# safe-autonomous-systems/fluidgym

Measured on AMD Instinct MI355X. Metric: env-steps/sec (batched) + pressure-Poisson HBM GB/s vs roofline, 1/2/4/8 GPUs, higher is better.
Workload: dtype f32; 1 GPU; ChannelJet2D-v0 (2D channel stand-in for 'cylinder Re=100 256x128'), 64 envs/GPU, 25 PISO steps/env step, random jets, stirred by a body force N(0,2.0) redrawn every env step; global_batch=64, parallelism=env-sharded x1, 1 bcast + 1 all_gather per step (RCCL), lanes_per_gpu=2, workload_modified=True, capped_solves=0, floor_released_solves=0, advection_solver_form=two-brick, velocity_solver=on-chip Jacobi sweeps (policy advection_jacobi; 11972 solves settled by

## Files before the change

fluidgym_amd/_lib.py:

```python
from __future__ import annotations

import ctypes
import os
from ctypes import POINTER, Structure, c_char_p, c_float, c_int, c_int32, c_int64, c_void_p

_HERE = os.path.dirname(os.path.abspath(__file__))
LIB_PATH = os.environ.get("FLUIDGYM_AMD_LIB") or os.path.join(_HERE, "libfluidgym_hip.so")
LIB_F64_PATH = os.environ.get("FLUIDGYM_AMD_LIB_F64") or os.path.join(_HERE, "libfluidgym_hip_f64.so")

FG_MAX_SCALARS = 4
FG_FIELD_SUMMARY_WORK_BYTES = 128
FG_OK = 0
FG_ERR_NOT_CONVERGED = -5
FG_ERR_NOT_FINITE = -6
FG_ERR_FLUX_BALANCE = -7
FG_PERIODIC, FG_FIXED = 0, 1
FG_DIRICHLET, FG_NEUMANN = 0, 1
FG_VELOCITY, FG_PRESSURE, FG_SCALAR, FG_VELOCITY_SOURCE, FG_VISCOSITY_FIELD = 0, 1, 2, 3, 4
FG_BOUND_VELOCITY, FG_BOUND_SCALAR = 8, 16
FG_SOLVER_CG, FG_SOLVER_JACOBI, FG_SOLVER_RBGS, FG_SOLVER_MGCG, FG_SOLVER_FDCG = 0, 1, 2, 3, 4
(FG_BUF_A, FG_BUF_C_OFF, FG_BUF_ADV_RHS, FG_BUF_VEL_RESULT, FG_BUF_H, FG_BUF_DIV, FG_BUF_P_RESULT,
 FG_BUF_SCALAR_RESULT) = range(8)
FG_ERR_UNSUPPORTED = -4
FG_ERR_INVALID_ARG = -1
# ... 298 lines not shown
    "fg_poisson_cg": (c_int, [c_void_p, c_void_p, c_void_p, c_void_p, c_float, c_int, c_int, POINTER(FgSolveInfo),
                              c_void_p]),
    "fg_poisson_fdcg": (c_int, [c_void_p, c_void_p, c_void_p, c_void_p, c_float, c_int, c_int, POINTER(FgSolveInfo),
                                c_void_p]),
    "fg_sparse_apply_ell": (c_int, [c_void_p, c_void_p, c_int32, c_int32, c_void_p, c_int64, c_int32, c_void_p, c_void_p]),
    "fg_sparse_apply_csr": (c_int, [c_void_p, c_void_p, c_void_p, c_int32, c_void_p, c_int64, c_int32, c_void_p, c_void_p]),
    "fg_stream_triad": (c_int, [c_void_p, c_void_p, c_void_p, c_float, c_int64, c_int32, POINTER(c_float), c_void_p]),
    "fg_mb_multilevel_status": (c_int, [c_void_p, POINTER(c_int32)]),
    "fg_mb_multilevel_apply": (c_int, [c_void_p, c_void_p, c_void_p, c_void_p]),
    "fg_mb_debug_ilu_apply": (c_int, [c_void_p, c_void_p, c_void_p, c_void_p]),
    "fg_mb_debug_pressure_cg": (c_int, [c_void_p, c_float, c_int32, c_int32, POINTER(c_int32), POINTER(c_int32), POINTER(ctypes.c_double), c_void_p]),
    "fg_mb_wall_forces": (c_int, [c_void_p, c_void_p, c_void_p, c_void_p, c_int32, c_int32, c_float, c_float, c_void_p, c_void_p]),
    "fg_mb_wall_forces_batch": (c_int, [c_void_p, c_void_p, c_void_p, c_void_p, c_int32, c_int32, c_float, c_float, c_void_p, c_void_p, c_void_p]),
    "fg_mb_debug_bicgstab": (c_int, [c_void_p, c_float, c_int32, c_int32, POINTER(c_int64), POINTER(ctypes.c_double), POINTER(c_float), c_void_p]),
    "fg_dacc_host_sum": (c_int, [POINTER(ctypes.c_double), c_int64, ctypes.c_double, POINTER(ctypes.c_double)]),
    "fg_dacc_device_sum": (c_int, [POINTER(ctypes.c_double), c_int64, ctypes.c_double, c_int32, POINTER(ctypes.c_double), c_void_p]),
    "fg_field_summary": (c_int, [c_void_p, c_int32, c_int32, c_int64, c_int32, c_void_p, c_void_p, c_void_p, ctypes.c_double, ctypes.c_double,
                                 c_int32, c_void_p, c_void_p]),
    "fg_plane_moments": (c_int, [POINTER(c_void_p), POINTER(c_int64), c_int32, c_int32, c_int32, c_int32, c_int32, c_int32, c_void_p, c_void_p,
                                 c_void_p, c_void_p, c_void_p]),
    "fg_plane_budgets": (c_int, [POINTER(c_void_p), POINTER(c_int64), c_int32, c_int32, c_int32, c_int32, c_int32, c_void_p, c_void_p, c_void_p,
                                 c_int32, c_int32, c_void_p, c_void_p, c_void_p, c_void_p, c_void_p]),
    "fg_plane_timecorr": (c_int, [POINTER(c_void_p), POINTER(c_int64), c_int32, c_int32, c_int32, c_int32, c_int32, c_int32, c_int32,
                                  POINTER(c_int32), c_void_p, c_void_p, c_void_p, c_void_p]),
    "fg_mb_cell_moments": (c_int, [c_void_p, c_void_p, c_int32, c_int32, c_int64, POINTER(c_int64), c_int32, c_int64, c_void_p, c_void_p,
                                   c_void_p]),
    "fg_mb_cell_moments_widths": (c_int, [c_void_p, c_void_p, c_int64, POINTER(c_int64), c_int32, c_void_p, c_void_p, POINTER(c_int32)]),
    "fg_mb_wall_distribution": (c_int, [c_void_p, c_void_p, c_void_p, c_int32, c_int32, c_int64, c_int64, c_void_p, c_void_p, c_void_p, c_int32,
                                        c_int32, c_float, c_void_p, c_void_p, c_void_p]),
    "fg_mb_wall_moments": (c_int, [c_void_p, c_void_p, c_void_p, c_int32, c_int32, c_int64, c_int64, c_void_p, c_void_p, c_void_p, c_int32,
                                   c_int32, c_float, c_void_p, c_int32, c_int64, c_void_p, c_void_p, c_void_p]),
    "fg_plane_spectra": (c_int, [POINTER(c_void_p), POINTER(c_int64), c_int32, c_int32, c_int32, c_int32, c_int32, POINTER(c_int32), c_int32,
                                 c_void_p, c_void_p, c_void_p]),
    "fg_plane_histogram": (c_int, [POINTER(c_void_p), POINTER(c_int64), c_int32, c_int32, c_int32, c_int32, c_int32, POINTER(c_int32), c_int32,
                                   c_void_p, c_void_p, c_int32, POINTER(c_int32), c_int32, c_int32, c_void_p, c_void_p, c_void_p]),
    "fg_coherence_litmus": (c_int, [c_int32, c_int32, c_int32, c_int32, POINTER(c_int64), POINTER(ctypes.c_double), c_void_p]),
    "fg_profile_enable": (c_int, [c_void_p, c_int]),
    "fg_profile_kinds": (c_int, []),
    "fg_profile_kind_name": (ctypes.c_char_p, [c_int]),
    "fg_profile_read": (c_int, [c_void_p, c_int, POINTER(ctypes.c_double), POINTER(c_int64), POINTER(ctypes.c_double),
                                POINTER(ctypes.c_double), POINTER(ctypes.c_double), POINTER(ctypes.c_double),
                                POINTER(c_int64), POINTER(c_int64), POINTER(ctypes.c_double), POINTER(c_int64)]),
    "fg_coords_to_transforms": (c_int, [c_void_p, c_void_p, c_int, c_int, c_int, c_int, c_void_p]),
    "fg_resampler_create": (c_int, [c_int, POINTER(ctypes.c_int32), POINTER(ctypes.c_int32), POINTER(ctypes.c_int32),
                                    POINTER(ctypes.c_float), c_int, c_int, POINTER(c_void_p)]),
    "fg_resampler_destroy": (c_int, [c_void_p]),
    "fg_resample": (c_int, [c_void_p, c_void_p, c_int, c_int, c_void_p, c_int, c_void_p]),
    "fg_frame_colorize": (c_int, [c_void_p, c_int32, c_int32, c_int32, c_int32, c_int32, POINTER(FgFrameSpec), c_void_p, c_void_p, c_void_p,
                                  POINTER(c_int32), c_int32, c_void_p, c_void_p]),
    "fg_render_isosurface": (c_int, [c_void_p, c_int32, c_int32, c_int32, c_int32, c_int32, c_int32, c_void_p, c_void_p, c_int32, c_int32,
                                     c_void_p, c_void_p, c_void_p, POINTER(FgRenderCamera), POINTER(FgRenderOptions), c_int32, c_int32,
                                     POINTER(c_int32), c_int32, c_void_p, c_void_p, c_void_p]),
    "fg_render_volume": (c_int, [c_void_p, c_int32, c_int32, c_int32, c_int32, c_int32, c_int32, c_void_p, c_void_p, c_void_p,
                                 POINTER(FgRenderCamera), POINTER(FgRenderOptions), c_int32, c_int32, POINTER(c_int32), c_int32, c_void_p,
                                 c_void_p]),
    "fg_obs_noise_add": (c_int, [POINTER(FgNoiseSegment), c_int32, c_int32, c_int32, ctypes.c_uint64, c_void_p, c_void_p, c_void_p]),
    "fg_obs_normalize": (c_int, [POINTER(FgNormSegment), c_int32, c_int32, c_int32, c_int64, c_int64, c_void_p, c_int32, c_int32,
                                 ctypes.c_double, ctypes.c_double, c_void_p]),
    "fg_obs_return_normalize": (c_int, [c_void_p, c_void_p, c_void_p, c_void_p, c_int32, c_int32, ctypes.c_double, c_int64,
                                        ctypes.c_double, ctypes.c_double, c_int32, c_void_p]),
    "fg_baseline_opposition": (c_int, [c_void_p, c_int64, c_int32, c_int32, c_int32, c_int32, POINTER(c_int32), POINTER(ctypes.c_double), c_int32,
                                       c_int32, c_void_p, c_void_p]),
    "fg_baseline_pd": (c_int, [c_void_p, c_int64, c_int32, c_int32, c_int32, c_int32, c_int32, c_void_p, ctypes.c_double, ctypes.c_double,
                               c_void_p, c_void_p, c_void_p, c_void_p, c_void_p]),
    "fg_point_sample": (c_int, [POINTER(FgPointGrid), POINTER(c_void_p), POINTER(c_int64), c_int32, c_void_p, c_int64, c_int32, c_void_p,
                                c_void_p]),
    "fg_tracer_advect": (c_int, [POINTER(FgPointGrid), c_float, c_int32, ctypes.c_uint32, c_void_p, c_void_p, c_void_p, c_void_p, c_void_p,
                                 c_int32, c_void_p]),
    "fg_mb_point_locate": (c_int, [POINTER(FgMbPointMesh), c_void_p, c_int64, c_int32, c_void_p, c_int32, c_void_p, c_void_p, c_void_p,
                                   c_void_p]),
    "fg_mb_point_sample": (c_int, [POINTER(FgMbPointMesh), POINTER(c_void_p), POINTER(c_int64), c_int32, c_void_p, c_void_p, c_int64,
                                   c_int32, c_void_p, c_void_p]),
    "fg_mb_tracer_advect": (c_int, [POINTER(FgMbPointMesh), c_float, c_int32, c_void_p, c_void_p, c_void_p, c_void_p, c_void_p, c_void_p,
                                    c_void_p, c_void_p, c_int32, c_void_p]),
    "fg_envglue_jet_schedule": (c_int, [c_void_p, c_void_p, c_void_p, c_void_p, c_int32, c_int32, c_int32, c_void_p, c_void_p, c_void_p]),
    "fg_envglue_channel_observe": (c_int, [c_void_p, c_void_p, c_void_p, c_int32, c_int32, c_int32, c_int32, c_float, c_float, c_void_p,
                                           c_void_p, c_void_p, c_void_p, c_void_p, c_void_p]),
    "fg_envglue_channel_observe_batch": (c_int, [c_void_p, c_void_p, c_void_p, c_int32, c_int32, c_int32, c_int32, c_void_p, c_float, c_void_p,
                                                 c_void_p, c_void_p, c_void_p, c_void_p, c_void_p]),
    "fg_mb_create": (c_int, [c_int32, c_int32, c_int32, POINTER(c_void_p)]),
    "fg_mb_destroy": (c_int, [c_void_p]),
    "fg_config_dump": (c_int, [c_void_p, ctypes.c_char_p, c_int]),
    "fg_mb_config_dump": (c_int, [c_void_p, ctypes.c_char_p, c_int]),
    "fg_switch_values": (c_int, [c_int32, ctypes.c_char_p, c_int32]),
    "fg_mb_add_block": (c_int, [c_void_p, POINTER(c_float), c_int32, c_int32, c_int32, POINTER(c_int32)]),
    "fg_mb_connect": (c_int, [c_void_p, c_int32, c_int32, c_int32, c_int32, c_int32, c_int32]),
    "fg_mb_make_periodic": (c_int, [c_void_p, c_int32, c_int32]),
    "fg_mb_set_reference_quirks": (c_int, [c_void_p, c_int32, c_int32]),
    "fg_mb_set_nonortho_flags": (c_int, [c_void_p, c_int32]),
    "fg_mb_finalize": (c_int, [c_void_p]),
    "fg_mb_sizes": (c_int, [c_void_p, POINTER(c_int32), POINTER(c_int32)]),
    "fg_mb_block_info": (c_int, [c_void_p, c_int32, POINTER(c_int32), POINTER(c_int32)]),
    "fg_mb_get_host_table": (c_int, [c_void_p, c_int32, c_void_p, POINTER(c_int64)]),
    "fg_mb_get_neighbors": (c_int, [c_void_p, POINTER(c_int32)]),
    "fg_mb_bind": (c_int, [c_void_p, c_void_p, c_void_p, c_void_p, c_void_p]),
    "fg_mb_set_viscosity": (c_int, [c_void_p, c_float]),
    "fg_mb_set_viscosity_batch": (c_int, [c_void_p, c_void_p]),
    "fg_mb_piso_step": (c_int, [c_void_p, c_void_p, POINTER(FgMbStepOptions), POINTER(c_int32), c_void_p]),
    "fg_mb_max_velocity": (c_int, [c_void_p, POINTER(c_float), c_void_p]),
    "fg_mb_set_residual_projection": (c_int, [c_void_p, POINTER(c_float)]),
    "fg_mb_set_stall_limit": (c_int, [c_void_p, c_int32]),
    "fg_mb_set_advection_start": (c_int, [c_void_p, c_int]),
    "fg_mb_set_advection_jacobi": (c_int, [c_void_p, c_int]),
    "fg_mb_advection_jacobi_counts": (c_int, [c_void_p, POINTER(c_int64)]),
    "fg_mb_set_multilevel": (c_int, [c_void_p, c_int32, c_int32, POINTER(c_int32), POINTER(c_int32), POINTER(c_int32), POINTER(c_float),
                                     POINTER(c_float), c_float, c_int32]),
    "fg_mb_env_status": (c_int, [c_void_p, POINTER(c_int32)]),
    "fg_mb_ladder": (c_int, [c_void_p, POINTER(c_int64), c_int32]),
    "fg_mb_debug_cycles": (c_int, [c_void_p, POINTER(ctypes.c_uint64)]),
    "fg_mb_solver_hints": (c_int, [c_void_p, POINTER(c_int32), c_int32]),
    "fg_mb_solver_unconverged": (c_int, [c_void_p, POINTER(c_int64)]),
    "fg_solver_unconverged": (c_int, [c_void_p, POINTER(c_int64)]),
    "fg_mb_solver_counters": (c_int, [c_void_p, POINTER(c_int64), c_int32]),
    "fg_set_advection_preconditioner": (c_int, [c_void_p, c_int]),
    "fg_debug_apply_preconditioner": (c_int, [c_void_p, c_int, c_int, c_void_p, c_void_p, POINTER(c_int32), c_void_p]),
    "fg_debug_apply_pressure_preconditioner": (c_int, [c_void_p, c_int, c_void_p, c_void_p, c_void_p, POINTER(ctypes.c_double),
                                                       POINTER(c_int32), c_void_p]),
    "fg_sgs_smagorinsky": (c_int, [c_void_p, c_float, c_void_p, c_void_p]),
    "fg_flow_diagnostic": (c_int, [c_void_p, c_int, c_void_p, c_void_p]),
    "fg_mb_flow_diagnostic": (c_int, [c_void_p, c_int, c_void_p, c_void_p]),
    "fg_set_fd_helmholtz": (c_int, [c_void_p, POINTER(c_float)]),
    "fg_advection_retries": (c_int, [c_void_p, POINTER(c_int64), c_int32]),
    "fg_advection_solver_form": (c_int, [c_void_p, c_int, POINTER(c_int32)]),
    "fg_set_double_fallback": (c_int, [c_void_p, c_int]),
    "fg_set_advection_jacobi": (c_int, [c_void_p, c_int]),
    "fg_advection_jacobi_counts": (c_int, [c_void_p, POINTER(c_int64)]),
    "fg_ladder": (c_int, [c_void_p, POINTER(c_int64), c_int32]),
    "fg_solver_counters": (c_int, [c_void_p, POINTER(c_int64), c_int32]),
    "fg_mb_profile_iterations": (c_int, [c_void_p, POINTER(c_int64)]),
    "fg_mb_unit_pressure_matrix": (c_int, [c_void_p, c_void_p]),
    "fg_mb_profile_enable": (c_int, [c_void_p, c_int32]),
    "fg_mb_profile_kind_name": (c_char_p, [c_int32]),
    "fg_mb_profile_read": (c_int, [c_void_p, c_int32, POINTER(ctypes.c_double), POINTER(c_int64), POINTER(ctypes.c_double),
                                   POINTER(c_int64)]),
    "fg_mb_get_buffer": (c_int, [c_void_p, c_int32, POINTER(c_void_p), POINTER(c_int64)]),
    "fg_mb_read_buffer": (c_int, [c_void_p, c_int32, c_void_p, c_void_p]),
    "fg_mb_single_step": (c_int, [c_void_p, POINTER(FgMbSimOptions), POINTER(c_int32), POINTER(c_float), c_void_p]),
    "fg_mb_update_advective_boundary": (c_int, [c_void_p, c_float, c_int32, c_int32, c_int32, c_int32, POINTER(c_float), c_float, c_void_p]),
    "fg_mb_make_divergence_free": (c_int, [c_void_p, POINTER(FgMbStepOptions), c_void_p]),
    "fg_mb_boundary_flux_balance": (c_int, [c_void_p, POINTER(c_float), c_void_p]),
    "fg_mb_get_boundary_tables": (c_int, [c_void_p, POINTER(c_int32), POINTER(c_int32), POINTER(c_float)]),
    "fg_mb_get_cell_transforms": (c_int, [c_void_p, POINTER(c_float)]),
}

def _f64_struct(cls):
    fields = []
    for name, tp in cls._fields_:
        if tp is c_float:
            tp = ctypes.c_double
        elif isinstance(tp, type) and issubclass(tp, ctypes.Array) and tp._type_ is c_float:
            tp = ctypes.c_double * tp._length_
        elif isinstance(tp, type) and issubclass(tp, Structure) and tp in _F64_STRUCTS:
            tp = _F64_STRUCTS[tp]
        fields.append((name, tp))
    return type(cls.__name__ + "F64", (Structure,), {"_fields_": fields})


_F64_STRUCTS: dict = {}
_F64_STRUCTS[FgStepOptions] = _f64_struct(FgStepOptions)
_F64_STRUCTS[FgSimOptions] = _f64_struct(FgSimOptions)
_F64_STRUCTS[FgMbStepOptions] = _f64_struct(FgMbStepOptions)
_F64_STRUCTS[FgMbSimOptions] = _f64_struct(FgMbSimOptions)
_F64_STRUCTS[FgPointGrid] = _f64_struct(FgPointGrid)
FgPointGridF64 = _F64_STRUCTS[FgPointGrid]
_F64_STRUCTS[FgMbPointMesh] = _f64_struct(FgMbPointMesh)
FgMbPointMeshF64 = _F64_STRUCTS[FgMbPointMesh]
# ... 88 lines not shown
```

fluidgym_amd/csrc/fg_api.hip:

```cpp
#include <stdio.h>
#include <string.h>

#include <cmath>
#include <string>
#include <vector>

#include <stdlib.h>

#include "fg_internal.h"
#include "fg_bicg.h"

static thread_local std::string g_last_error;
void fg_set_error(const std::string& msg) { g_last_error = msg; }

extern "C" int fg_abi_version(void) { return FG_ABI_VERSION; }
extern "C" const char* fg_last_error(void) { return g_last_error.c_str(); }

static FgBounds make_bounds(const fg_state* s, int channel) {
    FgBounds b;
    for (int f = 0; f < 6; ++f) {
        b.vel[f] = s->bvel[f];
        b.scal[f] = s->bscal[f];
        b.scalar_bc[f] = s->cfg.scalar_bc[f][channel < 0 ? 0 : channel];
    }
// ... 6 lines not shown
        if (!s->grid.fixed[f]) continue;
        FG_REQUIRE(s->bvel[f], FG_ERR_NOT_BOUND, "boundary velocity of a FIXED face not bound");
        if (need_scalar) FG_REQUIRE(s->bscal[f], FG_ERR_NOT_BOUND, "boundary scalar of a FIXED face not bound");
    }
    if (need_scalar) FG_REQUIRE(s->scalar, FG_ERR_NOT_BOUND, "passive scalar not bound");
    return FG_OK;
}

extern "C" int fg_create(const fg_config* cfg, const fg_real* hx, const fg_real* hy, const fg_real* hz, fg_handle* out) {
    FG_REQUIRE(cfg && out && hx && hy, FG_ERR_INVALID_ARG, "fg_create: null argument");
    FG_REQUIRE(cfg->dims == 2 || cfg->dims == 3, FG_ERR_INVALID_ARG, "dims must be 2 or 3");
    FG_REQUIRE(cfg->dims == 2 || hz, FG_ERR_INVALID_ARG, "hz required in 3-D");
    FG_REQUIRE(cfg->nx >= 3 && cfg->ny >= 3 && (cfg->dims == 2 ? cfg->nz == 1 : cfg->nz >= 3), FG_ERR_INVALID_ARG,
               "block needs >= 3 cells per axis (nz = 1 in 2-D)");
    FG_REQUIRE(cfg->batch >= 1, FG_ERR_INVALID_ARG, "batch must be >= 1");
    FG_REQUIRE(cfg->n_scalars >= 0 && cfg->n_scalars <= FG_MAX_SCALARS, FG_ERR_INVALID_ARG, "bad n_scalars");
    for (int a = 0; a < cfg->dims; ++a)
        FG_REQUIRE(cfg->face_type[2 * a] == cfg->face_type[2 * a + 1], FG_ERR_INVALID_ARG,
                   "a FIXED face needs a FIXED partner (CloseBoundary closes both, domain_structs.cpp:1981-2002)");
    FG_REQUIRE((long long)cfg->nx * cfg->ny * cfg->nz * cfg->batch * 6 < (1LL << 31), FG_ERR_UNSUPPORTED,
               "index space exceeds int32 (reference index_t is int32 as well)");
    FG_HIP_CHECK(hipSetDevice(cfg->device));

    fg_state* s = new fg_state();
    memset(s, 0, sizeof(*s));
    fg_switches_read(s);
    s->cfg = *cfg;
    FgGrid& g = s->grid;
    g.dims = cfg->dims; g.nx = cfg->nx; g.ny = cfg->ny; g.nz = cfg->nz;
    g.n = cfg->nx * cfg->ny * cfg->nz; g.B = cfg->batch;
    for (int f = 0; f < 6; ++f) g.fixed[f] = (f < 2 * cfg->dims) ? (cfg->face_type[f] == FG_FIXED) : 0;
    s->vec = (!FG_F64 && cfg->nx % 4 == 0) ? 4 : 1;
    s->viscosity = 0.f;

    const fg_real* hsrc[3] = {hx, hy, hz};
    const int hn[3] = {cfg->nx, cfg->ny, cfg->nz};
    for (int a = 0; a < 3; ++a) {
        std::vector<fg_real> h(hn[a], 1.f), rh(hn[a], 1.f);
        if (a < cfg->dims)
            for (int i = 0; i < hn[a]; ++i) {
                if (!(hsrc[a][i] > 0.f)) { delete s; fg_set_error("cell widths must be positive"); return FG_ERR_INVALID_ARG; }
                h[i] = hsrc[a][i]; rh[i] = 1.f / hsrc[a][i];
            }
        FG_HIP_CHECK(hipMalloc(&s->d_h[a], sizeof(fg_real) * hn[a]));
        FG_HIP_CHECK(hipMalloc(&s->d_rh[a], sizeof(fg_real) * hn[a]));
        FG_HIP_CHECK(hipMemcpy(s->d_h[a], h.data(), sizeof(fg_real) * hn[a], hipMemcpyHostToDevice));
        FG_HIP_CHECK(hipMemcpy(s->d_rh[a], rh.data(), sizeof(fg_real) * hn[a], hipMemcpyHostToDevice));
        g.h[a] = s->d_h[a]; g.rh[a] = s->d_rh[a];
    }
    const size_t BN = (size_t)g.B * g.n, d = g.dims;
    auto alloc = [&](fg_real** p, size_t count) -> hipError_t {
        hipError_t e = hipMalloc(p, sizeof(fg_real) * count);
        if (e == hipSuccess) e = hipMemset(*p, 0, sizeof(fg_real) * count);
        return e;
    };
    FG_HIP_CHECK(alloc(&s->A, BN));
    FG_HIP_CHECK(alloc(&s->rA, BN));
    FG_HIP_CHECK(alloc(&s->Coff, BN * 2 * d));
    FG_HIP_CHECK(alloc(&s->adv_rhs, BN * d));
    FG_HIP_CHECK(alloc(&s->vel_result, BN * d));
    FG_HIP_CHECK(alloc(&s->hvec, BN * d));
    FG_HIP_CHECK(alloc(&s->div, BN));
    FG_HIP_CHECK(alloc(&s->p_result, BN));
    FG_HIP_CHECK(alloc(&s->scal_result, BN));
    for (int i = 0; i < 8; ++i) FG_HIP_CHECK(alloc(&s->w[i], BN * d));
    const size_t nsys = (size_t)g.B * d;
    FG_HIP_CHECK(hipMalloc(&s->acc, sizeof(FgDacc) * nsys * FG_ACC_DOUBLES));
    FG_HIP_CHECK(hipMemset(s->acc, 0, sizeof(FgDacc) * nsys * FG_ACC_DOUBLES));
    FG_HIP_CHECK(hipMalloc(&s->flags, sizeof(int32_t) * nsys));
    FG_HIP_CHECK(hipMalloc(&s->info_dev, sizeof(fg_solve_info) * nsys));
    FG_HIP_CHECK(hipHostMalloc(&s->info_pinned, sizeof(fg_solve_info) * nsys));
    FG_HIP_CHECK(hipHostMalloc(&s->flags_pinned, sizeof(int32_t) * nsys));
    FG_HIP_CHECK(alloc(&s->scratch_B, (size_t)g.B * (4 + 2 * d)));
    FG_HIP_CHECK(hipMalloc(&s->d_bvel_ptrs, sizeof(fg_real*) * 6));
    FG_HIP_CHECK(hipMemset(s->d_bvel_ptrs, 0, sizeof(fg_real*) * 6));
    FG_HIP_CHECK(hipHostMalloc(&s->diag_pinned, sizeof(fg_real) * 2 * g.B));
    FG_HIP_CHECK(hipHostMalloc(&s->dt_pinned, sizeof(fg_real) * g.B));
    FG_HIP_CHECK(alloc(&s->dt_dev, g.B));
    FG_HIP_CHECK(hipMalloc(&s->env_sel_dev, sizeof(fg_env_sel) * g.B));
    s->t_rem_dev = nullptr;
#if !FG_F64
    FG_HIP_CHECK(hipMalloc(&s->t_rem_dev, sizeof(double) * g.B));
    FG_HIP_CHECK(hipMemset(s->t_rem_dev, 0, sizeof(double) * g.B));
#endif
    if (int rc = fg_poll_create(&s->poll, (int)(nsys > 2 * (size_t)g.B ? nsys : 2 * (size_t)g.B))) return rc;
    for (int k = 0; k < 4; ++k) { s->pred_bicg[k] = 2; s->pred_cg[k] = 1; }
    s->wall_forcing_axis = -1;
    s->ref64_inner = 1e-4f;
    s->fd_row_epoch = -1; s->rA_epoch = 0; s->fd_row_part_epoch = -1;
    for (int k = 0; k < 4; ++k) s->jac_hist[k] = FgJacHist{0, 0, 0};
    s->jac_solves = s->jac_fallbacks = 0;
    FG_HIP_CHECK(hipHostMalloc(&s->jac_prev, sizeof(float) * 4 * nsys));
    s->jac_rA_epoch = -1;
    FG_HIP_CHECK(hipMalloc(&s->fcg_alpha, sizeof(double) * 2 * (size_t)g.B));
    FG_HIP_CHECK(hipMemset(s->fcg_alpha, 0, sizeof(double) * 2 * (size_t)g.B));
    FG_HIP_CHECK(hipMalloc(&s->fcg_xsum, sizeof(FgDacc) * 2 * (size_t)g.B));
    FG_HIP_CHECK(hipMemset(s->fcg_xsum, 0, sizeof(FgDacc) * 2 * (size_t)g.B));
    FG_HIP_CHECK(hipMalloc(&s->fcg_lazy, sizeof(int32_t) * (size_t)g.B));
    FG_HIP_CHECK(hipMemset(s->fcg_lazy, 0, sizeof(int32_t) * (size_t)g.B));
    s->cg_return_best = 1;
    s->cg_reset_steps = 100;
    s->adv_from_result = 1;
    FG_HIP_CHECK(hipMalloc(&s->cg_acc, sizeof(FgDacc) * (size_t)g.B * 8 * 64));
    FG_HIP_CHECK(hipMemset(s->cg_acc, 0, sizeof(FgDacc) * (size_t)g.B * 8 * 64));
    FG_HIP_CHECK(hipMalloc(&s->cg_best.best_crit, sizeof(fg_real) * g.B));
    FG_HIP_CHECK(hipMalloc(&s->cg_best.saved_crit, sizeof(fg_real) * g.B));
    FG_HIP_CHECK(hipMalloc(&s->cg_best.save_at, sizeof(int32_t) * g.B));
    FG_HIP_CHECK(alloc(&s->cg_best.best_x, BN));
    *out = s;
    return FG_OK;
}

extern "C" int fg_destroy(fg_handle s) {
    if (!s) return FG_OK;
    for (int a = 0; a < 3; ++a) { (void)hipFree(s->d_h[a]); (void)hipFree(s->d_rh[a]); }
    fg_real* owned[] = {s->A, s->rA, s->Coff, s->adv_rhs, s->vel_result, s->hvec, s->div, s->p_result, s->scal_result,
                      s->scratch_B};
    for (fg_real* p : owned) (void)hipFree(p);
    for (int i = 0; i < 8; ++i) (void)hipFree(s->w[i]);
    (void)hipFree(s->acc); (void)hipFree(s->flags); (void)hipFree(s->info_dev);
    (void)hipHostFree(s->info_pinned); (void)hipHostFree(s->flags_pinned);
    fg_prof_destroy(s);
    fg_poll_destroy(&s->poll);
    (void)hipFree(s->d_bvel_ptrs); (void)hipHostFree(s->diag_pinned); (void)hipHostFree(s->dt_pinned); (void)hipFree(s->dt_dev); (void)hipFree(s->t_rem_dev); (void)hipFree(s->env_sel_dev);
    float* fd[] = {s->fd_Qx, s->fd_QxT, s->fd_Qz, s->fd_QzT, s->fd_lower, s->fd_inv, s->fd_cp};
    for (float* p : fd) if (p) (void)hipFree(p);
    if (s->fd_dct_tw) { (void)hipFree(s->fd_dct_tw); (void)hipFree(s->fd_dct_rot); }
    (void)hipFree(s->cg_acc); (void)hipFree(s->fcg_alpha); (void)hipFree(s->fcg_xsum); (void)hipFree(s->fcg_lazy);
    if (s->jac_prev) (void)hipHostFree(s->jac_prev);
    (void)hipFree(s->fd_row_part); (void)hipFree(s->fd_lam_x); (void)hipFree(s->fd_row_inv); (void)hipFree(s->fd_row_cp); (void)hipFree(s->fd_row_lower);
    (void)hipFree(s->line_inv); (void)hipFree(s->line_cp); (void)hipFree(s->ilu_d);
    (void)hipFree(s->r64_buf); (void)hipFree(s->r64_acc); (void)hipFree(s->ref64_x); (void)hipFree(s->force_uniform);
    (void)hipFree(s->fd_lam); (void)hipFree(s->helm_diag); (void)hipFree(s->helm_lower); (void)hipFree(s->helm_upper); (void)hipFree(s->helm_tmp); (void)hipFree(s->helm_lower_row); (void)hipFree(s->helm_lower_row2); (void)hipFree(s->line_inv2); (void)hipFree(s->line_cp2);
    (void)hipFree(s->cg_best.best_crit); (void)hipFree(s->cg_best.saved_crit); (void)hipFree(s->cg_best.save_at); (void)hipFree(s->cg_best.best_x);
    delete s;
    return FG_OK;
}

static int sync_bvel_ptrs(fg_state* s);
extern "C" int fg_bind(fg_handle s, int field, fg_real* ptr) {
    FG_REQUIRE(s, FG_ERR_INVALID_ARG, "null handle");
    if (field == FG_VELOCITY) s->velocity = ptr;
    else if (field == FG_PRESSURE) s->pressure = ptr;
    else if (field == FG_SCALAR) s->scalar = ptr;
    else if (field == FG_VELOCITY_SOURCE) s->velocity_source = ptr;
    else if (field == FG_VISCOSITY_FIELD) s->visc_field = ptr;
    else if (field >= FG_BOUND_VELOCITY && field < FG_BOUND_VELOCITY + 6) {
        s->bvel[field - FG_BOUND_VELOCITY] = ptr;
        return sync_bvel_ptrs(s);
    }
    else if (field >= FG_BOUND_SCALAR && field < FG_BOUND_SCALAR + 6) s->bscal[field - FG_BOUND_SCALAR] = ptr;
    else FG_REQUIRE(false, FG_ERR_INVALID_ARG, "fg_bind: unknown field id");
    return FG_OK;
}

extern "C" int fg_set_viscosity(fg_handle s, fg_real v) {
    FG_REQUIRE(s, FG_ERR_INVALID_ARG, "null handle");
    s->viscosity = v;
    return FG_OK;
}
extern "C" int fg_set_scalar_viscosity(fg_handle s, int ch, fg_real v) {
    FG_REQUIRE(s && ch >= 0 && ch < FG_MAX_SCALARS, FG_ERR_INVALID_ARG, "bad channel");
    s->scalar_viscosity[ch] = v;
    s->scalar_viscosity_set = true;
    return FG_OK;
}
extern "C" int fg_set_viscosity_batch(fg_handle s, const fg_real* nu_B) {
    FG_REQUIRE(s, FG_ERR_INVALID_ARG, "null handle");
    s->viscosity_B = nu_B;
    s->helm_pre_mask = 0;
    return FG_OK;
}
extern "C" int fg_set_scalar_viscosity_batch(fg_handle s, int ch, const fg_real* k_B) {
    FG_REQUIRE(s && ch >= 0 && ch < FG_MAX_SCALARS, FG_ERR_INVALID_ARG, "bad channel");
    s->scalar_viscosity_B[ch] = k_B;
    s->helm_pre_mask = 0;
    return FG_OK;
}

extern "C" int fg_set_fd_preconditioner(fg_handle s, const float* Qx, const float* QxT, const float* Qz, const float* QzT,
                                        const float* lower, const float* inv, const float* cp) {
    FG_REQUIRE(s && Qx && QxT && lower && inv && cp, FG_ERR_INVALID_ARG, "null argument");
    FG_REQUIRE(s->grid.fixed[2] && s->grid.fixed[3], FG_ERR_UNSUPPORTED, "FD preconditioner needs FIXED y faces");
    FG_REQUIRE(s->grid.dims == 2 || (Qz && QzT), FG_ERR_INVALID_ARG, "Qz required in 3-D");
#if !FG_F64
    FG_REQUIRE(s->grid.ny <= 640, FG_ERR_UNSUPPORTED, "FD preconditioner: at most 640 cells along y (LDS of the tridiagonal solve)");
#endif
    const size_t nx = s->grid.nx, ny = s->grid.ny, nz = s->grid.nz;
    auto up = [&](float** dst, const float* src, size_t count) -> hipError_t {
        if (*dst) (void)hipFree(*dst);
        hipError_t e = hipMalloc(dst, sizeof(float) * count);
        if (e == hipSuccess) e = hipMemcpy(*dst, src, sizeof(float) * count, hipMemcpyHostToDevice);
        return e;
    };
    FG_HIP_CHECK(up(&s->fd_Qx, Qx, nx * nx));
    FG_HIP_CHECK(up(&s->fd_QxT, QxT, nx * nx));
    if (s->grid.dims == 3) {
        FG_HIP_CHECK(up(&s->fd_Qz, Qz, nz * nz));
        FG_HIP_CHECK(up(&s->fd_QzT, QzT, nz * nz));
    }
    FG_HIP_CHECK(up(&s->fd_lower, lower, ny));
    FG_HIP_CHECK(up(&s->fd_inv, inv, nx * ny * nz));
    FG_HIP_CHECK(up(&s->fd_cp, cp, nx * ny * nz));
    s->fd_dct_x = 0;
    return FG_OK;
}

// ... 222 lines not shown
    a.vel = s->velocity;
    a.dt = dt_B;
    a.for_scalar = for_scalar;
    a.channel = channel;
    a.n_scalars = s->cfg.n_scalars;
    a.A = s->A; a.Coff = s->Coff; a.rhs = s->adv_rhs;
    if (for_scalar) {
        a.scal = s->scalar + (size_t)channel * s->grid.n;
        a.scal_env_stride = (long)s->cfg.n_scalars * s->grid.n;
        a.nu = fg_nu(s, 1, channel);
    } else {
        a.source = s->velocity_source;
        if (s->wall_forcing_axis >= 0)
            if (int rc = fg_launch_wall_forcing(s, (hipStream_t)stream)) return rc;
        a.force = s->wall_forcing_axis >= 0 ? s->force_uniform : nullptr;
        a.visc = s->visc_field;
        a.nu = fg_nu(s);
        a.rA = s->rA;
        s->adv_last_dt = dt_B;
        s->rA_epoch++;
        s->jac_rA_epoch = s->rA_epoch;
#if !FG_F64
        if (fg_fd_rowmean_ok(s) && s->vec == 4 && (s->grid.nx & 63) == 0) {
            if (!s->fd_row_part) FG_HIP_CHECK(hipMalloc(&s->fd_row_part, sizeof(float) * (size_t)s->grid.B * s->grid.ny * (s->grid.nx / 64)));
            a.row_part = s->fd_row_part;
            s->fd_row_part_epoch = s->rA_epoch;
        }
#endif
        if (buoy_axis >= 0) {
            a.buoy_T = s->scalar; a.buoy_stride = (long)s->cfg.n_scalars * s->grid.n; a.buoy_axis = buoy_axis; a.buoy_factor = buoy_factor;
            a.source_w = s->velocity_source;
        }
    }
    return fg_launch_adv_build(s, make_bounds(s, channel), a, (hipStream_t)stream);
}

static int advection_solve(fg_state* s, FgBicgArgs a, fg_solve_info* info, hipStream_t st, int for_scalar = 0, int channel = 0, bool* spec_ran = nullptr);

extern "C" int fg_solve_advection(fg_handle s, int for_scalar, int channel, fg_real tol, int max_iterations,
                                  fg_solve_info* info_host, void* stream) {
    FG_REQUIRE(s, FG_ERR_INVALID_ARG, "null handle");
    FgBicgArgs a;
    a.diag = s->A; a.off = s->Coff; a.rhs = s->adv_rhs;
    a.dt = s->cur_dt;
    a.tol = tol; a.max_iterations = max_iterations;
    if (for_scalar) { a.x = s->scal_result; a.nc = 1; a.use_x0 = 0; a.kind = 0; }
    else { a.x = s->vel_result; a.nc = s->grid.dims; a.use_x0 = s->adv_from_result; }
    return advection_solve(s, a, info_host, (hipStream_t)stream, for_scalar, channel);
}

extern "C" int fg_copy_scalar_result_to_blocks(fg_handle s, int channel, void* stream) {
    FG_REQUIRE(s && s->scalar, FG_ERR_NOT_BOUND, "scalar not bound");
    const int n = s->grid.n;
    if (s->cfg.n_scalars == 1) return fg_launch_copy_active(s, s->cur_dt, s->scal_result, s->scalar, 1, (hipStream_t)stream);
    FG_HIP_CHECK(hipMemcpy2DAsync(s->scalar + (size_t)channel * n, sizeof(fg_real) * n * s->cfg.n_scalars, s->scal_result,
                                  sizeof(fg_real) * n, sizeof(fg_real) * n, s->grid.B, hipMemcpyDeviceToDevice,
                                  (hipStream_t)stream));
    return FG_OK;
}

extern "C" int fg_setup_pressure_matrix(fg_handle s, void* stream) {
    FG_REQUIRE(s, FG_ERR_INVALID_ARG, "null handle");
    s->rA_epoch++;
    return fg_launch_pressure_setup(s, s->cur_dt, (hipStream_t)stream);
}

extern "C" int fg_setup_pressure_rhs(fg_handle s, const fg_real* dt_B, void* stream) {
    FG_REQUIRE(s && dt_B, FG_ERR_INVALID_ARG, "null argument");
    if (int rc = check_bound(s, false)) return rc;
    hipStream_t st = (hipStream_t)stream;
    if (int rc = fg_launch_h(s, dt_B, s->vel_result, st)) return rc;
    return fg_launch_div(s, make_bounds(s, 0), dt_B, s->hvec, s->div, st);
}

struct SpecH { fg_state* s; const fg_real* dt; const fg_step_options* opt; hipStream_t st; };
static int spec_h(void* p) {
    const SpecH* c = static_cast<const SpecH*>(p);
    fg_state* s = c->s;
    if (int rc = fg_launch_h(s, c->dt, s->vel_result, c->st)) return rc;
    return fg_launch_div(s, make_bounds(s, 0), c->dt, s->hvec, s->div, c->st, !c->opt->pressure_warm_start,
                         c->opt->pressure_method == FG_SOLVER_FDCG && s->fd_Qx != nullptr);
}

static int launch_corrector(fg_state* s, const fg_real* dt, const FgCgOutcome& o, bool last, hipStream_t st) {
    const bool mean_folded = last && o.mean_ready;
    FG_REQUIRE(!o.lazy_z || !last || mean_folded, FG_ERR_UNSUPPORTED, "fg_piso_step: an unmaterialised pressure without its folded mean");
    if (last && !mean_folded)
        if (int rc = fg_launch_mean_sub(s, dt, s->p_result, s->pressure, st)) return rc;
    const FgMeanRef mean = {s->fcg_xsum, s->info_dev, s->pressure, o.marks_valid ? s->fcg_lazy : nullptr, s->fcg_alpha};
    const FgLazyRef lazy = {s->fcg_lazy, s->fcg_alpha, last ? s->p_result : nullptr};
    const fg_real* p = o.lazy_z ? o.lazy_z : ((last && !mean_folded) ? s->pressure : s->p_result);
    return fg_launch_correct(s, dt, s->rA, s->hvec, p, s->vel_result, st, last ? s->velocity : nullptr, mean_folded ? &mean : nullptr, o.lazy_z ? &lazy : nullptr);
}

struct SpecCorrect { fg_state* s; const fg_real* dt; bool last; hipStream_t st; };
static int spec_correct(void* p, const FgCgOutcome& o) {
    const SpecCorrect* c = static_cast<const SpecCorrect*>(p);
    return launch_corrector(c->s, c->dt, o, c->last, c->st);
}

static int solve_pressure(fg_state* s, const fg_real* dt, int method, fg_real tol, int max_iterations, int use_previous,
                          fg_solve_info* info_host, hipStream_t st, bool finalize = true, int kind = 2, FgCgOutcome* out = nullptr,
                          FgCgSpec spec = FgCgSpec{}) {
    int rc = FG_OK;
    FgCgOutcome own;
    if (!out) out = &own;
    if (method == FG_SOLVER_CG || method == FG_SOLVER_FDCG) {
        FgCgArgs a;
        a.rA = s->rA; a.b = s->div; a.x = s->p_result;
        a.r = s->w[0]; a.p = s->w[1]; a.Ap = s->w[2];
        a.dt = dt; a.tol = tol; a.max_iterations = max_iterations; a.use_x0 = use_previous;
        a.reset_steps = s->cg_reset_steps;
        a.precond = (method == FG_SOLVER_FDCG);
        a.kind = kind;
        a.check_every = a.precond ? 2 : 16;
        a.lazy_ok = finalize ? 0 : 1;
        a.spec = spec;
#if !FG_F64
        if (s->ref64_outer > 0) a.lazy_ok = 0;
#endif
        rc = fg_cg_solve(s, a, info_host, st, out);
#if !FG_F64
        if (s->ref64_outer > 0 && (rc == FG_OK || rc == FG_ERR_NOT_CONVERGED)) rc = fg_refine64_pressure(s, a, info_host, st, out);
        if (s->double_fallback && (rc == FG_ERR_NOT_FINITE || (s->ladder_force & 2))) {
            std::vector<fg_solve_info> tmp;
            fg_solve_info* info = info_host;
            if (!info) { tmp.assign(s->info_pinned, s->info_pinned + s->grid.B); info = tmp.data(); }
            s->rung_count[2] += 1;
            rc = fg_rung64_cg(s, a, info, (s->ladder_force & 2) != 0, st, out);
        }
#endif
    } else {
        fg_set_error("fg_solve_pressure: only FG_SOLVER_CG drives the PISO step (Jacobi/RBGS are smoothers)");
        return FG_ERR_UNSUPPORTED;
    }
    if (rc != FG_OK && rc != FG_ERR_NOT_CONVERGED) return rc;
    if (finalize)
        if (int rc2 = fg_launch_mean_sub(s, dt, s->p_result, s->pressure, st)) return rc2;
    return rc;
}

extern "C" int fg_solve_pressure(fg_handle s, int method, fg_real tol, int max_iterations, int use_previous,
                                 fg_solve_info* info_host, void* stream) {
    FG_REQUIRE(s, FG_ERR_INVALID_ARG, "null handle");
    if (int rc = check_bound(s, false)) return rc;
    return solve_pressure(s, s->cur_dt, method, tol, max_iterations, use_previous, info_host, (hipStream_t)stream);
}

extern "C" int fg_set_pressure_refinement(fg_handle s, int32_t max_corrections, fg_real target_tol, fg_real inner_relative_tol) {
    FG_REQUIRE(s, FG_ERR_INVALID_ARG, "null handle");
    FG_REQUIRE(!FG_F64 || max_corrections <= 0, FG_ERR_UNSUPPORTED, "fg_set_pressure_refinement: the fp64 build solves in fp64 already");
    FG_REQUIRE(max_corrections <= 0 || (target_tol > 0 && inner_relative_tol > 0 && inner_relative_tol < 1), FG_ERR_INVALID_ARG,
               "fg_set_pressure_refinement: tolerances must be positive, the relative one below 1");
    s->ref64_outer = max_corrections > 0 ? max_corrections : 0;
    s->ref64_tol = (float)target_tol; s->ref64_inner = (float)inner_relative_tol;
    return FG_OK;
}

extern "C" int fg_correct_velocity(fg_handle s, void* stream) {
    FG_REQUIRE(s, FG_ERR_INVALID_ARG, "null handle");
    if (int rc = check_bound(s, false)) return rc;
    return fg_launch_correct(s, s->cur_dt, s->rA, s->hvec, s->pressure, s->vel_result, (hipStream_t)stream);
}

extern "C" int fg_copy_velocity_result_to_blocks(fg_handle s, void* stream) {
    FG_REQUIRE(s && s->velocity, FG_ERR_NOT_BOUND, "velocity not bound");
    return fg_launch_copy_active(s, s->cur_dt, s->vel_result, s->velocity, s->grid.dims, (hipStream_t)stream);
}
extern "C" int fg_copy_velocity_result_from_blocks(fg_handle s, void* stream) {
    FG_REQUIRE(s && s->velocity, FG_ERR_NOT_BOUND, "velocity not bound");
    return fg_launch_copy_active(s, nullptr, s->velocity, s->vel_result, s->grid.dims, (hipStream_t)stream);
}

static int max_iters(const fg_solve_info* info, int n) {
    int m = -1;
    for (int i = 0; i < n; ++i) m = info[i].used_iterations > m ? info[i].used_iterations : m;
    return m;
}

static int advection_solve(fg_state* s, FgBicgArgs a, fg_solve_info* info, hipStream_t st, int for_scalar, int channel, bool* spec_ran) {
    a.precond = (s->adv_precond == 1) ? 1 : (s->adv_precond == 3 ? 2 : (s->adv_precond == 4 ? 3 : 0));
    if (a.precond == 2 && !for_scalar && s->visc_field) a.precond = 0;
    if (a.precond == 2) {
        a.nu = fg_nu(s, for_scalar, channel);
        a.wall_lo = for_scalar ? (s->cfg.scalar_bc[2][channel] == FG_DIRICHLET) : 1;
        a.wall_hi = for_scalar ? (s->cfg.scalar_bc[3][channel] == FG_DIRICHLET) : 1;
    }
    const int nsys = s->grid.B * a.nc;
    std::vector<fg_solve_info> info_own;
    if (!info) { info_own.resize(nsys); info = info_own.data(); }
    int rc = fg_bicgstab_solve(s, a, info, st, spec_ran);
    bool failed = (rc == FG_ERR_NOT_CONVERGED || rc == FG_ERR_NOT_FINITE) || (s->ladder_force & 1);
#if !FG_F64
    if (failed && s->double_fallback && rc != FG_ERR_HIP) {
        s->rung_count[0] += 1;
        rc = fg_rung64_bicgstab(s, a, info, (s->ladder_force & 1) != 0, st);
        if (rc != FG_OK && rc != FG_ERR_NOT_CONVERGED && rc != FG_ERR_NOT_FINITE) return rc;
        failed = (rc != FG_OK) || (s->ladder_force & 4);
    }
#endif
    if (failed && (s->adv_precond == 2 || s->adv_precond == 5)) {
        s->line_retries += 1;
        s->rung_count[1] += 1;
        a.precond = s->adv_precond == 5 ? 3 : 1; a.use_x0 = 0;
        rc = fg_bicgstab_solve(s, a, info, st);
    }
    (void)nsys;
    return rc;
}

extern "C" int fg_piso_step(fg_handle s, const fg_real* dt_B, const fg_step_options* opt, int32_t* stats_host,
                            void* stream) {
    FG_REQUIRE(s && dt_B && opt, FG_ERR_INVALID_ARG, "null argument");
    const bool scalar = opt->advect_scalar && s->cfg.n_scalars > 0;
    if (int rc = check_bound(s, scalar)) return rc;
    FG_REQUIRE(opt->buoyancy_axis < s->grid.dims, FG_ERR_INVALID_ARG, "bad buoyancy axis");
    FG_REQUIRE(opt->buoyancy_axis < 0 || (s->velocity_source && s->scalar), FG_ERR_NOT_BOUND,
               "buoyancy needs velocity source and scalar bound");
    hipStream_t st = (hipStream_t)stream;
    const int B = s->grid.B, d = s->grid.dims;
    std::vector<fg_solve_info> info((size_t)B * d);
    int32_t stats[4] = {-1, -1, -1, -1};
    struct DropHelmRecord { fg_state* s; ~DropHelmRecord() { s->helm_pre_mask = 0; } } drop_helm_record{s};
    int status = FG_OK;
    auto soft = [&](int rc) {
        if (rc == FG_ERR_NOT_CONVERGED) { status = rc; return FG_OK; }
        return rc;
    };
#if !FG_F64
    const bool sweeps_first = s->adv_linesweep && s->grid.dims == 2 && s->jac_hist[0].skip == 0 && s->jac_hist[1].skip == 0;
    if (scalar && s->cfg.n_scalars == 1 && s->adv_precond == 3 && s->fd_lam && !s->visc_field && !sweeps_first) {
        const FgNu nu2[2] = {fg_nu(s, 1, 0), fg_nu(s)};
        const int wlo[2] = {s->cfg.scalar_bc[2][0] == FG_DIRICHLET, 1}, whi[2] = {s->cfg.scalar_bc[3][0] == FG_DIRICHLET, 1};
        if (int rc = fg_helm_factor_pair(s, dt_B, nu2, wlo, whi, st)) return rc;
    }
#endif
    if (scalar) {
        FgRange range_scalar("scalar_advection");
        for (int ch = 0; ch < s->cfg.n_scalars; ++ch) {
            if (int rc = fg_setup_advection(s, dt_B, 1, ch, stream)) return rc;
            FgBicgArgs a;
            a.diag = s->A; a.off = s->Coff; a.rhs = s->adv_rhs; a.x = s->scal_result; a.nc = 1;
            a.dt = dt_B; a.tol = opt->advection_tol; a.max_iterations = opt->max_iterations; a.use_x0 = 0; a.kind = 0;
            if (int rc = soft(advection_solve(s, a, info.data(), st, 1, ch))) return rc;
            const int m = max_iters(info.data(), B);
            stats[0] = m > stats[0] ? m : stats[0];
            s->ctr.add(0, info.data(), B);
            const int n = s->grid.n;
            if (s->cfg.n_scalars == 1) {
                if (int rc = fg_launch_copy_active(s, dt_B, s->scal_result, s->scalar, 1, st)) return rc;
            } else {
                (void)n;
                fg_set_error("multi-channel scalar copy with inactive envs not implemented");
                return FG_ERR_UNSUPPORTED;
            }
        }
    }
    fg_range_push("velocity_assembly_and_solve");
    struct PopOnce { bool armed = true; void fire() { if (armed) { fg_range_pop(); armed = false; } } ~PopOnce() { fire(); } } range_velocity;
    if (int rc = setup_advection(s, dt_B, 0, 0, stream, opt->buoyancy_axis, opt->buoyancy_factor)) return rc;
    bool h_div_ran = false;
    {
        FgBicgArgs a;
        a.diag = s->A; a.off = s->Coff; a.rhs = s->adv_rhs; a.x = s->vel_result; a.nc = d;
        a.dt = dt_B; a.tol = opt->advection_tol; a.max_iterations = opt->max_iterations; a.use_x0 = s->adv_from_result;
        SpecH spec_h_ctx = {s, dt_B, opt, st};
        if (opt->corrector_steps > 0) a.spec = FgSpecHook{spec_h, &spec_h_ctx};
        if (int rc = soft(advection_solve(s, a, info.data(), st, 0, 0, &h_div_ran))) return rc;
        stats[1] = max_iters(info.data(), B * d);
        s->ctr.add(1, info.data(), B * d);
    }
    range_velocity.fire();
    for (int c = 0; c < opt->corrector_steps; ++c) {
        FgRange range_corr(c == 0 ? "pressure_corrector_0" : "pressure_corrector_1+");
        const bool last = (c + 1 == opt->corrector_steps);
        if (!(c == 0 && h_div_ran)) {
            if (int rc = fg_launch_h(s, dt_B, s->vel_result, st)) return rc;
            if (int rc = fg_launch_div(s, make_bounds(s, 0), dt_B, s->hvec, s->div, st, !opt->pressure_warm_start,
                                       opt->pressure_method == FG_SOLVER_FDCG && s->fd_Qx != nullptr))
                return rc;
        }
        SpecCorrect spec_ctx = {s, dt_B, last, st};
        FgCgOutcome outcome;
        if (int rc = soft(solve_pressure(s, dt_B, opt->pressure_method, opt->pressure_tol, opt->max_iterations, opt->pressure_warm_start ? 1 : 0,
                                         info.data(), st, false, c == 0 ? 0 : 1, &outcome, FgCgSpec{spec_correct, &spec_ctx})))
            return rc;
        if (c < 2) { stats[2 + c] = max_iters(info.data(), B); s->ctr.add(2 + c, info.data(), B); }
        if (!outcome.spec_done)
            if (int rc = launch_corrector(s, dt_B, outcome, last, st)) return rc;
    }
    if (opt->corrector_steps <= 0)
        if (int rc = fg_launch_copy_active(s, dt_B, s->vel_result, s->velocity, d, st)) return rc;
    if (stats_host) memcpy(stats_host, stats, sizeof(stats));
    s->ctr.piso_steps += 1;
    return status;
}

extern "C" int fg_config_dump(fg_handle s, char* buf, int n) {
    FG_REQUIRE(s && buf && n > 0, FG_ERR_INVALID_ARG, "fg_config_dump: bad argument");
    std::string out = std::string("{\"build\": \"") + (FG_F64 ? "f64" : "f32") + "\"";
    fg_switches_json(s, out);
    const std::pair<const char*, long long> state[] = {
        {"fast_transform_x", s->fd_dct_x}, {"fd_preconditioner", s->fd_Qx ? 1 : 0}, {"helmholtz", s->fd_lam ? 1 : 0}, {"advection_preconditioner", s->adv_precond},
        {"advection_from_result", s->adv_from_result}, {"return_best", s->cg_return_best}, {"cg_reset_steps", s->cg_reset_steps}, {"double_fallback", s->double_fallback},
        {"wall_forcing_axis", s->wall_forcing_axis}, {"first_iterate_polls", s->fcg_first_polls}, {"unstored_pressure_solves", s->fcg_unstored},
        {"jacobi_speculation_misses", s->jac_spec_missed}, {"jacobi_floor_released", s->jac_floor_released}, {"pressure_refinement_corrections", s->ref64_corrections}};
    for (const auto& kv : state) fg_json_put(out, kv.first, kv.second);
    return fg_json_out(out + "}", buf, n);
}

extern "C" int fg_solver_unconverged(fg_handle s, int64_t* out4) {
    FG_REQUIRE(s != nullptr && out4 != nullptr, FG_ERR_INVALID_ARG, "fg_solver_unconverged: bad argument");
    for (int k = 0; k < 4; ++k) out4[k] = s->ctr.unconv[k];
    return FG_OK;
}

extern "C" int fg_solver_counters(fg_handle s, int64_t* out13, int32_t reset) {
    FG_REQUIRE(s != nullptr, FG_ERR_INVALID_ARG, "fg_solver_counters: null handle");
    if (out13) s->ctr.write(out13);
    if (reset) s->ctr.reset();
    return FG_OK;
}

extern "C" int fg_single_step(fg_handle s, const fg_sim_options* o, int32_t* out, fg_real* flux_host, void* stream);
extern "C" int fg_multi_step(fg_handle s, const fg_sim_options* o, int32_t n, const fg_real* const* bvel_schedule, int32_t* out_6n,
                             fg_real* flux_host, int32_t* steps_done, void* stream) {
    FG_REQUIRE(s && o && out_6n && n >= 0, FG_ERR_INVALID_ARG, "fg_multi_step: bad argument");
    if (steps_done) *steps_done = 0;
    for (int k = 0; k < n; ++k) {
        if (bvel_schedule)
            for (int f = 0; f < 2 * s->grid.dims; ++f)
                if (const fg_real* p = bvel_schedule[(size_t)k * 6 + f])
                    if (int rc = fg_bind(s, FG_BOUND_VELOCITY + f, const_cast<fg_real*>(p))) return rc;
        if (int rc = fg_single_step(s, o, out_6n + 6 * (size_t)k, flux_host, stream)) return rc;
        if (steps_done) *steps_done = k + 1;
        if (out_6n[6 * (size_t)k + 5] == 0 && !s->cg_return_best) break;
    }
    return FG_OK;
}

static inline bool is_close_zero(double a) { return std::fabs(a) <= 1e-8; }

extern "C" int fg_single_step(fg_handle s, const fg_sim_options* o, int32_t* out, fg_real* flux_host, void* stream) {
    fg_htrace("single_step_in");
    FgRange range_sim("fg_single_step");
    FG_REQUIRE(s && o && out, FG_ERR_INVALID_ARG, "null argument");
    if (int rc = check_bound(s, o->step.advect_scalar && s->cfg.n_scalars > 0)) return rc;
    hipStream_t st = (hipStream_t)stream;
    const int B = s->grid.B;
    const FgBounds bnd = make_bounds(s, 0);
    std::vector<double> t_rem(B, (double)o->time_step);
    int32_t stats[4] = {-1, -1, -1, -1};
    int substeps = 0, all_ok = 1;
    bool first = true;
    int fixed_left = o->adaptive ? 0 : (o->substeps > 0 ? o->substeps : 1);
    for (;;) {
        bool any = false;
        if (o->adaptive) {
            for (int b = 0; b < B; ++b) any = any || (t_rem[b] > 0 && !is_close_zero(t_rem[b]));
        } else {
            any = fixed_left > 0;
        }
        if (!any) break;
        auto advance = [&](int b, fg_real max_vel) -> fg_real {
            fg_real ts = 0.f;
            if (!o->adaptive) {
                ts = o->time_step;
            } else if (t_rem[b] > 0 && !is_close_zero(t_rem[b])) {
                const double mv = (double)max_vel;
                const double max_ts = is_close_zero(mv) ? t_rem[b] : (double)o->cfl / mv;
                double tsd;
                if (max_ts >= t_rem[b]) tsd = t_rem[b];
                else tsd = t_rem[b] / (double)(long long)std::ceil(t_rem[b] / max_ts);
                t_rem[b] -= tsd;
                ts = (fg_real)tsd;
            }
            return ts;
        };
        auto flux_guard = [&]() -> int {
            fg_real worst = 0.f;
            for (int b = 0; b < B; ++b) {
                if (flux_host) flux_host[b] = s->diag_pinned[b];
                const fg_real a = std::fabs(s->diag_pinned[b]);
                worst = (a > worst || a != a) ? a : worst;
            }
            if (!(worst <= o->flux_balance_tol)) {
                fg_set_error("Domain boundary fluxes not balanced, cannot proceed with simulation step.");
                return FG_ERR_FLUX_BALANCE;
            }
            return FG_OK;
        };
        bool deferred = false;
        FgPollOut po_cfl = FgPollOut{nullptr, 0};
        if (o->adaptive || first) {
            const FgPollOut po = fg_poll_next(&s->poll);
            po_cfl = po;
            if (first && !o->adaptive) { if (int rc = fg_launch_flux_balance(s, bnd, s->diag_pinned, st, FgPollOut{po.seq, po.value})) return rc; }
            if (o->adaptive) {
                deferred = po.gran != nullptr && s->dev_dt && s->t_rem_dev != nullptr;
                const FgDtRule rule = deferred ? FgDtRule{s->t_rem_dev, s->dt_dev, (float)o->cfl, (double)o->time_step, first ? 1 : 0}
                                               : FgDtRule{nullptr, nullptr, 0.f, 0.0, 0};
                if (int rc = fg_launch_max_velocity(s, bnd, s->scratch_B + B, st, s->diag_pinned + B, po.seq ? FgPollOut{po.seq + B, po.value, po.gran} : po,
                                                    first ? s->scratch_B : nullptr, first ? s->diag_pinned : nullptr, rule))
                    return rc;
            }
            fg_htrace("maxvel_launched");
            if (!deferred) {
                if (o->adaptive && po.gran) {
                    if (int rc = fg_poll_wait_words(&s->poll, po, 12 * B, first ? 2 * B : B, st)) return rc;
                    for (int b = 0; b < B; ++b) {
                        s->diag_pinned[B + b] = fg_poll_word_float(&s->poll, 12 * B + b);
                        if (first) s->diag_pinned[b] = fg_poll_word_float(&s->poll, 13 * B + b);
                    }
                } else if (int rc = fg_poll_wait(&s->poll, po, o->adaptive ? B : 0, o->adaptive ? 1 : B, st)) return rc;
                fg_htrace("maxvel_poll_done");
                if (first) if (int rc = flux_guard()) return rc;
            }
        }
        if (!deferred)
            for (int b = 0; b < B; ++b) s->dt_pinned[b] = advance(b, o->adaptive ? s->diag_pinned[B + b] : (fg_real)0);
        const bool folded = o->outflow_mask && fg_outflow_folds(s, o->outflow_mask);
        const bool dt_by_value = folded && B <= 64 && !deferred;
        if (!dt_by_value && !deferred) FG_HIP_CHECK(hipMemcpyAsync(s->dt_dev, s->dt_pinned, sizeof(fg_real) * B, hipMemcpyHostToDevice, st));
        if (o->outflow_mask) {
            for (int f = 0; f < 2 * s->grid.dims; ++f)
                if ((o->outflow_mask >> f) & 1) FG_REQUIRE(s->grid.fixed[f], FG_ERR_INVALID_ARG, "outflow face is not FIXED");
            if (!folded)
                for (int f = 0; f < 2 * s->grid.dims; ++f)
                    if ((o->outflow_mask >> f) & 1)
                        if (int rc = fg_launch_outflow(s, f, o->outflow_velm[f >> 1], s->dt_dev, st)) return rc;
            fg_real velm3[3] = {o->outflow_velm[0], o->outflow_velm[1], o->outflow_velm[2]};
            if (int rc = fg_launch_balance(s, bnd, o->outflow_mask, (fg_real)0.01 * o->outflow_tol, s->dt_dev, st, folded ? o->outflow_mask : 0, velm3,
                                           dt_by_value ? s->dt_pinned : nullptr))
                return rc;
        }
        int rc = fg_piso_step(s, s->dt_dev, &o->step, stats, stream);
        if (rc == FG_ERR_NOT_CONVERGED) all_ok = 0;
        else if (rc != FG_OK) return rc;
        if (deferred) {
            if (int rc2 = fg_poll_wait_words(&s->poll, po_cfl, 12 * B, first ? 2 * B : B, st)) return rc2;
            for (int b = 0; b < B; ++b) {
                s->diag_pinned[B + b] = fg_poll_word_float(&s->poll, 12 * B + b);
                if (first) s->diag_pinned[b] = fg_poll_word_float(&s->poll, 13 * B + b);
            }
            if (first) if (int rc2 = flux_guard()) return rc2;
            for (int b = 0; b < B; ++b) s->dt_pinned[b] = advance(b, s->diag_pinned[B + b]);
        }
        ++substeps;
        first = false;
        if (!o->adaptive) --fixed_left;
        if (substeps >= (o->max_substeps > 0 ? o->max_substeps : 100000)) break;
    }
    fg_htrace("single_step_out");
    for (int i = 0; i < 4; ++i) out[i] = stats[i];
    out[4] = substeps;
    out[5] = all_ok;
    return FG_OK;
}

extern "C" int fg_make_divergence_free(fg_handle s, fg_real tol, int max_iterations, fg_solve_info* info_host,
                                       void* stream) {
    FG_REQUIRE(s, FG_ERR_INVALID_ARG, "null handle");
    if (int rc = check_bound(s, false)) return rc;
    s->cur_dt = nullptr;
    hipStream_t st = (hipStream_t)stream;
    const size_t BN = (size_t)s->grid.B * s->grid.n;
    std::vector<fg_real> ones(BN, 1.f);
    FG_HIP_CHECK(hipMemcpyAsync(s->rA, ones.data(), sizeof(fg_real) * BN, hipMemcpyHostToDevice, st));
    s->rA_epoch++;
    FG_HIP_CHECK(hipStreamSynchronize(st));
    if (int rc = fg_launch_copy_active(s, nullptr, s->velocity, s->hvec, s->grid.dims, st)) return rc;
    if (int rc = fg_launch_div(s, make_bounds(s, 0), nullptr, s->hvec, s->div, st)) return rc;
    int rc = solve_pressure(s, nullptr, FG_SOLVER_CG, tol, max_iterations, 0, info_host, st);
    if (rc != FG_OK && rc != FG_ERR_NOT_CONVERGED) return rc;
    if (int rc2 = fg_launch_correct(s, nullptr, s->rA, s->hvec, s->pressure, s->vel_result, st)) return rc2;
    if (int rc2 = fg_launch_copy_active(s, nullptr, s->vel_result, s->velocity, s->grid.dims, st)) return rc2;
    return rc;
}

extern "C" int fg_reset_solver_state(fg_handle s, void* stream) {
    FG_REQUIRE(s && s->velocity, FG_ERR_NOT_BOUND, "velocity not bound");
    for (int k = 0; k < 4; ++k) s->jac_hist[k] = FgJacHist{0, 0, 0};
    FG_HIP_CHECK(hipMemsetAsync(s->p_result, 0, sizeof(fg_real) * (size_t)s->grid.B * s->grid.n, (hipStream_t)stream));
    return fg_launch_copy_active(s, nullptr, s->velocity, s->vel_result, s->grid.dims, (hipStream_t)stream);
}

extern "C" int fg_solver_hints(fg_handle s, int32_t* hints12, int32_t set) {
    FG_REQUIRE(s != nullptr && hints12 != nullptr, FG_ERR_INVALID_ARG, "fg_solver_hints: bad argument");
    for (int k = 0; k < 4; ++k) {
        FgJacHist& H = s->jac_hist[k];
        if (set) { H.sweeps = hints12[3 * k]; H.skip = hints12[3 * k + 1]; H.fails = hints12[3 * k + 2]; }
        else { hints12[3 * k] = H.sweeps; hints12[3 * k + 1] = H.skip; hints12[3 * k + 2] = H.fails; }
    }
    return FG_OK;
}

extern "C" int fg_get_buffer(fg_handle s, int which, fg_real** out_ptr, int64_t* out_count) {
    FG_REQUIRE(s && out_ptr && out_count, FG_ERR_INVALID_ARG, "null argument");
    const int64_t BN = (int64_t)s->grid.B * s->grid.n, d = s->grid.dims;
    switch (which) {
        case FG_BUF_A: *out_ptr = s->A; *out_count = BN; break;
        case FG_BUF_C_OFF: *out_ptr = s->Coff; *out_count = BN * 2 * d; break;
        case FG_BUF_ADV_RHS: *out_ptr = s->adv_rhs; *out_count = BN * d; break;
        case FG_BUF_VEL_RESULT: *out_ptr = s->vel_result; *out_count = BN * d; break;
        case FG_BUF_H: *out_ptr = s->hvec; *out_count = BN * d; break;
        case FG_BUF_DIV: *out_ptr = s->div; *out_count = BN; break;
        case FG_BUF_P_RESULT: *out_ptr = s->p_result; *out_count = BN; break;
        case FG_BUF_SCALAR_RESULT: *out_ptr = s->scal_result; *out_count = BN; break;
        default:
            if (which >= 100 && which < 108) { *out_ptr = s->w[which - 100]; *out_count = BN * d; break; }
            FG_REQUIRE(false, FG_ERR_INVALID_ARG, "unknown buffer id");
    }
    return FG_OK;
}

extern "C" int fg_read_buffer(fg_handle s, int which, fg_real* dst, void* stream) {
    fg_real* src = nullptr;
    int64_t count = 0;
    if (int rc = fg_get_buffer(s, which, &src, &count)) return rc;
    FG_REQUIRE(dst, FG_ERR_INVALID_ARG, "null destination");
    FG_HIP_CHECK(hipMemcpyAsync(dst, src, sizeof(fg_real) * count, hipMemcpyDeviceToDevice, (hipStream_t)stream));
    return FG_OK;
}

extern "C" int fg_poisson_apply(fg_handle s, const fg_real* rA, const fg_real* x, fg_real* y, void* stream) {
    FG_REQUIRE(s && rA && x && y, FG_ERR_INVALID_ARG, "null argument");
    return fg_poisson_apply_launch(s, rA, x, y, (hipStream_t)stream);
}

extern "C" int fg_poisson_jacobi(fg_handle s, const fg_real* rA, const fg_real* b, fg_real* x, int n_sweeps, fg_real omega,
                                 void* stream) {
    FG_REQUIRE(s && rA && b && x && n_sweeps >= 0, FG_ERR_INVALID_ARG, "bad argument");
    hipStream_t st = (hipStream_t)stream;
    fg_real* buf[2] = {x, s->w[5]};
    for (int i = 0; i < n_sweeps; ++i)
        if (int rc = fg_poisson_jacobi_launch(s, rA, b, buf[i & 1], buf[(i + 1) & 1], omega, st)) return rc;
// ... 53 lines not shown
```

fluidgym_amd/csrc/fg_internal.h:

```cpp
#pragma once
#include <hip/hip_runtime.h>
#include <hip/hip_ext.h>
#include <math.h>
#include <stdint.h>
#include <cstring>
#include <string>
#include <type_traits>

#include "../../include/fluidgym_hip.h"
#include "fg_switches.h"

#ifdef FG_REAL_DOUBLE
struct alignas(16) fg_real4 { double x, y, z, w; };
__host__ __device__ __forceinline__ fg_real4 make_fg_real4(double x, double y, double z, double w) { fg_real4 r; r.x = x; r.y = y; r.z = z; r.w = w; return r; }
#define FG_F64 1
#define FG_FMAX fmax
#define FG_FABS fabs
#define FG_SQRT sqrt
#else
typedef float4 fg_real4;
#define make_fg_real4 make_float4
#define FG_F64 0
#define FG_FMAX fmaxf
#define FG_FABS fabsf
// ... 562 lines not shown
    bool cg_for(const fg_real* dt) const { return cg_ns > 0 && cg_dt == dt; }
    void set_cg_start(int form) { cg_start = form; }
    bool take_bicg(int nc, const fg_real* dt) { const bool ready = bicg_nc == nc && bicg_dt == dt; clear(); return ready; }
    int take_cg(int ns, int best, const fg_real* dt) {
        const int got = (cg_ns == ns && cg_best == best && cg_dt == dt) ? cg_start : -1; clear(); return got;
    }
};

struct FgNu {
    fg_real v = 0; const fg_real* per_env = nullptr;
#ifdef __HIPCC__
    __device__ __forceinline__ fg_real at(int b) const { return per_env ? per_env[b] : v; }
#endif
    bool same(const FgNu& o) const { return v == o.v && per_env == o.per_env; }
};

struct fg_state {
    fg_config cfg;
    FgGrid grid;
    int vec;
    fg_real viscosity;
    fg_real scalar_viscosity[FG_MAX_SCALARS];
    bool scalar_viscosity_set;
    const fg_real* viscosity_B;
    const fg_real* scalar_viscosity_B[FG_MAX_SCALARS];
    fg_real* d_h[3];
    fg_real* d_rh[3];
    fg_real* velocity;
    fg_real* pressure;
    fg_real* scalar;
    fg_real* velocity_source;
    fg_real* visc_field;
    fg_real* bvel[6];
    fg_real* bscal[6];
    fg_real* A;
    fg_real* rA;
    fg_real* Coff;
    fg_real* adv_rhs;
    fg_real* vel_result;
    fg_real* hvec;
    fg_real* div;
    fg_real* p_result;
    fg_real* scal_result;
    fg_real* w[8];
    FgDacc* acc;
    int32_t* flags;
    fg_solve_info* info_dev;
    fg_solve_info* info_pinned;
    int32_t* flags_pinned;
    fg_real* scratch_B;
    FgProf prof;
    FgDacc* cg_acc;
    FgBest cg_best;
    int cg_return_best;
    int cg_reset_steps;
    int adv_from_result;
    int adv_precond; long long line_retries;
    int wall_forcing_axis; fg_real wall_forcing_coef[2]; fg_real* force_uniform;
    FG_SB_SWITCHES(FG_SW_MEMBER)
    double* fcg_alpha; FgDacc* fcg_xsum;
    int32_t* fcg_lazy;
    long jac_spec_missed;
    long jac_floor_released = 0;
    long fcg_unstored, fcg_first_polls;
    fg_real* line_inv; fg_real* line_cp;
    fg_real* ilu_d;
    int double_fallback; int ladder_force; long long rung_count[4];
    double* r64_buf; FgDacc* r64_acc;
    int ref64_outer; float ref64_tol, ref64_inner; double* ref64_x; long ref64_corrections;
    float* fd_Qx; float* fd_QxT; float* fd_Qz; float* fd_QzT; float* fd_lower; float* fd_inv; float* fd_cp;
    float* fd_lam; float* helm_diag; float* helm_lower; float* helm_upper; float* helm_tmp;
    float* helm_lower_row; float helm_rs; int helm_cb;
    float* line_inv2; float* line_cp2; float* helm_lower_row2; int helm_pre_mask; const fg_real* helm_pre_dt; FgNu helm_pre_nu[2]; int helm_pre_walls[2][2]; int helm_set;
    int fd_dct_x; float2* fd_dct_tw; float2* fd_dct_rot; float fd_dct_fwd[2]; float fd_dct_inv[2];
    float* fd_lam_x; float* fd_row_inv; float* fd_row_cp; float* fd_row_lower; long fd_row_epoch; mutable long rA_epoch;
    float* fd_row_part; long fd_row_part_epoch;
    int32_t* forms_rec;
    const fg_real* adv_last_dt;
    fg_real** d_bvel_ptrs;
    fg_real* diag_pinned;
    fg_real* dt_pinned;
    fg_real* dt_dev;
    double* t_rem_dev;
    int pred_bicg[4], pred_cg[4];
    int adv_jacobi, adv_jacobi_env; FgJacHist jac_hist[4]; float* jac_prev;
    long long jac_solves, jac_fallbacks;
    long jac_rA_epoch;
    FgCounters ctr;
    const fg_real* cur_dt;
    FgPoll poll;
    mutable int maxvel_clean;
    FgPrepared prepared;
    fg_env_sel* env_sel_dev;
    size_t n_cells() const { return (size_t)grid.n; }
};
inline FgNu fg_nu(const fg_state* s, int for_scalar = 0, int channel = 0) {
    FgNu n;
    if (for_scalar && s->scalar_viscosity_B[channel]) { n.v = s->scalar_viscosity[channel]; n.per_env = s->scalar_viscosity_B[channel]; }
    else if (for_scalar && s->scalar_viscosity_set) n.v = s->scalar_viscosity[channel];
    else { n.v = s->viscosity; n.per_env = s->viscosity_B; }
    return n;
}

void fg_set_error(const std::string& msg);
#define FG_REQUIRE(cond, code, msg)  \
    do {                             \
        if (!(cond)) {               \
            fg_set_error(msg);       \
            return code;             \
        }                            \
    } while (0)
#define FG_HIP_CHECK(expr)                                                                        \
    do {                                                                                          \
        hipError_t _e = (expr);                                                                   \
        if (_e != hipSuccess) {                                                                   \
            fg_set_error(std::string(#expr) + ": " + hipGetErrorString(_e));                      \
            return FG_ERR_HIP;                                                                    \
        }                                                                                         \
    } while (0)

#if FG_F64
#define FG_DISPATCH(s, ...)                                                       \
    do {                                                                          \
        if ((s)->grid.dims == 2) { constexpr int DIMS = 2, VEC = 1; __VA_ARGS__; } \
        else { constexpr int DIMS = 3, VEC = 1; __VA_ARGS__; }                    \
    } while (0)
#else
#define FG_DISPATCH(s, ...)                                                       \
    do {                                                                          \
        if ((s)->grid.dims == 2) {                                                \
            if ((s)->vec == 4) { constexpr int DIMS = 2, VEC = 4; __VA_ARGS__; }  \
            else { constexpr int DIMS = 2, VEC = 1; __VA_ARGS__; }                \
        } else {                                                                  \
            if ((s)->vec == 4) { constexpr int DIMS = 3, VEC = 4; __VA_ARGS__; }  \
            else { constexpr int DIMS = 3, VEC = 1; __VA_ARGS__; }                \
        }                                                                         \
    } while (0)
#endif

struct FgBicgBegin { FgDacc* acc; fg_real* sc; int32_t* flags; fg_solve_info* info; int nc; };
#ifdef __HIPCC__
__device__ __forceinline__ void fg_bicg_begin_sys(const FgBicgBegin& q, const fg_real* __restrict__ dt, int sys) {
    for (int k = 0; k < FG_ACC_DOUBLES; ++k) acc_st(q.acc + ((size_t)sys * FG_ACC_DOUBLES + k), 0.0);
    sc_st(q.sc + (sys * 2), 1.f); sc_st(q.sc + (sys * 2 + 1), 1.f);
    const bool active = (dt == nullptr) || (dt[sys / q.nc] > 0.f);
    flag_st(q.flags + (sys), active ? 0 : 3);
    q.info[sys].final_residual = 0.f;
    q.info[sys].used_iterations = -1;
    q.info[sys].converged = active ? 0 : 1;
    q.info[sys].is_finite = 1;
}
#endif
struct FgAdvArgs {
    const fg_real* vel;
    const fg_real* scal;
    long scal_env_stride;
    const fg_real* source;
    const fg_real* force;
    const fg_real* dt;
    FgNu nu;
    const fg_real* visc;
    int for_scalar;
    int channel, n_scalars;
    fg_real* A; fg_real* Coff; fg_real* rhs;
    fg_real* rA;
    FgBicgBegin begin;
    const fg_real* buoy_T; long buoy_stride; int buoy_axis; fg_real buoy_factor; fg_real* source_w;
    fg_real* row_part;
};
int fg_launch_adv_build(fg_state* s, const FgBounds& bnd, const FgAdvArgs& a, hipStream_t st);
int fg_launch_wall_forcing(const fg_state* s, hipStream_t st);
int fg_launch_sgs(const fg_state* s, const FgBounds& bnd, fg_real coefficient, fg_real* out, hipStream_t st);
int fg_launch_pressure_setup(const fg_state* s, const fg_real* dt, hipStream_t st);
int fg_launch_h(fg_state* s, const fg_real* dt, const fg_real* vel_result, hipStream_t st);
int fg_launch_div(fg_state* s, const FgBounds& bnd, const fg_real* dt, const fg_real* hvec, fg_real* div, hipStream_t st,
                  bool cg_from_zero = false,
                  bool fused_fwd = false);
struct FgMeanRef { const FgDacc* sums; const fg_solve_info* info; fg_real* p_copy; const int32_t* lazy; const double* alpha; };
struct FgLazyRef { const int32_t* lazy; const double* alpha; fg_real* p_res; };
int fg_launch_correct(const fg_state* s, const fg_real* dt, const fg_real* rA, const fg_real* hvec, const fg_real* p,
                      fg_real* vel_out, hipStream_t st, fg_real* vel_copy = nullptr, const FgMeanRef* mean = nullptr, const FgLazyRef* lazy = nullptr);
struct FgDtRule { double* t_rem; fg_real* dt_out; float cfl; double time_step; int reset; };
int fg_launch_max_velocity(const fg_state* s, const FgBounds& bnd, fg_real* out_B, hipStream_t st, fg_real* mirror_B = nullptr,
                           FgPollOut poll = FgPollOut{nullptr, 0}, fg_real* flux_B = nullptr, fg_real* flux_mirror = nullptr,
                           FgDtRule rule = FgDtRule{nullptr, nullptr, 0.f, 0.0, 0});
int fg_launch_flux_balance(const fg_state* s, const FgBounds& bnd, fg_real* out_B, hipStream_t st, FgPollOut poll = FgPollOut{nullptr, 0});
int fg_launch_copy_active(const fg_state* s, const fg_real* dt, const fg_real* src, fg_real* dst, int comps, hipStream_t st);
int fg_launch_buoyancy(const fg_state* s, const fg_real* dt, const fg_real* T, long t_env_stride, fg_real* source, int axis,
                       fg_real factor, hipStream_t st);
int fg_launch_outflow(const fg_state* s, int face, fg_real velm_axis, const fg_real* dt, hipStream_t st);
int fg_launch_balance(const fg_state* s, const FgBounds& bnd, int free_mask, fg_real atol, const fg_real* dt, hipStream_t st,
                      int outflow_mask = 0, const fg_real* outflow_velm = nullptr,
                      const fg_real* dt_host_values = nullptr);
bool fg_outflow_folds(const fg_state* s, int outflow_mask);
int fg_launch_mean_sub(const fg_state* s, const fg_real* active_dt, fg_real* p, fg_real* p_copy, hipStream_t st);

int fg_poisson_apply_launch(const fg_state* s, const fg_real* rA, const fg_real* x, fg_real* y, hipStream_t st);
int fg_poisson_jacobi_launch(const fg_state* s, const fg_real* rA, const fg_real* b, const fg_real* x, fg_real* xnew,
                             fg_real omega, hipStream_t st);
int fg_poisson_rbgs_launch(const fg_state* s, const fg_real* rA, const fg_real* b, fg_real* x, fg_real omega, int color,
                           hipStream_t st);
struct FgCgOutcome {
    const fg_real* lazy_z = nullptr;
    bool mean_ready = false;
    bool marks_valid = false;
    bool spec_done = false;
};
struct FgCgSpec { int (*fn)(void* ctx, const FgCgOutcome& o) = nullptr; void* ctx = nullptr; };
struct FgCgArgs {
    const fg_real* rA; const fg_real* b; fg_real* x;
    fg_real* r; fg_real* p; fg_real* Ap;
    const fg_real* dt;
    fg_real tol; int max_iterations; int use_x0; int reset_steps;
    int check_every;
    int precond;
    int kind = 2;
    int lazy_ok = 0;
    FgCgSpec spec;
};
int fg_cg_solve(fg_state* s, const FgCgArgs& a, fg_solve_info* info_host, hipStream_t st, FgCgOutcome* out = nullptr);

struct FgSpecHook { int (*fn)(void* ctx) = nullptr; void* ctx = nullptr; };
struct FgBicgArgs {
    const fg_real* diag; const fg_real* off;
    const fg_real* rhs; fg_real* x;
    int nc;
    const fg_real* dt;
    fg_real tol; int max_iterations; int use_x0;
    int precond = 0;
    FgNu nu; int wall_lo = 1, wall_hi = 1;
    int kind = 1;
    FgSpecHook spec;
};
int fg_bicgstab_solve(fg_state* s, const FgBicgArgs& a, fg_solve_info* info_host, hipStream_t st, bool* spec_ran = nullptr);
#if !FG_F64
enum FgSweepOutcome {
    FG_SWEEP_NOT_TRIED,
    FG_SWEEP_SOLVED,
    FG_SWEEP_SOLVED_SPEC,
    FG_SWEEP_GAVE_UP,
    FG_SWEEP_SPEC_MISSED,
};
bool fg_jacobi_ok(const fg_state* s, const FgBicgArgs& a);
bool fg_linesweep_ok(const fg_state* s, const FgBicgArgs& a);
int fg_linesweep_solve(fg_state* s, const FgBicgArgs& a, fg_solve_info* info_host, hipStream_t st, FgSweepOutcome* outcome);
int fg_jacobi_solve(fg_state* s, const FgBicgArgs& a, fg_solve_info* info_host, hipStream_t st, FgSweepOutcome* outcome);
#endif
int fg_rung64_bicgstab(fg_state* s, const FgBicgArgs& a, fg_solve_info* info_host, bool all_systems, hipStream_t st);
int fg_rung64_cg(fg_state* s, const FgCgArgs& a, fg_solve_info* info_host, bool all_envs, hipStream_t st, FgCgOutcome* out);

bool fg_zmarch_ok(const fg_state* s, int* zc_out);
int fg_zmarch_apply(const fg_state* s, const fg_real* rA, const fg_real* x, fg_real* y, int zc, hipStream_t st);
int fg_zmarch_relax(const fg_state* s, const fg_real* rA, const fg_real* b, const fg_real* x, fg_real* xnew, fg_real omega,
                    int color, int zc, hipStream_t st);
int fg_zmarch_cg_ap(const fg_state* s, const fg_real* rA, const fg_real* z, const fg_real* p_in, fg_real* p_out, fg_real* Ap,
                    FgDacc* acc, int32_t* flags, fg_solve_info* info, int prof_slot, fg_real tol, int it, int first,
                    int ns, int num_base, int zc, hipStream_t st);
#define FG_PROF_SELF ((const int32_t*)(uintptr_t)1)
int fg_prof_slot(const fg_state* s, int kind, const int32_t* flags, int nsys, double bytes_per_sys,
                 double flops_per_sys, hipStream_t st);
int fg_prof_collect(fg_state* s, hipStream_t st);
void fg_prof_prefetch(fg_state* s, hipStream_t st);
void fg_prof_destroy(fg_state* s);
bool fg_fd_dct_supported(int n);
struct FgCgJudge;
int fg_fd_dct_forward(fg_state* s, const fg_real* r, fg_real* out, hipStream_t st, int batch = 0, const FgCgJudge* judge = nullptr);
int fg_fd_dct_inverse(fg_state* s, const fg_real* u, fg_real* z, const fg_real* dot_with, FgDacc* dot_acc, int dot_stride,
                      int dot_ns, hipStream_t st, int batch = 0);
#define FG_LAUNCH_P(s, slot, kernel, grid, block, shmem, st, ...)                                              \
    do {                                                                                                       \
        const int slot__ = (slot);                                                                             \
        if (slot__ >= 0)                                                                                       \
            hipExtLaunchKernelGGL(kernel, grid, block, shmem, st, (s)->prof.ev[2 * slot__],                    \
                                  (s)->prof.ev[2 * slot__ + 1], 0, __VA_ARGS__);                               \
        else                                                                                                   \
            hipLaunchKernelGGL(kernel, grid, block, shmem, st, __VA_ARGS__);                                   \
    } while (0)
// ... 22 lines not shown
```

fluidgym_amd/csrc/fg_piso.hip:

```cpp
#include "fg_internal.h"
#include "fg_cg.h"
#include "fg_fftcg.h"

namespace {

template <int VEC>
__device__ __forceinline__ fg_real fg_elem_mask(int e, fg_real lo_mask_or_hi, bool is_edge_elem) {
    return is_edge_elem ? lo_mask_or_hi : 1.f;
}

template <int DIMS, int VEC>
__device__ __forceinline__ int fg_slab_index(const FgGrid& g, const FgCtx<DIMS, VEC>& c, int a) {
    if (a == 0) return c.k * g.ny + c.j;
    if (a == 1) return c.k * g.nx + c.i0;
    return c.j * g.nx + c.i0;
}
__device__ __forceinline__ int fg_slab_size(const FgGrid& g, int a) {
    return (a == 0) ? g.ny * g.nz : (a == 1) ? g.nx * g.nz : g.nx * g.ny;
}

template <int DIMS, int VEC, bool SCALAR, bool VISC = false>
__global__ __launch_bounds__(FG_BLOCK) void k_adv_build(FgGrid g, FgBounds bnd, FgAdvArgs a, int tiles_x,
                                                         int tiles_y, int tiles) {
    const FgCtx<DIMS, VEC> c = fg_make_ctx<DIMS, VEC>(g, tiles_x, tiles_y, tiles);
// ... 186 lines not shown
                                                 const fg_real* __restrict__ rA_, const fg_real* __restrict__ Coff,
                                                 const fg_real* __restrict__ rhs, const fg_real* __restrict__ velr,
                                                 fg_real* __restrict__ hvec, FgCgBegin begin, int tiles_x, int tiles_y, int tiles) {
    const FgCtx<DIMS, VEC> c = fg_make_ctx<DIMS, VEC>(g, tiles_x, tiles_y, tiles);
    if (begin.acc && fg_xcd_remap(blockIdx.x, gridDim.x) % (unsigned)tiles == 0) fg_cg_begin_env(begin, dt, c.b);
    if (!(dt[c.b] > 0.f) || !c.valid) return;
    const size_t N = g.n;
    const FgVec<VEC> rA = fg_load<VEC>(rA_ + (size_t)c.b * N + c.idx);
    FgVec<VEC> off[2 * DIMS];
#pragma unroll
    for (int f = 0; f < 2 * DIMS; ++f) off[f] = fg_load<VEC>(Coff + ((size_t)c.b * 2 * DIMS + f) * N + c.idx);
#pragma unroll
    for (int q = 0; q < DIMS; ++q) {
        const size_t base = ((size_t)c.b * DIMS + q) * N;
        const FgNbr<DIMS, VEC> u = fg_gather<DIMS, VEC>(velr + base, c);
        const FgVec<VEC> r = fg_load<VEC>(rhs + base + c.idx);
        FgVec<VEC> out;
#pragma unroll
        for (int e = 0; e < VEC; ++e) {
            fg_real H = off[0].v[e] * u.xm.v[e] + off[1].v[e] * u.xp.v[e] + off[2].v[e] * u.ym.v[e] +
                      off[3].v[e] * u.yp.v[e];
            if constexpr (DIMS == 3) H += off[4].v[e] * u.zm.v[e] + off[5].v[e] * u.zp.v[e];
            out.v[e] = rA.v[e] * (r.v[e] - H);
        }
        fg_store<VEC>(hvec + base + c.idx, out);
    }
}

template <int DIMS, int VEC>
__global__ __launch_bounds__(FG_BLOCK) void k_div(FgGrid g, FgBounds bnd, const fg_real* __restrict__ dt,
                                                   const fg_real* __restrict__ hvec, fg_real* __restrict__ div, FgCgStart start,
                                                   int tiles_x, int tiles_y, int tiles) {
    const FgCtx<DIMS, VEC> c = fg_make_ctx<DIMS, VEC>(g, tiles_x, tiles_y, tiles);
    if (dt && !(dt[c.b] > 0.f)) return;
    if (!c.valid && !start.acc) return;
    const size_t N = g.n;
    const FgMetric<DIMS, VEC> m = fg_metrics<DIMS, VEC>(g, c);
    fg_real acc[VEC];
#pragma unroll
    for (int e = 0; e < VEC; ++e) acc[e] = 0.f;
#pragma unroll
    for (int ax = 0; ax < DIMS; ++ax) {
        FgVec<VEC> ctr, lo, hi;
        fg_gather_axis<DIMS, VEC>(hvec + ((size_t)c.b * DIMS + ax) * N, c, ax, ctr, lo, hi);
        const int slab = fg_slab_index<DIMS, VEC>(g, c, ax);
        const int slab_n = fg_slab_size(g, ax);
#pragma unroll
        for (int e = 0; e < VEC; ++e) {
            fg_real area, mask_lo, mask_hi;
            if (ax == 0) { area = m.hy * m.hz; mask_lo = (e == 0) ? c.mxm : 1.f; mask_hi = (e == VEC - 1) ? c.mxp : 1.f; }
            else if (ax == 1) { area = m.hx[e] * m.hz; mask_lo = c.mym; mask_hi = c.myp; }
            else { area = m.hx[e] * m.hy; mask_lo = c.mzm; mask_hi = c.mzp; }
            const int bi = slab + ((ax == 0) ? 0 : e);
            fg_real F_hi, F_lo;
            if (mask_hi != 0.f) F_hi = 0.5f * (ctr.v[e] + hi.v[e]) * area;
            else F_hi = bnd.vel[2 * ax + 1][((size_t)c.b * DIMS + ax) * slab_n + bi] * area;
            if (mask_lo != 0.f) F_lo = 0.5f * (ctr.v[e] + lo.v[e]) * area;
            else F_lo = bnd.vel[2 * ax][((size_t)c.b * DIMS + ax) * slab_n + bi] * area;
            acc[e] += F_hi - F_lo;
        }
    }
    FgVec<VEC> out;
#pragma unroll
    for (int e = 0; e < VEC; ++e) out.v[e] = acc[e];
    if (c.valid) fg_store<VEC>(div + (size_t)c.b * N + c.idx, out);
    if (start.acc) {
        __shared__ fg_real lds[4];
        fg_real part[1] = {0.f};
        if (c.valid) {
            FgVec<VEC> z;
#pragma unroll
            for (int e = 0; e < VEC; ++e) { z.v[e] = 0.f; part[0] += out.v[e] * out.v[e]; }
            fg_store<VEC>(start.x + (size_t)c.b * N + c.idx, z);
            fg_store<VEC>(start.r + (size_t)c.b * N + c.idx, out);
        }
        fg_block_sum<1>(part, lds);
        if (threadIdx.x == 0) {
            const unsigned tile = fg_xcd_remap(blockIdx.x, gridDim.x) % tiles;
            fg_acc_add(fg_acc_ptr(start.acc, c.b, 0), start.ns, tile, (double)part[0]);
        }
    }
}

template <int DIMS, int VEC>
__global__ __launch_bounds__(FG_BLOCK) void k_correct(FgGrid g, const fg_real* __restrict__ dt,
                                                       const fg_real* __restrict__ rA_, const fg_real* __restrict__ hvec,
                                                       const fg_real* __restrict__ p, fg_real* __restrict__ vel_out,
                                                       fg_real* __restrict__ vel_copy, FgMeanRef mean, FgLazyRef lazy, int tiles_x, int tiles_y, int tiles) {
    const FgCtx<DIMS, VEC> c = fg_make_ctx<DIMS, VEC>(g, tiles_x, tiles_y, tiles);
    if ((dt && !(dt[c.b] > 0.f)) || !c.valid) return;
    const size_t N = g.n;
    const FgMetric<DIMS, VEC> m = fg_metrics<DIMS, VEC>(g, c);
    const FgVec<VEC> rA = fg_load<VEC>(rA_ + (size_t)c.b * N + c.idx);
    FgNbr<DIMS, VEC> P = fg_gather<DIMS, VEC>(p + (size_t)c.b * N, c);
    if (lazy.lazy) {
        const bool on = lazy.lazy[c.b] == 1;
        const fg_real sc = on ? (fg_real)lazy.alpha[2 * c.b] : (fg_real)0;
        auto scale = [&](FgVec<VEC>& v) {
#pragma unroll
            for (int e = 0; e < VEC; ++e) v.v[e] = on ? sc * v.v[e] : (fg_real)0;
        };
        scale(P.c); scale(P.xm); scale(P.xp); scale(P.ym); scale(P.yp);
        if constexpr (DIMS == 3) { scale(P.zm); scale(P.zp); }
        if (lazy.p_res) fg_store<VEC>(lazy.p_res + (size_t)c.b * N + c.idx, P.c);
    }
    if (mean.sums) {
        const int used = mean.info[c.b].used_iterations;
        const bool first_only = mean.lazy && mean.lazy[c.b] == 1;
        const fg_real mu = first_only ? (fg_real)(mean.alpha[2 * c.b] * acc_ld(mean.sums + (2 * c.b + 1)) / (double)g.n)
                           : used < 0 ? (fg_real)0 : (fg_real)(acc_ld(mean.sums + (2 * c.b + (used & 1))) / (double)g.n);
        FgVec<VEC> pc;
#pragma unroll
        for (int e = 0; e < VEC; ++e) pc.v[e] = P.c.v[e] - mu;
        fg_store<VEC>(mean.p_copy + (size_t)c.b * N + c.idx, pc);
    }
#pragma unroll
    for (int q = 0; q < DIMS; ++q) {
        const size_t base = ((size_t)c.b * DIMS + q) * N;
        const FgVec<VEC> h = fg_load<VEC>(hvec + base + c.idx);
        FgVec<VEC> out;
#pragma unroll
        for (int e = 0; e < VEC; ++e) {
            fg_real lo, hi, fac, rh;
            if (q == 0) {
                lo = P.xm.v[e]; hi = P.xp.v[e]; rh = m.rhx[e];
                const fg_real ml = (e == 0) ? c.mxm : 1.f, mh = (e == VEC - 1) ? c.mxp : 1.f;
                fac = (ml == 0.f || mh == 0.f) ? 1.f : 0.5f;
            } else if (q == 1) {
                lo = P.ym.v[e]; hi = P.yp.v[e]; rh = m.rhy;
                fac = (c.mym == 0.f || c.myp == 0.f) ? 1.f : 0.5f;
            } else {
                lo = P.zm.v[e]; hi = P.zp.v[e]; rh = m.rhz;
                fac = (c.mzm == 0.f || c.mzp == 0.f) ? 1.f : 0.5f;
            }
            out.v[e] = h.v[e] - rA.v[e] * ((hi - lo) * fac * rh);
        }
        fg_store<VEC>(vel_out + base + c.idx, out);
        if (vel_copy) fg_store<VEC>(vel_copy + base + c.idx, out);
    }
}

#if FG_F64
typedef long long fg_bits;
__device__ __forceinline__ fg_bits fg_real_bits(fg_real v) { return __double_as_longlong(v); }
__device__ __forceinline__ fg_real fg_bits_real(fg_bits b) { return __longlong_as_double(b); }
#else
typedef int fg_bits;
__device__ __forceinline__ fg_bits fg_real_bits(fg_real v) { return __float_as_int(v); }
__device__ __forceinline__ fg_real fg_bits_real(fg_bits b) { return __int_as_float(b); }
#endif
template <int DIMS>
__device__ __forceinline__ double fg_flux_balance_block(const FgGrid& g, const FgBounds& bnd, int b) {
    double acc = 0.0;
    const int lane = threadIdx.x & 63, wave = threadIdx.x >> 6;
    for (int f = 0; f < 2 * DIMS; ++f) {
        if (!g.fixed[f]) continue;
        const int ax = f >> 1;
        const int slab_n = fg_slab_size(g, ax);
        const double sgn = (f & 1) ? 1.0 : -1.0;
        const int n0 = (ax == 0) ? g.ny : g.nx;
        const int n1 = (DIMS == 3) ? ((ax == 2) ? g.ny : g.nz) : 1;
        const fg_real* __restrict__ h0 = (ax == 0) ? g.h[1] : g.h[0];
        const fg_real* __restrict__ h1 = (DIMS == 3) ? ((ax == 2) ? g.h[1] : g.h[2]) : nullptr;
        const fg_real* __restrict__ v = bnd.vel[f] + ((size_t)b * DIMS + ax) * slab_n;
        constexpr int RU = 4, WV = FG_BLOCK / 64;
        for (int i1b = wave; i1b < n1; i1b += WV * RU) {
            for (int i0 = lane; i0 < n0; i0 += 64) {
                fg_real val[RU], a1[RU];
#pragma unroll
                for (int u = 0; u < RU; ++u) {
                    const int i1 = i1b + u * WV;
                    const bool ok = i1 < n1;
                    a1[u] = ok ? (h1 ? h1[i1] : (fg_real)1) : (fg_real)0;
                    val[u] = ok ? v[(size_t)i1 * n0 + i0] : (fg_real)0;
                }
                const fg_real w0 = h0[i0];
#pragma unroll
                for (int u = 0; u < RU; ++u) acc += sgn * (double)(val[u] * (w0 * a1[u]));
            }
        }
    }
    __shared__ double lds_fb[4];
#pragma unroll
    for (int o = 32; o > 0; o >>= 1) acc += __shfl_down(acc, o, 64);
    if ((threadIdx.x & 63) == 0) lds_fb[threadIdx.x >> 6] = acc;
    __syncthreads();
    return lds_fb[0] + lds_fb[1] + lds_fb[2] + lds_fb[3];
}
__device__ __forceinline__ void fg_publish_max(fg_real* out_B, int32_t* done_B, fg_real* mirror_B, int b, fg_real mx, const FgPollOut& poll, int B,
                                               fg_real* flux_B = nullptr, fg_real* flux_mirror = nullptr, const FgDtRule& rule = FgDtRule{nullptr, nullptr, 0.f, 0.0, 0}) {
    const int lane = threadIdx.x & 63;
    int last_of_all = 0;
    if (lane == 0) {
        if (!mirror_B) {
            atomicMax(reinterpret_cast<fg_bits*>(out_B) + b, fg_real_bits(mx));
        } else {
            fg_bits prev = atomicMax(reinterpret_cast<fg_bits*>(out_B) + b, fg_real_bits(mx));
#if FG_F64
            asm volatile("" ::"v"((int)(prev >> 32)), "v"((int)prev));
#else
            asm volatile("" ::"v"(prev));
#endif
            if (atomicAdd(done_B + b, 1) == (int)gridDim.x - 1) last_of_all = (atomicAdd(done_B + B, 1) == B - 1);
        }
    }
    if (!mirror_B) return;
    if (__shfl(last_of_all, 0, 64)) {
#if !FG_F64
        if (poll.gran) {
            for (int e = lane; e < B; e += 64) {
                const fg_bits mbits = __hip_atomic_exchange(reinterpret_cast<fg_bits*>(out_B) + e, (fg_bits)0, __ATOMIC_RELAXED, __HIP_MEMORY_SCOPE_AGENT);
                if (rule.t_rem) {
                    double tr = rule.reset ? rule.time_step : rule.t_rem[e];
                    float ts = 0.f;
                    if (tr > 0.0 && !(fabs(tr) <= 1e-8)) {
                        const double mv = (double)__uint_as_float(mbits);
                        const double max_ts = (fabs(mv) <= 1e-8) ? tr : (double)rule.cfl / mv;
                        const double tsd = (max_ts >= tr) ? tr : tr / (double)(long long)ceil(tr / max_ts);
                        tr -= tsd;
                        ts = (float)tsd;
                    }
                    rule.t_rem[e] = tr;
                    rule.dt_out[e] = ts;
                }
                fg_poll_publish_word(poll, 12 * B + e, mbits);
                if (flux_B) fg_poll_publish_word(poll, 13 * B + e, __hip_atomic_exchange(reinterpret_cast<fg_bits*>(flux_B) + e, (fg_bits)0, __ATOMIC_RELAXED, __HIP_MEMORY_SCOPE_AGENT));
                atomicExch(done_B + e, 0);
            }
            if (lane == 0) atomicExch(done_B + B, 0);
            return;
        }
#endif
        for (int e = lane; e < B; e += 64) {
            mirror_B[e] = fg_bits_real(__hip_atomic_exchange(reinterpret_cast<fg_bits*>(out_B) + e, (fg_bits)0, __ATOMIC_RELAXED, __HIP_MEMORY_SCOPE_AGENT));
            if (flux_B) flux_mirror[e] = fg_bits_real(__hip_atomic_exchange(reinterpret_cast<fg_bits*>(flux_B) + e, (fg_bits)0, __ATOMIC_RELAXED, __HIP_MEMORY_SCOPE_AGENT));
            atomicExch(done_B + e, 0);
        }
        if (lane == 0) {
            atomicExch(done_B + B, 0);
            fg_poll_publish(poll, 0);
        }
    }
}

template <int DIMS>
__global__ __launch_bounds__(FG_BLOCK) void k_max_velocity(FgGrid g, FgBounds bnd, const fg_real* __restrict__ vel,
                                                            fg_real* __restrict__ out_B, int32_t* __restrict__ done_B,
                                                            fg_real* __restrict__ mirror_B, FgPollOut poll, fg_real* flux_B, fg_real* flux_mirror, FgDtRule rule) {
    const int b = blockIdx.y;
    const size_t N = g.n;
    fg_real mx = 0.f;
    for (int idx = blockIdx.x * blockDim.x + threadIdx.x; idx < g.n; idx += gridDim.x * blockDim.x) {
        const int i = idx % g.nx;
        const int j = (idx / g.nx) % g.ny;
        const int k = idx / (g.nx * g.ny);
        const fg_real rh[3] = {g.rh[0][i], g.rh[1][j], DIMS == 3 ? g.rh[2][k] : 1.f};
#pragma unroll
        for (int q = 0; q < DIMS; ++q) mx = FG_FMAX(mx, FG_FABS(vel[((size_t)b * DIMS + q) * N + idx] * rh[q]));
    }
    {
#pragma unroll
        for (int f = 0; f < 2 * DIMS; ++f) {
            if (!g.fixed[f]) continue;
            const int ax = f >> 1;
            const int slab_n = fg_slab_size(g, ax);
            const int edge = (f & 1) ? ((ax == 0) ? g.nx - 1 : (ax == 1) ? g.ny - 1 : g.nz - 1) : 0;
            for (int s = blockIdx.x * blockDim.x + threadIdx.x; s < slab_n; s += gridDim.x * blockDim.x) {
                int i, j, k;
                if (ax == 0) { i = edge; j = s % g.ny; k = s / g.ny; }
                else if (ax == 1) { j = edge; i = s % g.nx; k = s / g.nx; }
                else { k = edge; i = s % g.nx; j = s / g.nx; }
                const fg_real rh[3] = {g.rh[0][i], g.rh[1][j], DIMS == 3 ? g.rh[2][k] : 1.f};
#pragma unroll
                for (int q = 0; q < DIMS; ++q)
                    mx = FG_FMAX(mx, FG_FABS(bnd.vel[f][((size_t)b * DIMS + q) * slab_n + s] * rh[q]));
            }
        }
    }
    __shared__ fg_real lds[4];
    mx = fg_wave_max(mx);
    if ((threadIdx.x & 63) == 0) lds[threadIdx.x >> 6] = mx;
    __syncthreads();
    if (flux_B && blockIdx.x == 0) {
        const double total = fg_flux_balance_block<DIMS>(g, bnd, b);
        if (threadIdx.x == 0) {
            fg_bits prevf = __hip_atomic_exchange(reinterpret_cast<fg_bits*>(flux_B) + b, fg_real_bits((fg_real)total), __ATOMIC_RELAXED, __HIP_MEMORY_SCOPE_AGENT);
#if FG_F64
            asm volatile("" ::"v"((int)(prevf >> 32)), "v"((int)prevf));
#else
            asm volatile("" ::"v"(prevf));
#endif
        }
    }
    if (threadIdx.x < 64) {
        mx = FG_FMAX(FG_FMAX(lds[0], lds[1]), FG_FMAX(lds[2], lds[3]));
        fg_publish_max(out_B, done_B, mirror_B, b, mx, poll, (int)gridDim.y, flux_B, flux_mirror, rule);
    }
}

template <int DIMS>
__global__ __launch_bounds__(FG_BLOCK) void k_max_velocity_rows(FgGrid g, FgBounds bnd, const fg_real* __restrict__ vel,
                                                                 fg_real* __restrict__ out_B, int32_t* __restrict__ done_B,
                                                                 fg_real* __restrict__ mirror_B, int rows_per_block, FgPollOut poll,
                                                                 fg_real* flux_B, fg_real* flux_mirror, FgDtRule rule) {
    const int b = blockIdx.y;
    const size_t N = g.n;
    const int lane = threadIdx.x & 63, wave = threadIdx.x >> 6;
// ... 92 lines not shown

__global__ __launch_bounds__(FG_BLOCK) void k_sum_env(const fg_real* __restrict__ dt, const fg_real* __restrict__ p,
                                                       FgDacc* __restrict__ sums, int n) {
    const int b = blockIdx.y;
    if (dt && !(dt[b] > 0.f)) return;
    const fg_real* __restrict__ pb = p + (size_t)b * n;
    fg_real acc = 0.f;
    const int n4 = ((n & 3) == 0 && (reinterpret_cast<size_t>(pb) & 15) == 0) ? n >> 2 : 0;
    for (int i = blockIdx.x * blockDim.x + threadIdx.x; i < n4; i += gridDim.x * blockDim.x) {
        const fg_real4 v = reinterpret_cast<const fg_real4*>(pb)[i];
        acc += (v.x + v.y) + (v.z + v.w);
    }
    for (int i = n4 * 4 + blockIdx.x * blockDim.x + threadIdx.x; i < n; i += gridDim.x * blockDim.x) acc += pb[i];
    __shared__ fg_real lds[4];
    fg_real v[1] = {acc};
    fg_block_sum<1>(v, lds);
    if (threadIdx.x == 0) acc_add(sums + b, (double)v[0]);
}
__global__ __launch_bounds__(FG_BLOCK) void k_sub_mean(const fg_real* __restrict__ dt, fg_real* __restrict__ p,
                                                        fg_real* __restrict__ p_copy, const FgDacc* __restrict__ sums,
                                                        int n) {
    const int b = blockIdx.y;
    if (dt && !(dt[b] > 0.f)) return;
    const fg_real mean = (fg_real)(acc_ld(sums + b) / (double)n);
    fg_real* __restrict__ pb = p + (size_t)b * n;
    fg_real* __restrict__ cb = p_copy ? p_copy + (size_t)b * n : nullptr;
    const bool al = (n & 3) == 0 && (reinterpret_cast<size_t>(pb) & 15) == 0 && (!cb || (reinterpret_cast<size_t>(cb) & 15) == 0);
    const int n4 = al ? n >> 2 : 0;
    for (int i = blockIdx.x * blockDim.x + threadIdx.x; i < n4; i += gridDim.x * blockDim.x) {
        fg_real4 v = reinterpret_cast<fg_real4*>(pb)[i];
        v.x -= mean; v.y -= mean; v.z -= mean; v.w -= mean;
        reinterpret_cast<fg_real4*>(pb)[i] = v;
        if (cb) reinterpret_cast<fg_real4*>(cb)[i] = v;
    }
    for (int i = n4 * 4 + blockIdx.x * blockDim.x + threadIdx.x; i < n; i += gridDim.x * blockDim.x) {
        const fg_real v = pb[i] - mean;
        pb[i] = v;
        if (cb) cb[i] = v;
    }
}

template <int DIMS>
__global__ __launch_bounds__(FG_BLOCK) void k_outflow(FgGrid g, int face, fg_real velm_axis, const fg_real* __restrict__ dt,
                                                       const fg_real* __restrict__ vel, fg_real* __restrict__ bvel,
                                                       const fg_real* __restrict__ scal, fg_real* __restrict__ bscal,
                                                       int n_scalars) {
    const int b = blockIdx.y;
    const fg_real dtb = dt[b];
    if (!(dtb > 0.f)) return;
    const int ax = face >> 1;
    const int slab_n = fg_slab_size(g, ax);
    const int edge = (face & 1) ? ((ax == 0) ? g.nx - 1 : (ax == 1) ? g.ny - 1 : g.nz - 1) : 0;
    const fg_real tcoef = 1.f - 1.f / (1.f + 2.f * dtb * velm_axis * g.rh[ax][edge]);
    const size_t N = g.n;
    for (int s = blockIdx.x * blockDim.x + threadIdx.x; s < slab_n; s += gridDim.x * blockDim.x) {
        int i, j, k;
        if (ax == 0) { i = edge; j = s % g.ny; k = s / g.ny; }
        else if (ax == 1) { j = edge; i = s % g.nx; k = s / g.nx; }
        else { k = edge; i = s % g.nx; j = s / g.nx; }
        const size_t cell = ((size_t)k * g.ny + j) * g.nx + i;
#pragma unroll
        for (int q = 0; q < DIMS; ++q) {
            fg_real* pb = bvel + ((size_t)b * DIMS + q) * slab_n + s;
            const fg_real vb = *pb;
            *pb = vb - tcoef * (vb - vel[((size_t)b * DIMS + q) * N + cell]);
        }
        for (int ch = 0; ch < n_scalars; ++ch) {
            fg_real* pb = bscal + ((size_t)b * n_scalars + ch) * slab_n + s;
            const fg_real sb = *pb;
            *pb = sb - tcoef * (sb - scal[((size_t)b * n_scalars + ch) * N + cell]);
        }
    }
}

struct FgOutflowFold {
    int dt_n; fg_real dt_v[64]; fg_real* dt_out;
    int mask;
    fg_real velm[3];
    const fg_real* vel; const fg_real* scal;
    fg_real* bscal[6]; int nsc[6];
};
struct FgBvelRw { fg_real* p[6]; };
template <int DIMS>
__global__ __launch_bounds__(FG_BLOCK) void k_balance_fluxes(FgGrid g, FgBounds bnd, FgBvelRw bvel_rw_, int free_mask,
                                                              fg_real atol, const fg_real* __restrict__ dt, FgOutflowFold fold) {
    const int b = blockIdx.x;
    const fg_real dtb = fold.dt_n ? fold.dt_v[b] : (dt ? dt[b] : (fg_real)1);
    if (fold.dt_n && threadIdx.x == 0) fold.dt_out[b] = dtb;
    if ((dt || fold.dt_n) && !(dtb > 0.f)) return;
    if (fold.mask) {
        for (int face = 0; face < 2 * DIMS; ++face) {
            if (!((fold.mask >> face) & 1)) continue;
            const int ax = face >> 1;
            const int slab_n = fg_slab_size(g, ax);
            const int edge = (face & 1) ? ((ax == 0) ? g.nx - 1 : (ax == 1) ? g.ny - 1 : g.nz - 1) : 0;
            const fg_real tcoef = 1.f - 1.f / (1.f + 2.f * dtb * fold.velm[ax] * g.rh[ax][edge]);
            const size_t N = g.n;
            fg_real* bvel = bvel_rw_.p[face];
            for (int s = threadIdx.x; s < slab_n; s += blockDim.x) {
                int i, j, k;
                if (ax == 0) { i = edge; j = s % g.ny; k = s / g.ny; }
                else if (ax == 1) { j = edge; i = s % g.nx; k = s / g.nx; }
                else { k = edge; i = s % g.nx; j = s / g.nx; }
                const size_t cell = ((size_t)k * g.ny + j) * g.nx + i;
#pragma unroll
                for (int q = 0; q < DIMS; ++q) {
                    fg_real* pb = bvel + ((size_t)b * DIMS + q) * slab_n + s;
                    const fg_real vb = *pb;
                    *pb = vb - tcoef * (vb - fold.vel[((size_t)b * DIMS + q) * N + cell]);
                }
                for (int ch = 0; ch < fold.nsc[face]; ++ch) {
                    fg_real* pb = fold.bscal[face] + ((size_t)b * fold.nsc[face] + ch) * slab_n + s;
                    const fg_real sb = *pb;
                    *pb = sb - tcoef * (sb - fold.scal[((size_t)b * fold.nsc[face] + ch) * N + cell]);
                }
            }
        }
        __syncthreads();
    }
    double fixed = 0.0, freef = 0.0;
    for (int f = 0; f < 2 * DIMS; ++f) {
        if (!g.fixed[f]) continue;
        const int ax = f >> 1;
        const int slab_n = fg_slab_size(g, ax);
        const double sgn = (f & 1) ? 1.0 : -1.0;
        double acc = 0.0;
        for (int s = threadIdx.x; s < slab_n; s += blockDim.x) {
            int i = 0, j = 0, k = 0;
            if (ax == 0) { j = s % g.ny; k = s / g.ny; }
            else if (ax == 1) { i = s % g.nx; k = s / g.nx; }
            else { i = s % g.nx; j = s / g.nx; }
            fg_real area;
            if (ax == 0) area = g.h[1][j] * (DIMS == 3 ? g.h[2][k] : 1.f);
            else if (ax == 1) area = g.h[0][i] * (DIMS == 3 ? g.h[2][k] : 1.f);
            else area = g.h[0][i] * g.h[1][j];
            acc += sgn * (double)(bnd.vel[f][((size_t)b * DIMS + ax) * slab_n + s] * area);
        }
        if ((free_mask >> f) & 1) freef += acc; else fixed += acc;
    }
    __shared__ double lds[8];
#pragma unroll
    for (int o = 32; o > 0; o >>= 1) { fixed += __shfl_down(fixed, o, 64); freef += __shfl_down(freef, o, 64); }
    if ((threadIdx.x & 63) == 0) { lds[threadIdx.x >> 6] = fixed; lds[4 + (threadIdx.x >> 6)] = freef; }
    __syncthreads();
    fixed = lds[0] + lds[1] + lds[2] + lds[3];
    freef = lds[4] + lds[5] + lds[6] + lds[7];
    if (!(fabs(fixed + freef) > (double)atol)) return;
    const fg_real scale = (fg_real)(-fixed / freef);
    for (int f = 0; f < 2 * DIMS; ++f) {
        if (!((free_mask >> f) & 1) || !g.fixed[f]) continue;
        const int slab_n = fg_slab_size(g, f >> 1);
        fg_real* v = bvel_rw_.p[f] + (size_t)b * DIMS * slab_n;
        for (int s = threadIdx.x; s < DIMS * slab_n; s += blockDim.x) v[s] *= scale;
    }
}

inline unsigned fg_reduce_wgs(const fg_state* s) {
    if (s->reduce_wgs > 0) return (unsigned)s->reduce_wgs;
    const unsigned per_env = (512 + s->grid.B - 1) / s->grid.B;
    return per_env < 8 ? 8 : (per_env > 64 ? 64 : per_env);
}

inline dim3 stride_grid(const fg_state* s, long per_env_elems) {
    long blocks = (per_env_elems / 4 + FG_BLOCK - 1) / FG_BLOCK;
    const long cap = (2048 + s->grid.B - 1) / s->grid.B;
    if (blocks > cap) blocks = cap;
    if (blocks < 1) blocks = 1;
    return dim3((unsigned)blocks, (unsigned)s->grid.B, 1);
}

}


int fg_launch_adv_build(fg_state* s, const FgBounds& bnd, const FgAdvArgs& a_in, hipStream_t st) {
    FgAdvArgs a = a_in;
    a.begin.acc = s->acc; a.begin.sc = s->scratch_B + 4 * s->grid.B; a.begin.flags = s->flags; a.begin.info = s->info_dev;
    a.begin.nc = a.for_scalar ? 1 : s->grid.dims;
    s->prepared.set_bicg(a.begin.nc, a.dt);
    const double nd = (double)s->grid.n;
    const int slot = fg_prof_slot(s, FG_PK_ADV_BUILD, nullptr, s->grid.B, (s->grid.dims == 3 ? 56.0 : 44.0) * nd, 30.0 * nd, st);
    FG_DISPATCH(s, {
        const FgLaunch L = fg_launch_geometry<DIMS, VEC>(s->grid);
        if (a.for_scalar)
            FG_LAUNCH_P(s, slot, (k_adv_build<DIMS, VEC, true>), L.grid, dim3(FG_BLOCK), 0, st, s->grid, bnd, a, L.tiles_x,
                        L.tiles_y, L.tiles);
        else if (a.visc)
            FG_LAUNCH_P(s, slot, (k_adv_build<DIMS, VEC, false, true>), L.grid, dim3(FG_BLOCK), 0, st, s->grid, bnd, a, L.tiles_x,
                        L.tiles_y, L.tiles);
        else
            FG_LAUNCH_P(s, slot, (k_adv_build<DIMS, VEC, false>), L.grid, dim3(FG_BLOCK), 0, st, s->grid, bnd, a, L.tiles_x,
                        L.tiles_y, L.tiles);
    });
    FG_HIP_CHECK(hipGetLastError());
    return FG_OK;
}

template <int DIMS>
__global__ __launch_bounds__(FG_BLOCK) void k_sgs_smagorinsky(FgGrid g, FgBounds bnd, const fg_real* __restrict__ vel, fg_real coefficient,
                                                               fg_real* __restrict__ out) {
    const int b = blockIdx.y, c = blockIdx.x * FG_BLOCK + threadIdx.x;
    if (c >= g.n) return;
    const int ext[3] = {g.nx, g.ny, DIMS == 3 ? g.nz : 1};
    const int pos[3] = {c % g.nx, (c / g.nx) % g.ny, c / (g.nx * g.ny)};
    const int stride[3] = {1, g.nx, g.nx * g.ny};
    const fg_real* u = vel + (size_t)b * DIMS * g.n;
    fg_real grad[DIMS][DIMS];
    fg_real delta = 0.f;
#pragma unroll
    for (int a = 0; a < DIMS; ++a) {
        const fg_real h = g.h[a][pos[a]];
        delta = FG_FMAX(delta, h * h);
        fg_real dist = 2.f;
        fg_real diff[DIMS];
#pragma unroll
        for (int q = 0; q < DIMS; ++q) diff[q] = 0.f;
#pragma unroll
        for (int up = 0; up < 2; ++up) {
            const int f = 2 * a + up;
            const bool at = up ? (pos[a] + 1 == ext[a]) : (pos[a] == 0);
            if (at && g.fixed[f]) {
                int si = 0, mul = 1;
#pragma unroll
                for (int t = 0; t < DIMS; ++t) if (t != a) { si += pos[t] * mul; mul *= ext[t]; }
                const fg_real* bv = bnd.vel[f] + (size_t)b * DIMS * mul;
#pragma unroll
                for (int q = 0; q < DIMS; ++q) diff[q] += (up ? 1.f : -1.f) * bv[q * mul + si];
                dist -= 0.5f;
            } else {
                const int n = at ? (up ? c - (ext[a] - 1) * stride[a] : c + (ext[a] - 1) * stride[a]) : (up ? c + stride[a] : c - stride[a]);
#pragma unroll
                for (int q = 0; q < DIMS; ++q) diff[q] += (up ? 1.f : -1.f) * u[(size_t)q * g.n + n];
            }
        }
#pragma unroll
        for (int q = 0; q < DIMS; ++q) grad[q][a] = diff[q] / dist * g.rh[a][pos[a]];
    }
    fg_real d = 0.f;
#pragma unroll
// ... 17 lines not shown
    for (int idx = threadIdx.x; idx < rows * g.nx; idx += blockDim.x) {
        const int k = idx / g.nx, i = idx - k * g.nx;
        lo += (double)u[((size_t)k * g.ny + 0) * g.nx + i];
        hi += (double)u[((size_t)k * g.ny + (g.ny - 1)) * g.nx + i];
    }
    __shared__ double lds[2][16];
#pragma unroll
    for (int o = 32; o > 0; o >>= 1) { lo += __shfl_down(lo, o, 64); hi += __shfl_down(hi, o, 64); }
    if ((threadIdx.x & 63) == 0) { lds[0][threadIdx.x >> 6] = lo; lds[1][threadIdx.x >> 6] = hi; }
    __syncthreads();
    if (threadIdx.x == 0) {
        double sl = 0.0, sh = 0.0;
        for (int w = 0; w < (int)(blockDim.x >> 6); ++w) { sl += lds[0][w]; sh += lds[1][w]; }
        const double n = (double)rows * g.nx;
        const fg_real tau_lo = coef_lo * (fg_real)(sl / n), tau_hi = coef_hi * (fg_real)(sh / n);
        for (int q = 0; q < dims; ++q) force[b * dims + q] = (q == axis) ? (fg_real)0.5 * (tau_lo + tau_hi) : (fg_real)0;
    }
}

int fg_launch_wall_forcing(const fg_state* s, hipStream_t st) {
    hipLaunchKernelGGL(k_wall_forcing, dim3(s->grid.B), dim3(1024), 0, st, s->grid, (const fg_real*)s->velocity, s->wall_forcing_axis,
                       s->wall_forcing_coef[0], s->wall_forcing_coef[1], s->force_uniform, s->grid.dims);
    FG_HIP_CHECK(hipGetLastError());
    return FG_OK;
}

int fg_launch_sgs(const fg_state* s, const FgBounds& bnd, fg_real coefficient, fg_real* out, hipStream_t st) {
    const dim3 grid((s->grid.n + FG_BLOCK - 1) / FG_BLOCK, s->grid.B);
    if (s->grid.dims == 2) hipLaunchKernelGGL(k_sgs_smagorinsky<2>, grid, dim3(FG_BLOCK), 0, st, s->grid, bnd, (const fg_real*)s->velocity, coefficient, out);
    else hipLaunchKernelGGL(k_sgs_smagorinsky<3>, grid, dim3(FG_BLOCK), 0, st, s->grid, bnd, (const fg_real*)s->velocity, coefficient, out);
    FG_HIP_CHECK(hipGetLastError());
    return FG_OK;
}

int fg_launch_pressure_setup(const fg_state* s, const fg_real* dt, hipStream_t st) {
    const int n = s->grid.n;
    hipLaunchKernelGGL(k_reciprocal, stride_grid(s, n), dim3(FG_BLOCK), 0, st, s->A, s->rA, dt, n, (n % 4 == 0) ? n / 4 : 0);
    FG_HIP_CHECK(hipGetLastError());
    return FG_OK;
}

int fg_launch_h(fg_state* s, const fg_real* dt, const fg_real* vel_result, hipStream_t st) {
    fg_htrace("h_launch_in");
    FgCgBegin begin;
    begin.acc = s->cg_acc; begin.flags = s->flags; begin.info = s->info_dev; begin.mean_sums = s->acc; begin.best = s->cg_best;
    begin.track_best = s->cg_return_best; begin.ns = fg_cg_slots(s); begin.xsum = s->fcg_xsum;
    s->prepared.set_cg(begin.ns, begin.track_best, dt);
    const int slot_h = fg_prof_slot(s, FG_PK_H, nullptr, s->grid.B, (s->grid.dims == 3 ? 68.0 : 52.0) * (double)s->grid.n, 6.0 * s->grid.dims * s->grid.dims * (double)s->grid.n, st);
    FG_DISPATCH(s, {
        const FgLaunch L = fg_launch_geometry<DIMS, VEC>(s->grid);
        FG_LAUNCH_P(s, slot_h, (k_h<DIMS, VEC>), L.grid, dim3(FG_BLOCK), 0, st, s->grid, dt, s->rA, s->Coff, s->adv_rhs,
                    vel_result, s->hvec, begin, L.tiles_x, L.tiles_y, L.tiles);
    });
    FG_HIP_CHECK(hipGetLastError());
    fg_htrace("h_launch_out");
    return FG_OK;
}

int fg_launch_div(fg_state* s, const FgBounds& bnd, const fg_real* dt, const fg_real* hvec, fg_real* div,
                  hipStream_t st, bool cg_from_zero, bool fused_fwd) {
    FgCgStart start = {nullptr, nullptr, nullptr, 1};
    s->prepared.set_cg_start(0);
    if (cg_from_zero && dt != nullptr && s->prepared.cg_for(dt) && div == s->div) {
#if !FG_F64
        if (fused_fwd && fg_fcg_ok(s)) {
            s->prepared.set_cg_start(2);
            return fg_fcg_div_fwd(s, bnd, dt, hvec, div, s->prepared.cg_ns, st);
        }
#endif
        start.acc = s->cg_acc; start.r = s->w[0]; start.x = s->p_result; start.ns = s->prepared.cg_ns;
        s->prepared.set_cg_start(1);
    }
    const int slot_d = fg_prof_slot(s, FG_PK_DIV, nullptr, s->grid.B, 28.0 * (double)s->grid.n, 4.0 * s->grid.dims * (double)s->grid.n, st);
    FG_DISPATCH(s, {
        const FgLaunch L = fg_launch_geometry<DIMS, VEC>(s->grid);
        FG_LAUNCH_P(s, slot_d, (k_div<DIMS, VEC>), L.grid, dim3(FG_BLOCK), 0, st, s->grid, bnd, dt, hvec, div, start, L.tiles_x,
                    L.tiles_y, L.tiles);
    });
    FG_HIP_CHECK(hipGetLastError());
    return FG_OK;
}

int fg_launch_correct(const fg_state* s, const fg_real* dt, const fg_real* rA, const fg_real* hvec, const fg_real* p,
                      fg_real* vel_out, hipStream_t st, fg_real* vel_copy, const FgMeanRef* mean, const FgLazyRef* lazy) {
    fg_htrace("correct_in");
    const FgMeanRef mr = mean ? *mean : FgMeanRef{nullptr, nullptr, nullptr, nullptr, nullptr};
    const FgLazyRef lz = lazy ? *lazy : FgLazyRef{nullptr, nullptr, nullptr};
    const double cb = (s->grid.dims == 3 ? 36.0 : 28.0) + (vel_copy ? 4.0 * s->grid.dims : 0.0) + ((mean && mean->sums) || (lazy && lazy->p_res) ? 4.0 : 0.0);
    const int slot_c = fg_prof_slot(s, FG_PK_CORRECT, nullptr, s->grid.B, cb * (double)s->grid.n, 5.0 * s->grid.dims * (double)s->grid.n, st);
    FG_DISPATCH(s, {
        const FgLaunch L = fg_launch_geometry<DIMS, VEC>(s->grid);
        FG_LAUNCH_P(s, slot_c, (k_correct<DIMS, VEC>), L.grid, dim3(FG_BLOCK), 0, st, s->grid, dt, rA, hvec, p, vel_out, vel_copy, mr, lz,
                    L.tiles_x, L.tiles_y, L.tiles);
    });
    FG_HIP_CHECK(hipGetLastError());
    fg_htrace("correct_out");
    return FG_OK;
}

int fg_launch_max_velocity(const fg_state* s, const FgBounds& bnd, fg_real* out_B, hipStream_t st, fg_real* mirror_B, FgPollOut poll,
                           fg_real* flux_B, fg_real* flux_mirror, FgDtRule rule) {
    FG_REQUIRE(!rule.t_rem || (poll.gran && mirror_B && !FG_F64), FG_ERR_INVALID_ARG, "the device-side sub-step rule needs the result-word form");
    FG_REQUIRE(!flux_B || (mirror_B && flux_mirror), FG_ERR_INVALID_ARG, "the flux balance rides in the mirrored form only");
    int32_t* done_B = reinterpret_cast<int32_t*>(out_B + s->grid.B);
    FG_REQUIRE(!mirror_B || out_B == s->scratch_B + s->grid.B, FG_ERR_INVALID_ARG, "mirror needs the scratch row as out_B");
    if (!mirror_B || !s->maxvel_clean)
        FG_HIP_CHECK(hipMemsetAsync(out_B, 0, mirror_B ? sizeof(fg_real) * s->grid.B + sizeof(int32_t) * (s->grid.B + 1) : sizeof(fg_real) * s->grid.B, st));
    s->maxvel_clean = mirror_B ? 1 : 0;
    if ((s->grid.nx & 3) == 0) {
        const int rows = s->grid.ny * s->grid.nz;
        int rpb = 4;
        while ((long)((rows + 2 * rpb - 1) / (2 * rpb)) * s->grid.B >= 2048) rpb *= 2;
        while ((rows + rpb - 1) / rpb > (int)fg_reduce_wgs(s)) rpb *= 2;
        dim3 grid((rows + rpb - 1) / rpb, s->grid.B);
        const int slot_m = fg_prof_slot(s, FG_PK_MAXVEL, nullptr, s->grid.B, 4.0 * s->grid.dims * (double)s->grid.n, 2.0 * s->grid.dims * (double)s->grid.n, st);
        if (s->grid.dims == 2)
            FG_LAUNCH_P(s, slot_m, k_max_velocity_rows<2>, grid, dim3(FG_BLOCK), 0, st, s->grid, bnd, s->velocity, out_B, done_B,
                        mirror_B, rpb, poll, flux_B, flux_mirror, rule);
        else
            FG_LAUNCH_P(s, slot_m, k_max_velocity_rows<3>, grid, dim3(FG_BLOCK), 0, st, s->grid, bnd, s->velocity, out_B, done_B,
                        mirror_B, rpb, poll, flux_B, flux_mirror, rule);
        FG_HIP_CHECK(hipGetLastError());
        return FG_OK;
    }
    dim3 grid = stride_grid(s, (long)s->grid.n * 4);
    if (s->grid.dims == 2)
        hipLaunchKernelGGL(k_max_velocity<2>, grid, dim3(FG_BLOCK), 0, st, s->grid, bnd, s->velocity, out_B, done_B, mirror_B, poll, flux_B, flux_mirror, rule);
    else
        hipLaunchKernelGGL(k_max_velocity<3>, grid, dim3(FG_BLOCK), 0, st, s->grid, bnd, s->velocity, out_B, done_B, mirror_B, poll, flux_B, flux_mirror, rule);
    FG_HIP_CHECK(hipGetLastError());
    return FG_OK;
}

int fg_launch_flux_balance(const fg_state* s, const FgBounds& bnd, fg_real* out_B, hipStream_t st, FgPollOut poll) {
    if (s->grid.dims == 2)
        hipLaunchKernelGGL(k_flux_balance<2>, dim3(s->grid.B), dim3(FG_BLOCK), 0, st, s->grid, bnd, out_B, poll);
    else
        hipLaunchKernelGGL(k_flux_balance<3>, dim3(s->grid.B), dim3(FG_BLOCK), 0, st, s->grid, bnd, out_B, poll);
    FG_HIP_CHECK(hipGetLastError());
    return FG_OK;
}

int fg_launch_copy_active(const fg_state* s, const fg_real* dt, const fg_real* src, fg_real* dst, int comps,
                          hipStream_t st) {
    const long per_env = (long)comps * s->grid.n;
    hipLaunchKernelGGL(k_copy_active, stride_grid(s, per_env), dim3(FG_BLOCK), 0, st, dt, src, dst, per_env);
    FG_HIP_CHECK(hipGetLastError());
    return FG_OK;
}

int fg_launch_buoyancy(const fg_state* s, const fg_real* dt, const fg_real* T, long t_env_stride, fg_real* source, int axis,
                       fg_real factor, hipStream_t st) {
    hipLaunchKernelGGL(k_buoyancy, stride_grid(s, (long)s->grid.n * 4), dim3(FG_BLOCK), 0, st, dt, T, t_env_stride,
                       source, s->grid.dims, s->grid.n, axis, factor);
    FG_HIP_CHECK(hipGetLastError());
    return FG_OK;
}

int fg_launch_mean_sub(const fg_state* s, const fg_real* dt, fg_real* p, fg_real* p_copy, hipStream_t st) {
    FgDacc* sums = s->acc;
    dim3 grid = stride_grid(s, (long)s->grid.n * 4);
    dim3 rgrid(grid.x > fg_reduce_wgs(s) ? fg_reduce_wgs(s) : grid.x, grid.y);
    hipLaunchKernelGGL(k_sum_env, rgrid, dim3(FG_BLOCK), 0, st, dt, p, sums, s->grid.n);
    hipLaunchKernelGGL(k_sub_mean, grid, dim3(FG_BLOCK), 0, st, dt, p, p_copy, sums, s->grid.n);
    FG_HIP_CHECK(hipGetLastError());
    return FG_OK;
}

int fg_launch_outflow(const fg_state* s, int face, fg_real velm_axis, const fg_real* dt, hipStream_t st) {
    const int slab_n = (face >> 1) == 0 ? s->grid.ny * s->grid.nz : (face >> 1) == 1 ? s->grid.nx * s->grid.nz : s->grid.nx * s->grid.ny;
    dim3 grid((slab_n + FG_BLOCK - 1) / FG_BLOCK, s->grid.B);
    const int nsc = (s->scalar && s->bscal[face]) ? s->cfg.n_scalars : 0;
    if (s->grid.dims == 2)
        hipLaunchKernelGGL(k_outflow<2>, grid, dim3(FG_BLOCK), 0, st, s->grid, face, velm_axis, dt, s->velocity, s->bvel[face],
                           s->scalar, s->bscal[face], nsc);
    else
        hipLaunchKernelGGL(k_outflow<3>, grid, dim3(FG_BLOCK), 0, st, s->grid, face, velm_axis, dt, s->velocity, s->bvel[face],
                           s->scalar, s->bscal[face], nsc);
    FG_HIP_CHECK(hipGetLastError());
    return FG_OK;
}

int fg_launch_balance(const fg_state* s, const FgBounds& bnd, int free_mask, fg_real atol, const fg_real* dt, hipStream_t st,
                      int outflow_mask, const fg_real* outflow_velm, const fg_real* dt_host_values) {
    FgOutflowFold fold;
    fold = FgOutflowFold{};
    if (dt_host_values) {
        fold.dt_n = s->grid.B; fold.dt_out = s->dt_dev;
        for (int b = 0; b < s->grid.B; ++b) fold.dt_v[b] = dt_host_values[b];
    }
    if (outflow_mask) {
        fold.mask = outflow_mask; fold.vel = s->velocity; fold.scal = s->scalar;
        for (int a = 0; a < 3; ++a) fold.velm[a] = outflow_velm[a];
        for (int f = 0; f < 6; ++f) { fold.bscal[f] = s->bscal[f]; fold.nsc[f] = (s->scalar && s->bscal[f]) ? s->cfg.n_scalars : 0; }
    }
    FgBvelRw rw;
    for (int f = 0; f < 6; ++f) rw.p[f] = s->bvel[f];
    if (s->grid.dims == 2)
        hipLaunchKernelGGL(k_balance_fluxes<2>, dim3(s->grid.B), dim3(FG_BLOCK), 0, st, s->grid, bnd, rw, free_mask, atol, dt, fold);
    else
        hipLaunchKernelGGL(k_balance_fluxes<3>, dim3(s->grid.B), dim3(FG_BLOCK), 0, st, s->grid, bnd, rw, free_mask, atol, dt, fold);
    FG_HIP_CHECK(hipGetLastError());
    return FG_OK;
}

bool fg_outflow_folds(const fg_state* s, int outflow_mask) {
    for (int f = 0; f < 2 * s->grid.dims; ++f) {
        if (!((outflow_mask >> f) & 1)) continue;
        const int ax = f >> 1;
        const long slab_n = ax == 0 ? (long)s->grid.ny * s->grid.nz : ax == 1 ? (long)s->grid.nx * s->grid.nz : (long)s->grid.nx * s->grid.ny;
        if (slab_n > 4 * FG_BLOCK) return false;
    }
    return outflow_mask != 0;
}
```

fluidgym_amd/native.py:

```python
from __future__ import annotations

import ctypes
import os
from typing import Dict, List, Optional, Sequence

import numpy as np
import torch

from . import _lib as L


def _ptr(t: Optional[torch.Tensor]):
    return None if t is None else ctypes.c_void_p(t.data_ptr())


def _stream(device) -> ctypes.c_void_p:
    return ctypes.c_void_p(torch.cuda.current_stream(device).cuda_stream)


class LinsolveError(RuntimeError):
    """A linear solve failed (reference: ``PISOtorch_diff.LinsolveError``, PISOtorch_diff.py:262)."""


class NativeSolver:
# ... 326 lines not shown
                    sched[6 * k + int(face)] = base + k * step_bytes
        out = (ctypes.c_int32 * (6 * n))()
        flux = (self._c_real * self.B)()
        done = ctypes.c_int32(0)
        rc = self.lib.fg_multi_step(self.handle, ctypes.byref(o), int(n), sched, out, flux, ctypes.byref(done), _stream(self.device))
        if boundary_schedule:
            for face, t in boundary_schedule.items():
                self.bvel[int(face)] = t[max(min(done.value, n - 1), 0)]
        self.last_multi_results = [(bool(out[6 * k + 5]), [int(out[6 * k + i]) for i in range(4)], int(out[6 * k + 4])) for k in range(min(done.value, n))]
        if rc == L.FG_ERR_FLUX_BALANCE:
            raise RuntimeError(
                "Domain boundary fluxes not balanced, cannot proceed with simulation step. "
                f"Flux balance: {list(flux)}, flux_balance_tol: {kw.get('flux_balance_tol', 1e-5)}")
        if rc == L.FG_ERR_NOT_FINITE:
            raise LinsolveError("linear solve produced a non-finite residual")
        L.check(rc)
        return self.last_multi_results

    def set_pressure_refinement(self, max_corrections: int = 3, target_tol: float = 1e-10, inner_relative_tol: float = 1e-4):
        L.check(self.lib.fg_set_pressure_refinement(self.handle, int(max_corrections), self._c_real(target_tol), self._c_real(inner_relative_tol)), lib=self.lib)

    def solver_hints(self, values=None):
        buf = (ctypes.c_int32 * 12)(*([0] * 12 if values is None else [int(v) for v in values]))
        L.check(self.lib.fg_solver_hints(self.handle, buf, 0 if values is None else 1), lib=self.lib)
        return list(buf)

    def reset_solver_state(self):
        L.check(self.lib.fg_reset_solver_state(self.handle, _stream(self.device)), lib=self.lib)

    def env_restore_field(self, which_field: int, bank: torch.Tensor, sel, signed_components: bool = False):
        assert bank.is_cuda and bank.dtype == self.dtype and bank.is_contiguous(), f"a bank is a contiguous {self.dtype} CUDA tensor"
        self._env_sel = sel
        L.check(self.lib.fg_env_restore_field(self.handle, int(which_field), _ptr(bank), int(bank.shape[0]), sel, len(sel),
                                              int(bool(signed_components)), _stream(self.device)), lib=self.lib)

    def env_reset_solver_state(self, sel):
        self._env_sel = sel
        L.check(self.lib.fg_env_reset_solver_state(self.handle, sel, len(sel), _stream(self.device)), lib=self.lib)

    def make_divergence_free(self, tol=1e-5, max_iterations=1000):
        info = self._infos(self.B)
        rc = self.lib.fg_make_divergence_free(self.handle, tol, max_iterations, info, _stream(self.device))
        L.check(rc, allow=(L.FG_ERR_NOT_CONVERGED,))
        return list(info)

    def poisson_apply(self, rA, x, y=None):
        y = torch.empty_like(x) if y is None else y
        L.check(self.lib.fg_poisson_apply(self.handle, _ptr(rA), _ptr(x), _ptr(y), _stream(self.device)), lib=self.lib)
        return y

    def poisson_jacobi(self, rA, b, x, sweeps, omega=1.0):
        L.check(self.lib.fg_poisson_jacobi(self.handle, _ptr(rA), _ptr(b), _ptr(x), sweeps, omega, _stream(self.device)), lib=self.lib)
        return x

    def poisson_rbgs(self, rA, b, x, sweeps, omega=1.0):
        L.check(self.lib.fg_poisson_rbgs(self.handle, _ptr(rA), _ptr(b), _ptr(x), sweeps, omega, _stream(self.device)), lib=self.lib)
        return x

    def poisson_cg(self, rA, b, x, tol=1e-5, max_iterations=5000, use_x0=False):
        info = self._infos(self.B)
        rc = self.lib.fg_poisson_cg(self.handle, _ptr(rA), _ptr(b), _ptr(x), tol, max_iterations, int(use_x0), info,
                                    _stream(self.device))
        L.check(rc, allow=(L.FG_ERR_NOT_CONVERGED, L.FG_ERR_NOT_FINITE))
        return list(info)


    def solver_counters(self, reset: bool = False) -> dict:
        unconv = (ctypes.c_int64 * 4)()
        L.check(self.lib.fg_solver_unconverged(self.handle, unconv))
        out = (ctypes.c_int64 * 13)()
        L.check(self.lib.fg_solver_counters(self.handle, out, int(reset)), lib=self.lib)
        names = ("scalar", "velocity", "pressure0", "pressure1")
        res = {n: {"mean": (out[k] / out[4 + k]) if out[4 + k] else None, "max": int(out[8 + k]), "systems": int(out[4 + k]),
                    "unconverged": int(unconv[k])}
               for k, n in enumerate(names)}
        res["piso_steps"] = int(out[12])
        return res

    def config_dump(self) -> dict:
        out = L.read_json(self.lib.fg_config_dump, self.handle, lib=self.lib)
        out["env"] = {k: v for k, v in sorted(os.environ.items()) if k.startswith(("FG_", "FLUIDGYM_"))}
        return out

    def set_return_best(self, on: bool = True):
        L.check(self.lib.fg_set_return_best(self.handle, int(on)), lib=self.lib)

    def set_cg_reset_steps(self, steps: int = 100):
        L.check(self.lib.fg_set_cg_reset_steps(self.handle, int(steps)), lib=self.lib)

    def set_advection_start(self, from_result: bool = True):
        L.check(self.lib.fg_set_advection_start(self.handle, int(from_result)), lib=self.lib)

    def set_wall_stress_forcing(self, axis: int, coef_lo: float = 0.0, coef_hi: float = 0.0) -> None:
        L.check(self.lib.fg_set_wall_stress_forcing(self.handle, int(axis), float(coef_lo), float(coef_hi)), lib=self.lib)

    def set_advection_preconditioner(self, mode: int = 0):
        L.check(self.lib.fg_set_advection_preconditioner(self.handle, int(mode)), lib=self.lib)

    def apply_advection_preconditioner(self, mode: int, r: torch.Tensor, return_forms: bool = False):
        r = r.to(self.device, self.dtype).contiguous()
        z = torch.empty_like(r)
        forms = (ctypes.c_int32 * L.FG_FORM_SLOTS)()
        L.check(self.lib.fg_debug_apply_preconditioner(self.handle, int(mode), int(r.shape[1]), ctypes.c_void_p(r.data_ptr()),
                                                       ctypes.c_void_p(z.data_ptr()), forms, _stream(self.device)), lib=self.lib)
        return (z, list(forms)) if return_forms else z

    def apply_pressure_preconditioner(self, form: int, r: torch.Tensor, rA: Optional[torch.Tensor] = None):
        r = r.to(self.device, self.dtype).contiguous()
        z = torch.empty_like(r)
        ra = ctypes.c_void_p(None) if rA is None else ctypes.c_void_p(rA.data_ptr())
        rz = (ctypes.c_double * self.B)()
        forms = (ctypes.c_int32 * L.FG_FORM_SLOTS)()
        L.check(self.lib.fg_debug_apply_pressure_preconditioner(self.handle, int(form), ra, ctypes.c_void_p(r.data_ptr()),
                                                                ctypes.c_void_p(z.data_ptr()), rz, forms, _stream(self.device)),
                lib=self.lib)
        return z, list(rz), list(forms)

    def advection_retries(self, reset: bool = False) -> int:
        out = ctypes.c_int64()
        L.check(self.lib.fg_advection_retries(self.handle, ctypes.byref(out), int(reset)), lib=self.lib)
        return int(out.value)

    def set_double_fallback(self, on: bool = True) -> None:
        L.check(self.lib.fg_set_double_fallback(self.handle, int(bool(on))), lib=self.lib)

    def set_advection_jacobi(self, on: bool = True) -> None:
        L.check(self.lib.fg_set_advection_jacobi(self.handle, int(bool(on))), lib=self.lib)

    def advection_jacobi_counts(self) -> Dict[str, int]:
        out = (ctypes.c_int64 * 2)()
        L.check(self.lib.fg_advection_jacobi_counts(self.handle, out), lib=self.lib)
        return {"settled_by_sweeps": int(out[0]), "handed_to_bicgstab": int(out[1])}

    def ladder(self, force_mask: int = -1) -> Dict[str, int]:
        out = (ctypes.c_int64 * 4)()
        L.check(self.lib.fg_ladder(self.handle, out, int(force_mask)), lib=self.lib)
        return {"advection_fp64": int(out[0]), "advection_preconditioned": int(out[1]), "pressure_fp64": int(out[2])}

    def advection_solver_form(self, nc: Optional[int] = None) -> str:
        out = ctypes.c_int32()
        L.check(self.lib.fg_advection_solver_form(self.handle, int(self.dims if nc is None else nc), ctypes.byref(out)), lib=self.lib)
        return ("five", "two-brick", "two-zmarch")[out.value]

    def profile_enable(self, on: bool = True):
        L.check(self.lib.fg_profile_enable(self.handle, int(on)), lib=self.lib)

    def profile_read(self):
        out = {}
        for k in range(self.lib.fg_profile_kinds()):
            ms, by, fl, fms, fby, ams = (ctypes.c_double() for _ in range(6))
            n, fn, nl, an = (ctypes.c_int64() for _ in range(4))
            L.check(self.lib.fg_profile_read(self.handle, k, ctypes.byref(ms), ctypes.byref(n), ctypes.byref(by),
                                             ctypes.byref(fl), ctypes.byref(fms), ctypes.byref(fby), ctypes.byref(fn),
                                             ctypes.byref(nl), ctypes.byref(ams), ctypes.byref(an)))
            out[self.lib.fg_profile_kind_name(k).decode()] = dict(
                ms=ms.value, samples=n.value, bytes=by.value, flops=fl.value, full_ms=fms.value,
                full_bytes=fby.value, full_samples=fn.value, launches=nl.value, all_ms=ams.value,
                all_samples=an.value)
        return out

    def poisson_fdcg(self, rA, b, x, tol=1e-5, max_iterations=500, use_x0=False):
        info = self._infos(self.B)
        rc = self.lib.fg_poisson_fdcg(self.handle, _ptr(rA), _ptr(b), _ptr(x), tol, max_iterations, int(use_x0), info,
                                      _stream(self.device))
        L.check(rc, allow=(L.FG_ERR_NOT_CONVERGED, L.FG_ERR_NOT_FINITE))
        return list(info)
# ... 26 lines not shown
```

include/fluidgym_hip.h:

```cpp
#ifndef FLUIDGYM_HIP_H
#define FLUIDGYM_HIP_H

#include <stdint.h>

#ifdef __cplusplus
extern "C" {
#endif

#define FG_ABI_VERSION 1

#ifdef FG_REAL_DOUBLE
typedef double fg_real;
#else
typedef float fg_real;
#endif
#define FG_MAX_SCALARS 4

#define FG_OK 0
#define FG_ERR_INVALID_ARG (-1)
#define FG_ERR_NOT_BOUND (-2)
#define FG_ERR_HIP (-3)
#define FG_ERR_UNSUPPORTED (-4)
#define FG_ERR_NOT_CONVERGED (-5)
#define FG_ERR_NOT_FINITE (-6)
// ... 344 lines not shown
    int64_t bvel_stride, bvel_comp_stride;
} fg_mb_point_mesh;
int fg_mb_point_locate(const fg_mb_point_mesh* mesh, const fg_real* points, int64_t points_env_stride, int32_t n_points,
                       const int32_t* start_cell, int32_t max_walk, int32_t* cell_out, fg_real* xi_out, int32_t* status_out, void* stream);
int fg_mb_point_sample(const fg_mb_point_mesh* mesh, const fg_real* const* extra, const int64_t* extra_stride, int32_t n_extra,
                       const int32_t* cell, const fg_real* xi, int64_t cell_env_stride, int32_t n_points, fg_real* out, void* stream);
int fg_mb_tracer_advect(const fg_mb_point_mesh* mesh, fg_real dt, int32_t substeps, const uint8_t* respawn_slots, const fg_real* seed_pos,
                        const int32_t* seed_cell, fg_real* pos, int32_t* cell, fg_real* age, int32_t* wraps, uint32_t* lost,
                        int32_t n_tracers, void* stream);

int fg_envglue_jet_schedule(const float* target, const float* current, const float* decay, const float* shape, int32_t n,
                            int32_t batch, int32_t nx, float* jets, float* last, void* stream);
int fg_envglue_channel_observe(const float* velocity, const float* pressure, const int64_t* sensor, int32_t n_sensors,
                               int32_t batch, int32_t ny, int32_t nx, float shear_scale, float penalty, float* obs_velocity,
                               float* obs_pressure, float* cross, float* shear, float* reward, void* stream);
int fg_envglue_channel_observe_batch(const float* velocity, const float* pressure, const int64_t* sensor, int32_t n_sensors,
                                     int32_t batch, int32_t ny, int32_t nx, const float* shear_scale_B, float penalty,
                                     float* obs_velocity, float* obs_pressure, float* cross, float* shear, float* reward,
                                     void* stream);

typedef struct fg_mb_state* fg_mb_handle;
int fg_mb_create(int32_t dims, int32_t batch, int32_t device, fg_mb_handle* out);
int fg_mb_destroy(fg_mb_handle h);
int fg_mb_add_block(fg_mb_handle h, const fg_real* vertex_coords_host, int32_t nx, int32_t ny, int32_t nz, int32_t* block_id);
int fg_mb_connect(fg_mb_handle h, int32_t block1, int32_t face1, int32_t block2, int32_t face2, int32_t axis1, int32_t axis2);
int fg_mb_make_periodic(fg_mb_handle h, int32_t block, int32_t axis);
int fg_mb_set_reference_quirks(fg_mb_handle h, int32_t connected_diagonal_offset, int32_t first_layer_rule);
int fg_mb_set_nonortho_flags(fg_mb_handle h, int32_t flags);
int fg_mb_finalize(fg_mb_handle h);
int fg_mb_sizes(fg_mb_handle h, int32_t* n_cells, int32_t* n_boundary_faces);
int fg_mb_block_info(fg_mb_handle h, int32_t block, int32_t* cell_offset, int32_t* boundary_slot0 );
int fg_mb_get_neighbors(fg_mb_handle h, int32_t* out_host );
int fg_mb_get_host_table(fg_mb_handle h, int32_t which, void* out, int64_t* count);
int fg_mb_bind(fg_mb_handle h, fg_real* velocity, fg_real* pressure_result, fg_real* boundary_velocity, const fg_real* source);
int fg_mb_set_viscosity(fg_mb_handle h, fg_real nu);
int fg_mb_set_viscosity_batch(fg_mb_handle h, const fg_real* nu_B);
typedef struct fg_mb_step_options {
    int32_t corrector_steps;
    int32_t advect_non_ortho_steps;
    int32_t pressure_non_ortho_steps;
    int32_t max_iterations;
    fg_real advection_tol;
    fg_real pressure_tol;
    int32_t pressure_use_bicgstab;
    int32_t pressure_warm_start;
    int32_t pressure_project_mean;
    fg_real pressure_stall_accept;
    int32_t solver_double_fallback;
    int32_t bicg_precondition_fallback;
} fg_mb_step_options;
int fg_mb_piso_step(fg_mb_handle h, const fg_real* dt_B, const fg_mb_step_options* opt, int32_t* stats_host, void* stream);
int fg_mb_env_status(fg_mb_handle h, int32_t* out_B_host);
int fg_mb_ladder(fg_mb_handle h, int64_t* out4_host, int32_t force_mask);
int fg_mb_debug_cycles(fg_mb_handle h, uint64_t* out12_host);
int fg_mb_solver_hints(fg_mb_handle h, int32_t* hints48, int32_t set);
int fg_mb_env_restore_field(fg_mb_handle h, int which_field, const fg_real* bank, int32_t S, const fg_env_sel* sel, int32_t n_sel,
                            int32_t signed_components, void* stream);
int fg_mb_env_reset_solver_state(fg_mb_handle h, const fg_env_sel* sel, int32_t n_sel, void* stream);
typedef struct fg_mb_reset_noise {
    uint64_t seed;
    double sigma_velocity, sigma_pressure;
    const uint32_t* episodes;
} fg_mb_reset_noise;
int fg_mb_restore_envs(fg_mb_handle h, const fg_real* bank_velocity , const fg_real* bank_pressure ,
                       const fg_real* bank_boundary , int32_t S, const fg_env_sel* sel,
                       int32_t n_sel, const fg_mb_reset_noise* noise , void* stream);
typedef struct fg_mb_inflow_params {
    int32_t slot0, count;
    int32_t outflow_slot0, outflow_count, outflow_slot0_b, outflow_count_b;
    int32_t n_streamwise, n_transverse;
    int32_t sim_steps, k;
    int32_t env_offset, reserved;
    uint64_t seed;
    double dt, f_lo, f_hi, streamwise_rms, transverse_rms, kappa, y_mid, outflow_tol;
    const void* base;
    const double* y;
    const double* modes;
    const uint32_t* counters;
    float* signal;
} fg_mb_inflow_params;
int fg_mb_inflow_disturbance(fg_mb_handle h, const fg_mb_inflow_params* params, void* stream);
int fg_mb_solver_counters(fg_mb_handle h, int64_t* out13_host, int32_t reset);
int fg_config_dump(fg_handle h, char* buf, int n);
int fg_mb_config_dump(fg_mb_handle h, char* buf, int n);
int fg_switch_values(int32_t family, char* buf, int32_t n);
int fg_mb_solver_unconverged(fg_mb_handle h, int64_t* out4_host);
typedef struct fg_mb_sim_options {
    fg_mb_step_options step;
    fg_real time_step;
    fg_real cfl;
    int32_t adaptive;
    int32_t substeps;
    fg_real flux_balance_tol;
    int32_t outflow_slot0;
    int32_t outflow_count;
    fg_real outflow_velm[3];
    fg_real outflow_tol;
    int32_t max_substeps;
    int32_t outflow_slot0_b;
    int32_t outflow_count_b;
} fg_mb_sim_options;
int fg_mb_single_step(fg_mb_handle h, const fg_mb_sim_options* opt, int32_t* out_host, fg_real* flux_host, void* stream);
int fg_mb_update_advective_boundary(fg_mb_handle h, fg_real dt, int32_t slot0, int32_t count, int32_t slot0_b, int32_t count_b,
                                    const fg_real* velm, fg_real tol, void* stream);
int fg_mb_make_divergence_free(fg_mb_handle h, const fg_mb_step_options* opt, void* stream);
int fg_mb_boundary_flux_balance(fg_mb_handle h, fg_real* out_B_host, void* stream);
int fg_mb_get_boundary_tables(fg_mb_handle h, int32_t* cell, int32_t* face, fg_real* transform);
int fg_mb_get_cell_transforms(fg_mb_handle h, fg_real* transform);
int fg_mb_max_velocity(fg_mb_handle h, fg_real* out_B_host, void* stream);
int fg_mb_flow_diagnostic(fg_mb_handle h, int kind, fg_real* out, void* stream);
int fg_mb_set_residual_projection(fg_mb_handle h, const fg_real* y_host);
int fg_mb_set_stall_limit(fg_mb_handle h, int32_t iterations);
int fg_mb_set_advection_start(fg_mb_handle h, int from_result);
int fg_mb_set_advection_jacobi(fg_mb_handle h, int on);
int fg_mb_advection_jacobi_counts(fg_mb_handle h, int64_t* out2);
int fg_mb_set_multilevel(fg_mb_handle h, int32_t n4, int32_t n8, const int32_t* a4_host, const int32_t* parent4_host,
                         const int32_t* rect4_host , const fg_real* d4g_host,
                         const fg_real* aci8_host, fg_real geom_diag_sum, int32_t enable);
int fg_mb_debug_bicgstab(fg_mb_handle h, fg_real tol, int32_t max_iterations, int32_t reps, int64_t* out4,
                         double* acc_out , fg_real* sc_out , void* stream);
int fg_mb_multilevel_apply(fg_mb_handle h, const fg_real* r_BN, fg_real* z_BN, void* stream);
int fg_mb_debug_pressure_cg(fg_mb_handle h, fg_real tol, int32_t max_iterations, int32_t project_mean, int32_t* iterations_B,
                            int32_t* converged_B, double* residual_B, void* stream);
int fg_mb_debug_ilu_apply(fg_mb_handle h, const fg_real* r_BdN, fg_real* z_BdN, void* stream);
int fg_mb_multilevel_status(fg_mb_handle h, int32_t* out3);
int fg_mb_wall_forces(fg_mb_handle h, const int32_t* cell_index, const int32_t* slot_index, const fg_real* geom, int32_t n,
                      int32_t layers, fg_real area_scale, fg_real viscosity, fg_real* out, void* stream);
int fg_mb_wall_forces_batch(fg_mb_handle h, const int32_t* cell_index, const int32_t* slot_index, const fg_real* geom, int32_t n,
                            int32_t layers, fg_real area_scale, fg_real viscosity, const fg_real* viscosity_B, fg_real* out,
                            void* stream);
int fg_mb_unit_pressure_matrix(fg_mb_handle h, void* stream);
int fg_mb_profile_enable(fg_mb_handle h, int32_t on);
const char* fg_mb_profile_kind_name(int32_t kind);
int fg_mb_profile_read(fg_mb_handle h, int32_t kind, double* ms_sum, int64_t* samples, double* bytes_sum, int64_t* launches);
int fg_mb_profile_iterations(fg_mb_handle h, int64_t* iterations);
#define FG_MB_BUF_A 0
#define FG_MB_BUF_C_OFF 1
#define FG_MB_BUF_RHS 2
#define FG_MB_BUF_H 3
#define FG_MB_BUF_DIV 4
#define FG_MB_BUF_P_DIAG 5
#define FG_MB_BUF_P_OFF 6
#define FG_MB_BUF_VELOCITY_RESULT 7
#define FG_MB_BUF_KRYLOV0 8
#define FG_MB_BUF_PRESSURE_X 13
int fg_mb_get_buffer(fg_mb_handle h, int32_t which, const fg_real** ptr, int64_t* count);
int fg_mb_read_buffer(fg_mb_handle h, int32_t which, fg_real* dst_device, void* stream);

int fg_coords_to_transforms(const float* coords, float* transforms, int dims, int nx, int ny, int nz,
                            void* stream);

#ifdef __cplusplus
}
#endif
#endif
```

Baseline: 10330 env-steps/s.

## Carry per-tile velocity maxima from corrector into fused next-step head kernel

```diff
diff --git a/fluidgym_amd/_lib.py b/fluidgym_amd/_lib.py
--- a/fluidgym_amd/_lib.py
+++ b/fluidgym_amd/_lib.py
@@ -404,6 +404,7 @@
     "fg_mb_destroy": (c_int, [c_void_p]),
     "fg_config_dump": (c_int, [c_void_p, ctypes.c_char_p, c_int]),
     "fg_mb_config_dump": (c_int, [c_void_p, ctypes.c_char_p, c_int]),
+    "fg_last_cfl_maxima": (c_int, [c_void_p, c_void_p]),
     "fg_switch_values": (c_int, [c_int32, ctypes.c_char_p, c_int32]),
     "fg_mb_add_block": (c_int, [c_void_p, POINTER(c_float), c_int32, c_int32, c_int32, POINTER(c_int32)]),
     "fg_mb_connect": (c_int, [c_void_p, c_int32, c_int32, c_int32, c_int32, c_int32, c_int32]),
diff --git a/fluidgym_amd/csrc/fg_api.hip b/fluidgym_amd/csrc/fg_api.hip
--- a/fluidgym_amd/csrc/fg_api.hip
+++ b/fluidgym_amd/csrc/fg_api.hip
@@ -112,6 +112,8 @@
 #if !FG_F64
     FG_HIP_CHECK(hipMalloc(&s->t_rem_dev, sizeof(double) * g.B));
     FG_HIP_CHECK(hipMemset(s->t_rem_dev, 0, sizeof(double) * g.B));
+    FG_DISPATCH(s, { s->tile_max_tiles = fg_launch_geometry<DIMS, VEC>(g).tiles; });
+    FG_HIP_CHECK(alloc(&s->tile_max, (size_t)g.B * s->tile_max_tiles));
 #endif
     if (int rc = fg_poll_create(&s->poll, (int)(nsys > 2 * (size_t)g.B ? nsys : 2 * (size_t)g.B))) return rc;
     for (int k = 0; k < 4; ++k) { s->pred_bicg[k] = 2; s->pred_cg[k] = 1; }
@@ -152,7 +154,7 @@
     (void)hipHostFree(s->info_pinned); (void)hipHostFree(s->flags_pinned);
     fg_prof_destroy(s);
     fg_poll_destroy(&s->poll);
-    (void)hipFree(s->d_bvel_ptrs); (void)hipHostFree(s->diag_pinned); (void)hipHostFree(s->dt_pinned); (void)hipFree(s->dt_dev); (void)hipFree(s->t_rem_dev); (void)hipFree(s->env_sel_dev);
+    (void)hipFree(s->d_bvel_ptrs); (void)hipHostFree(s->diag_pinned); (void)hipHostFree(s->dt_pinned); (void)hipFree(s->dt_dev); (void)hipFree(s->t_rem_dev); (void)hipFree(s->tile_max); (void)hipFree(s->env_sel_dev);
     float* fd[] = {s->fd_Qx, s->fd_QxT, s->fd_Qz, s->fd_QzT, s->fd_lower, s->fd_inv, s->fd_cp};
     for (float* p : fd) if (p) (void)hipFree(p);
     if (s->fd_dct_tw) { (void)hipFree(s->fd_dct_tw); (void)hipFree(s->fd_dct_rot); }
@@ -541,7 +543,7 @@
                          c->opt->pressure_method == FG_SOLVER_FDCG && s->fd_Qx != nullptr);
 }
 
-static int launch_corrector(fg_state* s, const fg_real* dt, const FgCgOutcome& o, bool last, hipStream_t st) {
+static int launch_corrector(fg_state* s, const fg_real* dt, const FgCgOutcome& o, bool last, hipStream_t st, bool* tiles_left = nullptr) {
     const bool mean_folded = last && o.mean_ready;
     FG_REQUIRE(!o.lazy_z || !last || mean_folded, FG_ERR_UNSUPPORTED, "fg_piso_step: an unmaterialised pressure without its folded mean");
     if (last && !mean_folded)
@@ -549,13 +551,17 @@
     const FgMeanRef mean = {s->fcg_xsum, s->info_dev, s->pressure, o.marks_valid ? s->fcg_lazy : nullptr, s->fcg_alpha};
     const FgLazyRef lazy = {s->fcg_lazy, s->fcg_alpha, last ? s->p_result : nullptr};
     const fg_real* p = o.lazy_z ? o.lazy_z : ((last && !mean_folded) ? s->pressure : s->p_result);
-    return fg_launch_correct(s, dt, s->rA, s->hvec, p, s->vel_result, st, last ? s->velocity : nullptr, mean_folded ? &mean : nullptr, o.lazy_z ? &lazy : nullptr);
-}
-
-struct SpecCorrect { fg_state* s; const fg_real* dt; bool last; hipStream_t st; };
+    fg_real* tile_max = (last && tiles_left) ? s->tile_max : nullptr;
+    if (int rc = fg_launch_correct(s, dt, s->rA, s->hvec, p, s->vel_result, st, last ? s->velocity : nullptr, mean_folded ? &mean : nullptr, o.lazy_z ? &lazy : nullptr, tile_max))
+        return rc;
+    if (tile_max) *tiles_left = true;
+    return FG_OK;
+}
+
+struct SpecCorrect { fg_state* s; const fg_real* dt; bool last; hipStream_t st; bool* tiles_left; };
 static int spec_correct(void* p, const FgCgOutcome& o) {
     const SpecCorrect* c = static_cast<const SpecCorrect*>(p);
-    return launch_corrector(c->s, c->dt, o, c->last, c->st);
+    return launch_corrector(c->s, c->dt, o, c->last, c->st, c->tiles_left);
 }
 
 static int solve_pressure(fg_state* s, const fg_real* dt, int method, fg_real tol, int max_iterations, int use_previous,
@@ -668,8 +674,15 @@
     return rc;
 }
 
+static int piso_step(fg_handle s, const fg_real* dt_B, const fg_step_options* opt, int32_t* stats_host, void* stream, bool* tiles_left);
 extern "C" int fg_piso_step(fg_handle s, const fg_real* dt_B, const fg_step_options* opt, int32_t* stats_host,
                             void* stream) {
+    return piso_step(s, dt_B, opt, stats_host, stream, nullptr);
+}
+static int piso_step(fg_handle s, const fg_real* dt_B, const fg_step_options* opt, int32_t* stats_host, void* stream, bool* tiles_left) {
+    if (tiles_left) *tiles_left = false;
+    bool tiles_now = false;
+    bool* const tiles_arg = (tiles_left && s && s->tile_max) ? &tiles_now : nullptr;
     FG_REQUIRE(s && dt_B && opt, FG_ERR_INVALID_ARG, "null argument");
     const bool scalar = opt->advect_scalar && s->cfg.n_scalars > 0;
     if (int rc = check_bound(s, scalar)) return rc;
@@ -739,19 +752,21 @@
                                        opt->pressure_method == FG_SOLVER_FDCG && s->fd_Qx != nullptr))
                 return rc;
         }
-        SpecCorrect spec_ctx = {s, dt_B, last, st};
+        tiles_now = false;
+        SpecCorrect spec_ctx = {s, dt_B, last, st, tiles_arg};
         FgCgOutcome outcome;
         if (int rc = soft(solve_pressure(s, dt_B, opt->pressure_method, opt->pressure_tol, opt->max_iterations, opt->pressure_warm_start ? 1 : 0,
                                          info.data(), st, false, c == 0 ? 0 : 1, &outcome, FgCgSpec{spec_correct, &spec_ctx})))
             return rc;
         if (c < 2) { stats[2 + c] = max_iters(info.data(), B); s->ctr.add(2 + c, info.data(), B); }
         if (!outcome.spec_done)
-            if (int rc = launch_corrector(s, dt_B, outcome, last, st)) return rc;
+            if (int rc = launch_corrector(s, dt_B, outcome, last, st, tiles_arg)) return rc;
     }
     if (opt->corrector_steps <= 0)
         if (int rc = fg_launch_copy_active(s, dt_B, s->vel_result, s->velocity, d, st)) return rc;
     if (stats_host) memcpy(stats_host, stats, sizeof(stats));
     s->ctr.piso_steps += 1;
+    if (tiles_left) *tiles_left = opt->corrector_steps > 0 && tiles_now;
     return status;
 }
 
@@ -763,7 +778,8 @@
         {"fast_transform_x", s->fd_dct_x}, {"fd_preconditioner", s->fd_Qx ? 1 : 0}, {"helmholtz", s->fd_lam ? 1 : 0}, {"advection_preconditioner", s->adv_precond},
         {"advection_from_result", s->adv_from_result}, {"return_best", s->cg_return_best}, {"cg_reset_steps", s->cg_reset_steps}, {"double_fallback", s->double_fallback},
         {"wall_forcing_axis", s->wall_forcing_axis}, {"first_iterate_polls", s->fcg_first_polls}, {"unstored_pressure_solves", s->fcg_unstored},
-        {"jacobi_speculation_misses", s->jac_spec_missed}, {"jacobi_floor_released", s->jac_floor_released}, {"pressure_refinement_corrections", s->ref64_corrections}};
+        {"jacobi_speculation_misses", s->jac_spec_missed}, {"jacobi_floor_released", s->jac_floor_released}, {"pressure_refinement_corrections", s->ref64_corrections},
+        {"step_heads_carried", s->step_heads_carried}};
     for (const auto& kv : state) fg_json_put(out, kv.first, kv.second);
     return fg_json_out(out + "}", buf, n);
 }
@@ -781,17 +797,18 @@
     return FG_OK;
 }
 
-extern "C" int fg_single_step(fg_handle s, const fg_sim_options* o, int32_t* out, fg_real* flux_host, void* stream);
+static int single_step(fg_handle s, const fg_sim_options* o, int32_t* out, fg_real* flux_host, void* stream, bool* carried);
 extern "C" int fg_multi_step(fg_handle s, const fg_sim_options* o, int32_t n, const fg_real* const* bvel_schedule, int32_t* out_6n,
                              fg_real* flux_host, int32_t* steps_done, void* stream) {
     FG_REQUIRE(s && o && out_6n && n >= 0, FG_ERR_INVALID_ARG, "fg_multi_step: bad argument");
     if (steps_done) *steps_done = 0;
+    bool carried = false;
     for (int k = 0; k < n; ++k) {
         if (bvel_schedule)
             for (int f = 0; f < 2 * s->grid.dims; ++f)
                 if (const fg_real* p = bvel_schedule[(size_t)k * 6 + f])
                     if (int rc = fg_bind(s, FG_BOUND_VELOCITY + f, const_cast<fg_real*>(p))) return rc;
-        if (int rc = fg_single_step(s, o, out_6n + 6 * (size_t)k, flux_host, stream)) return rc;
+        if (int rc = single_step(s, o, out_6n + 6 * (size_t)k, flux_host, stream, &carried)) return rc;
         if (steps_done) *steps_done = k + 1;
         if (out_6n[6 * (size_t)k + 5] == 0 && !s->cg_return_best) break;
     }
@@ -801,6 +818,20 @@
 static inline bool is_close_zero(double a) { return std::fabs(a) <= 1e-8; }
 
 extern "C" int fg_single_step(fg_handle s, const fg_sim_options* o, int32_t* out, fg_real* flux_host, void* stream) {
+    bool carried = false;
+    return single_step(s, o, out, flux_host, stream, &carried);
+}
+
+extern "C" int fg_last_cfl_maxima(fg_handle s, fg_real* out_B) {
+    FG_REQUIRE(s && out_B && s->diag_pinned, FG_ERR_INVALID_ARG, "fg_last_cfl_maxima: bad argument");
+    for (int b = 0; b < s->grid.B; ++b) out_B[b] = s->diag_pinned[s->grid.B + b];
+    return FG_OK;
+}
+
+static int single_step(fg_handle s, const fg_sim_options* o, int32_t* out, fg_real* flux_host, void* stream, bool* carried) {
+    const bool carried_in = *carried;
+    *carried = false;
+    bool tiles_valid = carried_in;
     fg_htrace("single_step_in");
     FgRange range_sim("fg_single_step");
     FG_REQUIRE(s && o && out, FG_ERR_INVALID_ARG, "null argument");
@@ -849,6 +880,10 @@
             }
             return FG_OK;
         };
+        const bool folded = o->outflow_mask && fg_outflow_folds(s, o->outflow_mask);
+        bool head = false;
+        const bool tiles_in = tiles_valid;
+        tiles_valid = false;
         bool deferred = false;
         FgPollOut po_cfl = FgPollOut{nullptr, 0};
         if (o->adaptive || first) {
@@ -859,8 +894,15 @@
                 deferred = po.gran != nullptr && s->dev_dt && s->t_rem_dev != nullptr;
                 const FgDtRule rule = deferred ? FgDtRule{s->t_rem_dev, s->dt_dev, (float)o->cfl, (double)o->time_step, first ? 1 : 0}
                                                : FgDtRule{nullptr, nullptr, 0.f, 0.0, 0};
-                if (int rc = fg_launch_max_velocity(s, bnd, s->scratch_B + B, st, s->diag_pinned + B, po.seq ? FgPollOut{po.seq + B, po.value, po.gran} : po,
-                                                    first ? s->scratch_B : nullptr, first ? s->diag_pinned : nullptr, rule))
+                head = deferred && tiles_in && fg_step_head_applies(s) && (!o->outflow_mask || folded);
+                if (head) {
+                    const fg_real velm3[3] = {o->outflow_velm[0], o->outflow_velm[1], o->outflow_velm[2]};
+                    if (int rc = fg_launch_step_head(s, bnd, st, FgPollOut{po.seq + B, po.value, po.gran}, first, rule, o->outflow_mask,
+                                                     (fg_real)0.01 * o->outflow_tol, velm3))
+                        return rc;
+                    s->step_heads_carried += 1;
+                } else if (int rc = fg_launch_max_velocity(s, bnd, s->scratch_B + B, st, s->diag_pinned + B, po.seq ? FgPollOut{po.seq + B, po.value, po.gran} : po,
+                                                           first ? s->scratch_B : nullptr, first ? s->diag_pinned : nullptr, rule))
                     return rc;
             }
             fg_htrace("maxvel_launched");
@@ -878,10 +920,9 @@
         }
         if (!deferred)
             for (int b = 0; b < B; ++b) s->dt_pinned[b] = advance(b, o->adaptive ? s->diag_pinned[B + b] : (fg_real)0);
-        const bool folded = o->outflow_mask && fg_outflow_folds(s, o->outflow_mask);
         const bool dt_by_value = folded && B <= 64 && !deferred;
         if (!dt_by_value && !deferred) FG_HIP_CHECK(hipMemcpyAsync(s->dt_dev, s->dt_pinned, sizeof(fg_real) * B, hipMemcpyHostToDevice, st));
-        if (o->outflow_mask) {
+        if (o->outflow_mask && !head) {
             for (int f = 0; f < 2 * s->grid.dims; ++f)
                 if ((o->outflow_mask >> f) & 1) FG_REQUIRE(s->grid.fixed[f], FG_ERR_INVALID_ARG, "outflow face is not FIXED");
             if (!folded)
@@ -893,7 +934,7 @@
                                            dt_by_value ? s->dt_pinned : nullptr))
                 return rc;
         }
-        int rc = fg_piso_step(s, s->dt_dev, &o->step, stats, stream);
+        int rc = piso_step(s, s->dt_dev, &o->step, stats, stream, &tiles_valid);
         if (rc == FG_ERR_NOT_CONVERGED) all_ok = 0;
         else if (rc != FG_OK) return rc;
         if (deferred) {
@@ -911,6 +952,7 @@
         if (substeps >= (o->max_substeps > 0 ? o->max_substeps : 100000)) break;
     }
     fg_htrace("single_step_out");
+    *carried = tiles_valid;
     for (int i = 0; i < 4; ++i) out[i] = stats[i];
     out[4] = substeps;
     out[5] = all_ok;
diff --git a/fluidgym_amd/csrc/fg_internal.h b/fluidgym_amd/csrc/fg_internal.h
--- a/fluidgym_amd/csrc/fg_internal.h
+++ b/fluidgym_amd/csrc/fg_internal.h
@@ -668,6 +668,8 @@
     fg_real* dt_pinned;
     fg_real* dt_dev;
     double* t_rem_dev;
+    fg_real* tile_max; int tile_max_tiles;
+    long long step_heads_carried;
     int pred_bicg[4], pred_cg[4];
     int adv_jacobi, adv_jacobi_env; FgJacHist jac_hist[4]; float* jac_prev;
     long long jac_solves, jac_fallbacks;
@@ -765,7 +767,8 @@
 struct FgMeanRef { const FgDacc* sums; const fg_solve_info* info; fg_real* p_copy; const int32_t* lazy; const double* alpha; };
 struct FgLazyRef { const int32_t* lazy; const double* alpha; fg_real* p_res; };
 int fg_launch_correct(const fg_state* s, const fg_real* dt, const fg_real* rA, const fg_real* hvec, const fg_real* p,
-                      fg_real* vel_out, hipStream_t st, fg_real* vel_copy = nullptr, const FgMeanRef* mean = nullptr, const FgLazyRef* lazy = nullptr);
+                      fg_real* vel_out, hipStream_t st, fg_real* vel_copy = nullptr, const FgMeanRef* mean = nullptr, const FgLazyRef* lazy = nullptr,
+                      fg_real* tile_max = nullptr);
 struct FgDtRule { double* t_rem; fg_real* dt_out; float cfl; double time_step; int reset; };
 int fg_launch_max_velocity(const fg_state* s, const FgBounds& bnd, fg_real* out_B, hipStream_t st, fg_real* mirror_B = nullptr,
                            FgPollOut poll = FgPollOut{nullptr, 0}, fg_real* flux_B = nullptr, fg_real* flux_mirror = nullptr,
@@ -779,6 +782,9 @@
                       int outflow_mask = 0, const fg_real* outflow_velm = nullptr,
                       const fg_real* dt_host_values = nullptr);
 bool fg_outflow_folds(const fg_state* s, int outflow_mask);
+bool fg_step_head_applies(const fg_state* s);
+int fg_launch_step_head(const fg_state* s, const FgBounds& bnd, hipStream_t st, FgPollOut poll, bool first, FgDtRule rule, int outflow_mask,
+                        fg_real atol, const fg_real* outflow_velm);
 int fg_launch_mean_sub(const fg_state* s, const fg_real* active_dt, fg_real* p, fg_real* p_copy, hipStream_t st);
 
 int fg_poisson_apply_launch(const fg_state* s, const fg_real* rA, const fg_real* x, fg_real* y, hipStream_t st);
diff --git a/fluidgym_amd/csrc/fg_piso.hip b/fluidgym_amd/csrc/fg_piso.hip
--- a/fluidgym_amd/csrc/fg_piso.hip
+++ b/fluidgym_amd/csrc/fg_piso.hip
@@ -292,61 +292,81 @@
     }
 }
 
-template <int DIMS, int VEC>
+template <int DIMS, int VEC, bool TMAX = false>
 __global__ __launch_bounds__(FG_BLOCK) void k_correct(FgGrid g, const fg_real* __restrict__ dt,
                                                        const fg_real* __restrict__ rA_, const fg_real* __restrict__ hvec,
                                                        const fg_real* __restrict__ p, fg_real* __restrict__ vel_out,
-                                                       fg_real* __restrict__ vel_copy, FgMeanRef mean, FgLazyRef lazy, int tiles_x, int tiles_y, int tiles) {
+                                                       fg_real* __restrict__ vel_copy, FgMeanRef mean, FgLazyRef lazy, fg_real* __restrict__ tile_max,
+                                                       int tiles_x, int tiles_y, int tiles) {
     const FgCtx<DIMS, VEC> c = fg_make_ctx<DIMS, VEC>(g, tiles_x, tiles_y, tiles);
-    if ((dt && !(dt[c.b] > 0.f)) || !c.valid) return;
-    const size_t N = g.n;
-    const FgMetric<DIMS, VEC> m = fg_metrics<DIMS, VEC>(g, c);
-    const FgVec<VEC> rA = fg_load<VEC>(rA_ + (size_t)c.b * N + c.idx);
-    FgNbr<DIMS, VEC> P = fg_gather<DIMS, VEC>(p + (size_t)c.b * N, c);
-    if (lazy.lazy) {
-        const bool on = lazy.lazy[c.b] == 1;
-        const fg_real sc = on ? (fg_real)lazy.alpha[2 * c.b] : (fg_real)0;
-        auto scale = [&](FgVec<VEC>& v) {
-#pragma unroll
-            for (int e = 0; e < VEC; ++e) v.v[e] = on ? sc * v.v[e] : (fg_real)0;
-        };
-        scale(P.c); scale(P.xm); scale(P.xp); scale(P.ym); scale(P.yp);
-        if constexpr (DIMS == 3) { scale(P.zm); scale(P.zp); }
-        if (lazy.p_res) fg_store<VEC>(lazy.p_res + (size_t)c.b * N + c.idx, P.c);
-    }
-    if (mean.sums) {
-        const int used = mean.info[c.b].used_iterations;
-        const bool first_only = mean.lazy && mean.lazy[c.b] == 1;
-        const fg_real mu = first_only ? (fg_real)(mean.alpha[2 * c.b] * acc_ld(mean.sums + (2 * c.b + 1)) / (double)g.n)
-                           : used < 0 ? (fg_real)0 : (fg_real)(acc_ld(mean.sums + (2 * c.b + (used & 1))) / (double)g.n);
-        FgVec<VEC> pc;
-#pragma unroll
-        for (int e = 0; e < VEC; ++e) pc.v[e] = P.c.v[e] - mu;
-        fg_store<VEC>(mean.p_copy + (size_t)c.b * N + c.idx, pc);
-    }
-#pragma unroll
-    for (int q = 0; q < DIMS; ++q) {
-        const size_t base = ((size_t)c.b * DIMS + q) * N;
-        const FgVec<VEC> h = fg_load<VEC>(hvec + base + c.idx);
-        FgVec<VEC> out;
-#pragma unroll
-        for (int e = 0; e < VEC; ++e) {
-            fg_real lo, hi, fac, rh;
-            if (q == 0) {
-                lo = P.xm.v[e]; hi = P.xp.v[e]; rh = m.rhx[e];
-                const fg_real ml = (e == 0) ? c.mxm : 1.f, mh = (e == VEC - 1) ? c.mxp : 1.f;
-                fac = (ml == 0.f || mh == 0.f) ? 1.f : 0.5f;
-            } else if (q == 1) {
-                lo = P.ym.v[e]; hi = P.yp.v[e]; rh = m.rhy;
-                fac = (c.mym == 0.f || c.myp == 0.f) ? 1.f : 0.5f;
-            } else {
-                lo = P.zm.v[e]; hi = P.zp.v[e]; rh = m.rhz;
-                fac = (c.mzm == 0.f || c.mzp == 0.f) ? 1.f : 0.5f;
+    if (dt && !(dt[c.b] > 0.f)) return;
+    if (!c.valid && !TMAX) return;
+    fg_real mx = 0.f;
+    if (c.valid) {
+        const size_t N = g.n;
+        const FgMetric<DIMS, VEC> m = fg_metrics<DIMS, VEC>(g, c);
+        const FgVec<VEC> rA = fg_load<VEC>(rA_ + (size_t)c.b * N + c.idx);
+        FgNbr<DIMS, VEC> P = fg_gather<DIMS, VEC>(p + (size_t)c.b * N, c);
+        if (lazy.lazy) {
+            const bool on = lazy.lazy[c.b] == 1;
+            const fg_real sc = on ? (fg_real)lazy.alpha[2 * c.b] : (fg_real)0;
+            auto scale = [&](FgVec<VEC>& v) {
+#pragma unroll
+                for (int e = 0; e < VEC; ++e) v.v[e] = on ? sc * v.v[e] : (fg_real)0;
+            };
+            scale(P.c); scale(P.xm); scale(P.xp); scale(P.ym); scale(P.yp);
+            if constexpr (DIMS == 3) { scale(P.zm); scale(P.zp); }
+            if (lazy.p_res) fg_store<VEC>(lazy.p_res + (size_t)c.b * N + c.idx, P.c);
+        }
+        if (mean.sums) {
+            const int used = mean.info[c.b].used_iterations;
+            const bool first_only = mean.lazy && mean.lazy[c.b] == 1;
+            const fg_real mu = first_only ? (fg_real)(mean.alpha[2 * c.b] * acc_ld(mean.sums + (2 * c.b + 1)) / (double)g.n)
+                               : used < 0 ? (fg_real)0 : (fg_real)(acc_ld(mean.sums + (2 * c.b + (used & 1))) / (double)g.n);
+            FgVec<VEC> pc;
+#pragma unroll
+            for (int e = 0; e < VEC; ++e) pc.v[e] = P.c.v[e] - mu;
+            fg_store<VEC>(mean.p_copy + (size_t)c.b * N + c.idx, pc);
+        }
+#pragma unroll
+        for (int q = 0; q < DIMS; ++q) {
+            const size_t base = ((size_t)c.b * DIMS + q) * N;
+            const FgVec<VEC> h = fg_load<VEC>(hvec + base + c.idx);
+            FgVec<VEC> out;
+#pragma unroll
+            for (int e = 0; e < VEC; ++e) {
+                fg_real lo, hi, fac, rh;
+                if (q == 0) {
+                    lo = P.xm.v[e]; hi = P.xp.v[e]; rh = m.rhx[e];
+                    const fg_real ml = (e == 0) ? c.mxm : 1.f, mh = (e == VEC - 1) ? c.mxp : 1.f;
+                    fac = (ml == 0.f || mh == 0.f) ? 1.f : 0.5f;
+                } else if (q == 1) {
+                    lo = P.ym.v[e]; hi = P.yp.v[e]; rh = m.rhy;
+                    fac = (c.mym == 0.f || c.myp == 0.f) ? 1.f : 0.5f;
+                } else {
+                    lo = P.zm.v[e]; hi = P.zp.v[e]; rh = m.rhz;
+                    fac = (c.mzm == 0.f || c.mzp == 0.f) ? 1.f : 0.5f;
+                }
+                out.v[e] = h.v[e] - rA.v[e] * ((hi - lo) * fac * rh);
             }
-            out.v[e] = h.v[e] - rA.v[e] * ((hi - lo) * fac * rh);
-        }
-        fg_store<VEC>(vel_out + base + c.idx, out);
-        if (vel_copy) fg_store<VEC>(vel_copy + base + c.idx, out);
+            fg_store<VEC>(vel_out + base + c.idx, out);
+            if (vel_copy) fg_store<VEC>(vel_copy + base + c.idx, out);
+            if constexpr (TMAX) {
+                const fg_real rhq = (q == 1) ? m.rhy : m.rhz;
+#pragma unroll
+                for (int e = 0; e < VEC; ++e) mx = FG_FMAX(mx, FG_FABS(out.v[e] * ((q == 0) ? m.rhx[e] : rhq)));
+            }
+        }
+    }
+    if constexpr (TMAX) {
+        __shared__ fg_real lds_tm[FG_BLOCK / 64];
+        mx = fg_wave_max(mx);
+        if ((threadIdx.x & 63) == 0) lds_tm[threadIdx.x >> 6] = mx;
+        __syncthreads();
+        if (threadIdx.x == 0) {
+            const unsigned bid = fg_xcd_remap(blockIdx.x, gridDim.x);
+            tile_max[(size_t)c.b * tiles + bid % (unsigned)tiles] = FG_FMAX(FG_FMAX(lds_tm[0], lds_tm[1]), FG_FMAX(lds_tm[2], lds_tm[3]));
+        }
     }
 }
 
@@ -397,6 +417,22 @@
     __syncthreads();
     return lds_fb[0] + lds_fb[1] + lds_fb[2] + lds_fb[3];
 }
+#if !FG_F64
+__device__ __forceinline__ float fg_dt_rule_env(const FgDtRule& rule, int e, fg_bits mbits) {
+    double tr = rule.reset ? rule.time_step : rule.t_rem[e];
+    float ts = 0.f;
+    if (tr > 0.0 && !(fabs(tr) <= 1e-8)) {
+        const double mv = (double)__uint_as_float(mbits);
+        const double max_ts = (fabs(mv) <= 1e-8) ? tr : (double)rule.cfl / mv;
+        const double tsd = (max_ts >= tr) ? tr : tr / (double)(long long)ceil(tr / max_ts);
+        tr -= tsd;
+        ts = (float)tsd;
+    }
+    rule.t_rem[e] = tr;
+    rule.dt_out[e] = ts;
+    return ts;
+}
+#endif
 __device__ __forceinline__ void fg_publish_max(fg_real* out_B, int32_t* done_B, fg_real* mirror_B, int b, fg_real mx, const FgPollOut& poll, int B,
                                                fg_real* flux_B = nullptr, fg_real* flux_mirror = nullptr, const FgDtRule& rule = FgDtRule{nullptr, nullptr, 0.f, 0.0, 0}) {
     const int lane = threadIdx.x & 63;
@@ -420,19 +456,7 @@
         if (poll.gran) {
             for (int e = lane; e < B; e += 64) {
                 const fg_bits mbits = __hip_atomic_exchange(reinterpret_cast<fg_bits*>(out_B) + e, (fg_bits)0, __ATOMIC_RELAXED, __HIP_MEMORY_SCOPE_AGENT);
-                if (rule.t_rem) {
-                    double tr = rule.reset ? rule.time_step : rule.t_rem[e];
-                    float ts = 0.f;
-                    if (tr > 0.0 && !(fabs(tr) <= 1e-8)) {
-                        const double mv = (double)__uint_as_float(mbits);
-                        const double max_ts = (fabs(mv) <= 1e-8) ? tr : (double)rule.cfl / mv;
-                        const double tsd = (max_ts >= tr) ? tr : tr / (double)(long long)ceil(tr / max_ts);
-                        tr -= tsd;
-                        ts = (float)tsd;
-                    }
-                    rule.t_rem[e] = tr;
-                    rule.dt_out[e] = ts;
-                }
+                if (rule.t_rem) fg_dt_rule_env(rule, e, mbits);
                 fg_poll_publish_word(poll, 12 * B + e, mbits);
                 if (flux_B) fg_poll_publish_word(poll, 13 * B + e, __hip_atomic_exchange(reinterpret_cast<fg_bits*>(flux_B) + e, (fg_bits)0, __ATOMIC_RELAXED, __HIP_MEMORY_SCOPE_AGENT));
                 atomicExch(done_B + e, 0);
@@ -691,12 +715,8 @@
 };
 struct FgBvelRw { fg_real* p[6]; };
 template <int DIMS>
-__global__ __launch_bounds__(FG_BLOCK) void k_balance_fluxes(FgGrid g, FgBounds bnd, FgBvelRw bvel_rw_, int free_mask,
-                                                              fg_real atol, const fg_real* __restrict__ dt, FgOutflowFold fold) {
-    const int b = blockIdx.x;
-    const fg_real dtb = fold.dt_n ? fold.dt_v[b] : (dt ? dt[b] : (fg_real)1);
-    if (fold.dt_n && threadIdx.x == 0) fold.dt_out[b] = dtb;
-    if ((dt || fold.dt_n) && !(dtb > 0.f)) return;
+__device__ __forceinline__ void fg_balance_env(const FgGrid& g, const FgBounds& bnd, const FgBvelRw& bvel_rw_, int free_mask, fg_real atol,
+                                               fg_real dtb, const FgOutflowFold& fold, int b) {
     if (fold.mask) {
         for (int face = 0; face < 2 * DIMS; ++face) {
             if (!((fold.mask >> face) & 1)) continue;
@@ -763,6 +783,92 @@
         for (int s = threadIdx.x; s < DIMS * slab_n; s += blockDim.x) v[s] *= scale;
     }
 }
+template <int DIMS>
+__global__ __launch_bounds__(FG_BLOCK) void k_balance_fluxes(FgGrid g, FgBounds bnd, FgBvelRw bvel_rw_, int free_mask,
+                                                              fg_real atol, const fg_real* __restrict__ dt, FgOutflowFold fold) {
+    const int b = blockIdx.x;
+    const fg_real dtb = fold.dt_n ? fold.dt_v[b] : (dt ? dt[b] : (fg_real)1);
+    if (fold.dt_n && threadIdx.x == 0) fold.dt_out[b] = dtb;
+    if ((dt || fold.dt_n) && !(dtb > 0.f)) return;
+    fg_balance_env<DIMS>(g, bnd, bvel_rw_, free_mask, atol, dtb, fold, b);
+}
+
+#if !FG_F64
+constexpr int HEAD_R = 4;
+struct FgHeadArgs {
+    const fg_real* tile_max; int tiles;
+    fg_real* out_B; int32_t* done_B;
+    fg_real* flux_B;
+    FgDtRule rule;
+    int free_mask; fg_real atol;
+};
+template <int DIMS>
+__global__ __launch_bounds__(FG_BLOCK) void k_step_head(FgGrid g, FgBounds bnd, FgBvelRw rw, FgHeadArgs a, FgPollOut poll, FgOutflowFold fold) {
+    const int b = blockIdx.x, B = gridDim.x;
+    const int lane = threadIdx.x & 63, wave = threadIdx.x >> 6;
+    fg_real tm = 0.f;
+    for (int t = threadIdx.x; t < a.tiles; t += FG_BLOCK) tm = FG_FMAX(tm, a.tile_max[(size_t)b * a.tiles + t]);
+    fg_real val[2 * DIMS][HEAD_R][DIMS], rhv[2 * DIMS][HEAD_R][DIMS];
+#pragma unroll
+    for (int f = 0; f < 2 * DIMS; ++f) {
+        const int ax = f >> 1;
+        const int slab_n = fg_slab_size(g, ax);
+        const int edge = (f & 1) ? ((ax == 0) ? g.nx - 1 : (ax == 1) ? g.ny - 1 : g.nz - 1) : 0;
+#pragma unroll
+        for (int r = 0; r < HEAD_R; ++r) {
+            const int s_raw = (int)threadIdx.x + r * FG_BLOCK;
+            const bool ok = g.fixed[f] && s_raw < slab_n;
+            const int s = ok ? s_raw : 0;
+            int i, j, k;
+            if (ax == 0) { i = edge; j = (DIMS == 3) ? s % g.ny : s; k = (DIMS == 3) ? s / g.ny : 0; }
+            else if (ax == 1) { j = edge; i = (DIMS == 3) ? s % g.nx : s; k = (DIMS == 3) ? s / g.nx : 0; }
+            else { k = edge; i = s % g.nx; j = s / g.nx; }
+            rhv[f][r][0] = g.rh[0][i];
+            rhv[f][r][1] = g.rh[1][j];
+            if constexpr (DIMS == 3) rhv[f][r][2] = g.rh[2][k];
+#pragma unroll
+            for (int q = 0; q < DIMS; ++q) val[f][r][q] = ok ? bnd.vel[f][((size_t)b * DIMS + q) * slab_n + s] : (fg_real)0;
+        }
+    }
+    fg_real mx = tm;
+#pragma unroll
+    for (int f = 0; f < 2 * DIMS; ++f)
+#pragma unroll
+        for (int r = 0; r < HEAD_R; ++r)
+#pragma unroll
+            for (int q = 0; q < DIMS; ++q) mx = FG_FMAX(mx, FG_FABS(val[f][r][q] * rhv[f][r][q]));
+    __shared__ fg_real lds_mx[FG_BLOCK / 64];
+    __shared__ fg_real lds_dt;
+    __shared__ int lds_last;
+    mx = fg_wave_max(mx);
+    if (lane == 0) lds_mx[wave] = mx;
+    __syncthreads();
+    mx = FG_FMAX(FG_FMAX(lds_mx[0], lds_mx[1]), FG_FMAX(lds_mx[2], lds_mx[3]));
+    double total = 0.0;
+    if (a.flux_B) total = fg_flux_balance_block<DIMS>(g, bnd, b);
+    fg_bits prev = 0, prevf = 0;
+    if (threadIdx.x == 0) {
+        prev = __hip_atomic_exchange(reinterpret_cast<fg_bits*>(a.out_B) + b, fg_real_bits(mx), __ATOMIC_RELAXED, __HIP_MEMORY_SCOPE_AGENT);
+        if (a.flux_B) prevf = __hip_atomic_exchange(reinterpret_cast<fg_bits*>(a.flux_B) + b, fg_real_bits((fg_real)total), __ATOMIC_RELAXED, __HIP_MEMORY_SCOPE_AGENT);
+        lds_dt = fg_dt_rule_env(a.rule, b, fg_real_bits(mx));
+    }
+    __syncthreads();
+    const fg_real dtb = lds_dt;
+    if (a.free_mask && dtb > 0.f) fg_balance_env<DIMS>(g, bnd, rw, a.free_mask, a.atol, dtb, fold, b);
+    if (threadIdx.x == 0) {
+        asm volatile("" ::"v"(prev), "v"(prevf));
+        lds_last = (atomicAdd(a.done_B + B, 1) == B - 1);
+    }
+    __syncthreads();
+    if (lds_last && wave == 0) {
+        for (int e = lane; e < B; e += 64) {
+            fg_poll_publish_word(poll, 12 * B + e, __hip_atomic_exchange(reinterpret_cast<fg_bits*>(a.out_B) + e, (fg_bits)0, __ATOMIC_RELAXED, __HIP_MEMORY_SCOPE_AGENT));
+            if (a.flux_B) fg_poll_publish_word(poll, 13 * B + e, __hip_atomic_exchange(reinterpret_cast<fg_bits*>(a.flux_B) + e, (fg_bits)0, __ATOMIC_RELAXED, __HIP_MEMORY_SCOPE_AGENT));
+        }
+        if (lane == 0) atomicExch(a.done_B + B, 0);
+    }
+}
+#endif
 
 inline unsigned fg_reduce_wgs(const fg_state* s) {
     if (s->reduce_wgs > 0) return (unsigned)s->reduce_wgs;
@@ -946,7 +1052,7 @@
 }
 
 int fg_launch_correct(const fg_state* s, const fg_real* dt, const fg_real* rA, const fg_real* hvec, const fg_real* p,
-                      fg_real* vel_out, hipStream_t st, fg_real* vel_copy, const FgMeanRef* mean, const FgLazyRef* lazy) {
+                      fg_real* vel_out, hipStream_t st, fg_real* vel_copy, const FgMeanRef* mean, const FgLazyRef* lazy, fg_real* tile_max) {
     fg_htrace("correct_in");
     const FgMeanRef mr = mean ? *mean : FgMeanRef{nullptr, nullptr, nullptr, nullptr, nullptr};
     const FgLazyRef lz = lazy ? *lazy : FgLazyRef{nullptr, nullptr, nullptr};
@@ -954,8 +1060,13 @@
     const int slot_c = fg_prof_slot(s, FG_PK_CORRECT, nullptr, s->grid.B, cb * (double)s->grid.n, 5.0 * s->grid.dims * (double)s->grid.n, st);
     FG_DISPATCH(s, {
         const FgLaunch L = fg_launch_geometry<DIMS, VEC>(s->grid);
-        FG_LAUNCH_P(s, slot_c, (k_correct<DIMS, VEC>), L.grid, dim3(FG_BLOCK), 0, st, s->grid, dt, rA, hvec, p, vel_out, vel_copy, mr, lz,
-                    L.tiles_x, L.tiles_y, L.tiles);
+        FG_REQUIRE(!tile_max || L.tiles == s->tile_max_tiles, FG_ERR_INVALID_ARG, "fg_launch_correct: tile maxima of another launch geometry");
+        if (tile_max)
+            FG_LAUNCH_P(s, slot_c, (k_correct<DIMS, VEC, true>), L.grid, dim3(FG_BLOCK), 0, st, s->grid, dt, rA, hvec, p, vel_out, vel_copy, mr, lz,
+                        tile_max, L.tiles_x, L.tiles_y, L.tiles);
+        else
+            FG_LAUNCH_P(s, slot_c, (k_correct<DIMS, VEC>), L.grid, dim3(FG_BLOCK), 0, st, s->grid, dt, rA, hvec, p, vel_out, vel_copy, mr, lz,
+                        tile_max, L.tiles_x, L.tiles_y, L.tiles);
     });
     FG_HIP_CHECK(hipGetLastError());
     fg_htrace("correct_out");
@@ -1077,3 +1188,62 @@
     }
     return outflow_mask != 0;
 }
+
+bool fg_step_head_applies(const fg_state* s) {
+#if FG_F64
+    return false;
+#else
+    if (!s->tile_max) return false;
+    for (int f = 0; f < 2 * s->grid.dims; ++f) {
+        if (!s->grid.fixed[f]) continue;
+        const int ax = f >> 1;
+        const long slab_n = ax == 0 ? (long)s->grid.ny * s->grid.nz : ax == 1 ? (long)s->grid.nx * s->grid.nz : (long)s->grid.nx * s->grid.ny;
+        if (slab_n > HEAD_R * FG_BLOCK) return false;
+    }
+    return true;
+#endif
+}
+
+int fg_launch_step_head(const fg_state* s, const FgBounds& bnd, hipStream_t st, FgPollOut poll, bool first, FgDtRule rule, int outflow_mask,
+                        fg_real atol, const fg_real* outflow_velm) {
+#if FG_F64
+    fg_set_error("fg_launch_step_head: fp32 library only");
+    return FG_ERR_UNSUPPORTED;
+#else
+    FG_REQUIRE(fg_step_head_applies(s) && poll.gran && rule.t_rem && rule.dt_out, FG_ERR_INVALID_ARG, "the step head needs result words and the device-side sub-step rule");
+    FG_REQUIRE(!outflow_mask || fg_outflow_folds(s, outflow_mask), FG_ERR_INVALID_ARG, "the step head folds the outflow update of small slabs only");
+    const int B = s->grid.B;
+    FgHeadArgs a;
+    a.tile_max = s->tile_max; a.tiles = s->tile_max_tiles;
+    a.out_B = s->scratch_B + B; a.done_B = reinterpret_cast<int32_t*>(s->scratch_B + 2 * B);
+    a.flux_B = first ? s->scratch_B : nullptr;
+    a.rule = rule; a.free_mask = outflow_mask; a.atol = atol;
+    if (!s->maxvel_clean) FG_HIP_CHECK(hipMemsetAsync(a.out_B, 0, sizeof(fg_real) * B + sizeof(int32_t) * (B + 1), st));
+    s->maxvel_clean = 1;
+    FgOutflowFold fold;
+    fold = FgOutflowFold{};
+    if (outflow_mask) {
+        fold.mask = outflow_mask; fold.vel = s->velocity; fold.scal = s->scalar;
+        for (int x = 0; x < 3; ++x) fold.velm[x] = outflow_velm[x];
+        for (int f = 0; f < 6; ++f) { fold.bscal[f] = s->bscal[f]; fold.nsc[f] = (s->scalar && s->bscal[f]) ? s->cfg.n_scalars : 0; }
+    }
+    FgBvelRw rw;
+    for (int f = 0; f < 6; ++f) rw.p[f] = s->bvel[f];
+    const int d = s->grid.dims;
+    double bytes = 4.0 * s->tile_max_tiles, cells = 0.0;
+    for (int f = 0; f < 2 * d; ++f) {
+        if (!s->grid.fixed[f]) continue;
+        const int ax = f >> 1;
+        const double slab_n = ax == 0 ? (double)s->grid.ny * s->grid.nz : ax == 1 ? (double)s->grid.nx * s->grid.nz : (double)s->grid.nx * s->grid.ny;
+        bytes += 4.0 * d * slab_n * (((outflow_mask >> f) & 1) ? 3.0 : 1.0);
+        cells += slab_n;
+    }
+    const int slot_m = fg_prof_slot(s, FG_PK_MAXVEL, nullptr, B, bytes, 2.0 * d * cells + s->tile_max_tiles, st);
+    if (d == 2)
+        FG_LAUNCH_P(s, slot_m, k_step_head<2>, dim3(B), dim3(FG_BLOCK), 0, st, s->grid, bnd, rw, a, poll, fold);
+    else
+        FG_LAUNCH_P(s, slot_m, k_step_head<3>, dim3(B), dim3(FG_BLOCK), 0, st, s->grid, bnd, rw, a, poll, fold);
+    FG_HIP_CHECK(hipGetLastError());
+    return FG_OK;
+#endif
+}
diff --git a/fluidgym_amd/native.py b/fluidgym_amd/native.py
--- a/fluidgym_amd/native.py
+++ b/fluidgym_amd/native.py
@@ -432,6 +432,11 @@
         out["env"] = {k: v for k, v in sorted(os.environ.items()) if k.startswith(("FG_", "FLUIDGYM_"))}
         return out
 
+    def last_cfl_maxima(self) -> list:
+        out = (self._c_real * self.B)()
+        L.check(self.lib.fg_last_cfl_maxima(self.handle, out), lib=self.lib)
+        return list(out)
+
     def set_return_best(self, on: bool = True):
         L.check(self.lib.fg_set_return_best(self.handle, int(on)), lib=self.lib)
 
diff --git a/include/fluidgym_hip.h b/include/fluidgym_hip.h
--- a/include/fluidgym_hip.h
+++ b/include/fluidgym_hip.h
@@ -450,6 +450,7 @@
 int fg_mb_inflow_disturbance(fg_mb_handle h, const fg_mb_inflow_params* params, void* stream);
 int fg_mb_solver_counters(fg_mb_handle h, int64_t* out13_host, int32_t reset);
 int fg_config_dump(fg_handle h, char* buf, int n);
+int fg_last_cfl_maxima(fg_handle h, fg_real* out_B_host);
 int fg_mb_config_dump(fg_mb_handle h, char* buf, int n);
 int fg_switch_values(int32_t family, char* buf, int32_t n);
 int fg_mb_solver_unconverged(fg_mb_handle h, int64_t* out4_host);
```

Measured after the change: 10720 env-steps/s (median of 4 runs). +3.8%, better.
